# yz-cnsdqz/PSI-release

Measured on AMD Instinct MI355X. Metric: fitting iters/sec (SMPL-X+SDF+Chamfer), PROX-E batch=32, higher is better.
Workload: dtype f32

## Files before the change

include/psi_hip.h:

```cpp
#ifndef PSI_HIP_H
#define PSI_HIP_H

#include <stdint.h>

#ifdef __cplusplus
extern "C" {
#endif

#define PSI_EINVAL (-22)
#define PSI_ETIMEOUT (-110)
#define PSI_ENOMEM (-12)

const char *psi_last_error(void);
int psi_version(void);
int psi_device_info(int *cu_count, int *wave_size, int *clock_khz, int *is_gfx950);

int psi_chamfer_arith_mode(void);
size_t psi_chamfer_workspace_bytes(int B, int n, int m);
int psi_chamfer_forward(const float *xyz1, const float *xyz2, int B, int n, int m,
                        float *dist1, int32_t *idx1, float *dist2, int32_t *idx2,
                        void *workspace, void *stream);
int psi_scratch_release(void *stream, int all);
int psi_chamfer_backward(const float *xyz1, const float *xyz2, float *gradxyz1, float *gradxyz2,
                         const float *graddist1, const float *graddist2,
                         const int32_t *idx1, const int32_t *idx2, int B, int n, int m, void *stream);

typedef struct psi_nn_index psi_nn_index;
int psi_nn_index_create(psi_nn_index **out, const float *h_points, int m);
void psi_nn_index_destroy(psi_nn_index *index);
int psi_nn_index_query(const psi_nn_index *index, const float *xyz1, int B, int n, float *dist1, int32_t *idx1,
                       int32_t *hint, void *stream);

typedef struct psi_nn_index_set psi_nn_index_set;
int psi_nn_index_set_create(psi_nn_index_set **out, const psi_nn_index *const *indices, int S);
void psi_nn_index_set_destroy(psi_nn_index_set *set);
int psi_nn_index_set_query(const psi_nn_index_set *set, const int32_t *slot, const float *xyz1, int B, int n,
                           float *dist1, int32_t *idx1, void *stream);

int psi_sdf_sample_forward(const float *sdf, const int32_t *scene_id, const float *gmin, const float *gmax,
                           const float *verts, int B, int V, int D, int S, int align_corners,
                           float *out_sdf, float *out_grad, void *stream);
int psi_sdf_sample_backward(const float *grad_sdf, const float *out_grad, int B, int V,
                            float *grad_verts, void *stream);
int psi_sdf_penetration_stats(const float *sdf_vals, long n, float *stats, void *stream);

typedef struct psi_lbs_model psi_lbs_model;
int psi_lbs_create(psi_lbs_model **out, const float *h_v_template, const float *h_shapedirs,
                   const float *h_posedirs, const float *h_J_regressor, const float *h_weights,
                   const int32_t *h_parents, int V, int J, int NB);
void psi_lbs_destroy(psi_lbs_model *model);
size_t psi_lbs_workspace_floats(const psi_lbs_model *model, int B);
int psi_lbs_forward(const psi_lbs_model *model, const float *betas, const float *pose, const float *transl,
                    const float *cam_ext, int B, float *verts, float *joints, float *ws, void *stream);
int psi_lbs_backward(const psi_lbs_model *model, const float *grad_verts, const float *betas, const float *pose,
                     const float *cam_ext, int B, float *ws, float *grad_betas, float *grad_pose,
                     float *grad_transl, void *stream);

typedef struct psi_fit_engine psi_fit_engine;
typedef struct psi_fit_config {
    int B, n_contact, m_scene, D, align_corners, world_size, num_pca_comps, max_history;
    int nn_mode;
    float w_rec, w_vposer, w_contact, w_collision, contact_const;
    float lr, beta1, beta2, eps;
    int independent_bodies;
    int concurrent_engines;
    double lr_d, beta1_d, beta2_d;
} psi_fit_config;
int psi_fit_create(psi_fit_engine **out, const psi_lbs_model *lbs, const psi_fit_config *cfg,
                   const float *h_w1, const float *h_b1, const float *h_w2, const float *h_b2,
                   const float *h_w3, const float *h_b3, const float *h_lh_comp, const float *h_rh_comp,
                   const float *h_pose_mean, const int32_t *h_contact_ids,
                   const float *d_scene_verts, const float *d_sdf, const float *h_gmin, const float *h_gmax);
void psi_fit_destroy(psi_fit_engine *engine);
typedef struct psi_fit_scene {
    const float *d_verts;
    const float *d_sdf;
    int m, D;
    float gmin[3], gmax[3];
} psi_fit_scene;
int psi_fit_create_scenes(psi_fit_engine **out, const psi_lbs_model *lbs, const psi_fit_config *cfg,
                          const float *h_w1, const float *h_b1, const float *h_w2, const float *h_b2,
                          const float *h_w3, const float *h_b3, const float *h_lh_comp, const float *h_rh_comp,
                          const float *h_pose_mean, const int32_t *h_contact_ids,
                          const psi_fit_scene *h_scenes, int S);
int psi_fit_set_scene_slots(psi_fit_engine *engine, const int32_t *d_slot, void *stream);
int psi_fit_scene_count(const psi_fit_engine *engine);
int psi_fit_set_problem(psi_fit_engine *engine, const float *d_xhr, const float *d_x_init, const float *d_cam_ext,
                        int reset_optimizer, void *stream);
int psi_fit_forward(psi_fit_engine *engine, float *d_stats, int use_graph, void *stream);
int psi_fit_backward_step(psi_fit_engine *engine, const float *d_stats, int use_graph, void *stream);
int psi_fit_iterate(psi_fit_engine *engine, int n_iter, int use_graph, void *stream);
int psi_fit_read(psi_fit_engine *engine, float *d_x_out, float *d_history_out, int n_hist, int *h_step, void *stream);
int psi_fit_read_losses(psi_fit_engine *engine, int adam_step, float *d_out4, void *stream);
int psi_fit_decode_forward(psi_fit_engine *engine, const float *d_x75, const float *d_cam_ext, float *d_verts, void *stream);
int psi_fit_decode_backward(psi_fit_engine *engine, const float *d_grad_verts, float *d_grad_x75, void *stream);

#define PSI_DP_ID_BYTES 128
typedef struct psi_dp_comm psi_dp_comm;
int psi_dp_unique_id(char *h_id128);
int psi_dp_comm_create(psi_dp_comm **out, const char *h_id128, int rank, int world);
void psi_dp_comm_destroy(psi_dp_comm *comm);
int psi_dp_comm_info(const psi_dp_comm *comm, int *rank, int *world, int *rccl_version);
int psi_dp_allreduce_sum(psi_dp_comm *comm, float *d_buf, int n, void *stream);
int psi_fit_iterate_dp(psi_fit_engine *engine, psi_dp_comm *comm, int n_iter, int use_graph, float *d_stats, void *stream);
int psi_fit_dp_mode(const psi_fit_engine *engine);
int psi_fit_chain_mode(const psi_fit_engine *engine);
int psi_stream_wait(void *stream, int timeout_ms);

int psi_fit_profile(psi_fit_engine *engine, int n_rep, char *h_names, int name_stride, float *h_ms, int max_stages,
                    int *h_n_stages, void *stream);
int psi_fit_copy_buffer(psi_fit_engine *engine, const char *name, float *d_out, long n_floats, void *stream);

size_t psi_linear_workspace_floats(int M, int N, int K);
int psi_linear_forward(const void *x, int x_is_bf16, const float *W, const float *bias, const float *residual, int M, int N, int K,
                       int act, float slope, float *y, float *act_out, float *ws, void *stream);
int psi_linear_forward3(const void *x, int x_is_bf16, const float *W, const float *bias, const float *residual, int M, int N, int K,
                        int act, float slope, float *y, float *act_out, float *ws, void *stream);
size_t psi_linear_backward_workspace_floats(int M, int N, int K);
int psi_linear_backward3(const float *gy, const float *act_out, const float *x, const float *W, int M, int N, int K, float slope, float *gx,
                         float *gW, float *gbias, float *ws, void *stream);
int psi_linear_backward(const float *gy, const float *act_out, const void *x, int x_is_bf16, const float *W, int M, int N, int K,
                        float slope, void *gx, float *gW, float *gbias, float *ws, void *stream);

size_t psi_bn_workspace_floats(long M, int C);
int psi_bn_forward(const void *x, const void *residual, const float *gamma, const float *beta, float *running_mean,
                   float *running_var, long long *num_batches_tracked, long M, int C, int relu, float momentum, float eps,
                   void *y, float *save_mean, float *save_invstd, float *ws, void *stream);
int psi_bn_backward(const void *dy, const void *x, const void *y, const float *gamma, const float *save_mean,
                    const float *save_invstd, long M, int C, int relu, void *dx, void *dresidual, float *dgamma, float *dbeta,
                    float *ws, void *stream);

int psi_conv3x3_supported(int Cin, int Cout, int H, int W);
int psi_conv3x3_forward(const void *x, const void *w, const float *bias, int N, int H, int W, int Cin, int Cout, void *y, void *stream);
size_t psi_conv3x3_wrw_workspace_floats(int N, int H, int W, int Cin, int Cout);
int psi_conv3x3_weight_grad(const void *x, const void *dy, int N, int H, int W, int Cin, int Cout, float *gw, float *ws, void *stream);
int psi_conv3x3_rotate_weight(const void *w, int Cin, int Cout, void *wt, void *stream);
int psi_conv3x3_prepare_weight(const float *w32, int Cin, int Cout, void *wb, void *wt, void *stream);

int psi_maxpool3x3s2_forward(const void *x, int N, int H, int W, int C, void *y, void *idx, void *stream);
int psi_maxpool3x3s2_backward(const void *dy, const void *idx, int N, int H, int W, int C, void *dx, void *stream);

int psi_conv2d_supported(int Cin, int Cout, int KH, int KW, int stride, int pad);
int psi_conv2d_forward(const void *x, int x_bf16, const float *w, const float *bias, int N, int H, int W, int Cin, int Cout, int KH, int KW,
                       int stride, int pad, void *y, int y_bf16, int nterm, void *stream);
int psi_conv2d_input_grad(const void *dy, int dy_bf16, const float *wt, int N, int H, int W, int Cin, int Cout, int KH, int KW, int stride, int pad,
                          void *dx, int dx_bf16, int nterm, void *stream);
int psi_conv2d_prepared_ok(int Cin, int Cout, int KH, int KW, int stride, int pad);
int psi_conv2d_prepare_weight(const float *w, int Cout, int KH, int KW, int Cin, int nterm, void *wf, void *wt, void *stream);
int psi_conv2d_forward_p(const void *x, int x_bf16, const void *wf, const float *bias, int N, int H, int W, int Cin, int Cout, int KH, int KW,
                         int stride, int pad, void *y, int y_bf16, int nterm, void *stream);
int psi_conv2d_input_grad_p(const void *dy, int dy_bf16, const void *wt, int N, int H, int W, int Cin, int Cout, int KH, int KW, int stride, int pad,
                            void *dx, int dx_bf16, int nterm, void *stream);
size_t psi_conv2d_wgrad_workspace_floats(int N, int H, int W, int Cin, int Cout, int KH, int KW, int stride, int pad);
int psi_conv2d_weight_grad(const void *x, int x_bf16, const void *dy, int dy_bf16, int N, int H, int W, int Cin, int Cout, int KH, int KW, int stride,
                           int pad, float *gw, float *ws, int nterm, void *stream);
int psi_adam_step(void *const *p, const void *const *g, void *const *m, void *const *v, const long *n, int count, float *step, unsigned *ticket,
                  double lr, double beta1, double beta2, double eps, double weight_decay, void *stream);
int psi_bn_forward_t(const void *x, int map_f32, const void *residual, const float *gamma, const float *beta, float *running_mean,
                     float *running_var, long long *num_batches_tracked, long M, int C, int relu, float momentum, float eps, void *y,
                     float *save_mean, float *save_invstd, float *ws, int eval_mode, void *stream);
int psi_bn_backward_t(const void *dy, int map_f32, const void *x, const void *y, const float *gamma, const float *beta, const float *save_mean,
                      const float *save_invstd, long M, int C, int relu, void *dx, void *dresidual, float *dgamma, float *dbeta, float *ws,
                      void *stream);
int psi_maxpool3x3s2_forward_t(const void *x, int map_f32, int N, int H, int W, int C, void *y, void *idx, void *stream);
int psi_maxpool3x3s2_backward_t(const void *dy, int map_f32, const void *idx, int N, int H, int W, int C, void *dx, void *stream);

size_t psi_cvae_losses_workspace_floats(void);
int psi_cvae_target(const float *xh72, const float *cam_int, const float *max_d, int B, float *out75, void *stream);
int psi_cvae_losses_forward(const float *rec75, const float *target75, const float *xh72, const float *cam_int, const float *max_d,
                            const float *mu0, const float *logvar0, int nz0, const float *mu1, const float *logvar1, int nz1, int B,
                            float w_rec, float w_kl, float w_vposer, float fca, const float *fca_dev, float *ws, float *xh_rec75,
                            float *losses5, void *stream);
int psi_cvae_losses_backward(const float *rec75, const float *target75, const float *xh72, const float *cam_int, const float *max_d,
                             const float *mu0, const float *logvar0, int nz0, const float *mu1, const float *logvar1, int nz1, int B,
                             float w_rec, float w_kl, float w_vposer, float fca, const float *fca_dev, const float *xh_rec75,
                             const float *g_losses5, const float *g_xh_rec75, float *g_rec75, float *g_mu0, float *g_logvar0,
                             float *g_mu1, float *g_logvar1, void *stream);

size_t psi_scene_losses_workspace_floats(void);
int psi_scene_losses_forward(const float *dist, long n_contact, const float *sdf_vals, long n_sdf, float w_contact, float w_collision,
                             float gate, float *ws, float *losses2, float *stats2, void *stream);
int psi_scene_losses_backward(const float *g_losses2, const float *stats2, const float *dist, const float *xyz1, const int32_t *idx,
                              const int32_t *slot, const float *verts_table, long m, const int32_t *vid, const float *sdf_vals,
                              const float *sdf_grad, int B, int V, int n_c, float w_contact, float w_collision, float gate,
                              const int32_t *chain, float *g_verts, void *stream);
int psi_contact_slot_chain(const int32_t *vid, int n_c, int32_t *chain, void *stream);

int psi_lbs_sdf_counts(const psi_lbs_model *model, const float *betas, const float *pose, const float *transl,
                       const float *cam_ext, int B, const float *sdf, const int32_t *scene_id, const float *gmin,
                       const float *gmax, int D, int S, int align_corners, int32_t *counts, float *ws, void *stream);

typedef struct psi_kmeans psi_kmeans;
int psi_kmeans_create(psi_kmeans **out, const float *obs, int N, int d, const float *guess, int k, int R, float thresh);
void psi_kmeans_destroy(psi_kmeans *km);
int psi_kmeans_iterate(psi_kmeans *km, int n_iter, void *stream);
int psi_kmeans_read(psi_kmeans *km, float *book, int32_t *k_eff, double *avg_dist, int32_t *iters, int *h_converged, void *stream);
int psi_vq(const float *obs, int N, int d, const float *book, int k, int32_t *code, float *dist, void *stream);

typedef struct psi_raster_mesh psi_raster_mesh;
int psi_raster_mesh_create(psi_raster_mesh **out, const float *d_verts, const int32_t *d_faces, const float *d_vlabel, int nv, int nf);
void psi_raster_mesh_destroy(psi_raster_mesh *mesh);
size_t psi_raster_workspace_bytes(int nf, int n_views, int W, int H);
int psi_raster_render(psi_raster_mesh *mesh, const float *d_w2c, const float *d_intr, int n_views, int W, int H, float near_z,
                      float *d_depth, int32_t *d_tri, float *d_seg, int32_t *d_stats, void *d_workspace, void *stream);

typedef struct psi_raster_bodies psi_raster_bodies;
int psi_raster_bodies_create(psi_raster_bodies **out, const int32_t *d_faces, int V, int F);
void psi_raster_bodies_destroy(psi_raster_bodies *bodies);
int psi_raster_bodies_normals(psi_raster_bodies *bodies, const float *d_bverts, int B, float *d_normals, void *stream);
size_t psi_raster_bodies_workspace_bytes(int F, int draws_per_pass, int n_views, int W, int H);
int psi_raster_bodies_render(psi_raster_mesh *scene, const float *d_vrgb, psi_raster_bodies *bodies, const float *d_bverts, int B,
                             const int32_t *d_draw_body, const int32_t *d_draw_view, const float *d_draw_rgb, int M, const float *d_w2c,
                             const float *d_intr, int n_views, int W, int H, float near_z, const float *d_sdepth, const int32_t *d_stri,
                             float bg_r, float bg_g, float bg_b, int draws_per_pass, uint8_t *d_rgb, float *d_depth, int32_t *d_draw,
                             float *d_bdepth, int32_t *d_bid, int32_t *d_counts, int32_t *d_stats, void *d_workspace, void *stream);

typedef struct psi_mesh_sdf psi_mesh_sdf;
int psi_mesh_sdf_create(psi_mesh_sdf **out, const float *d_verts, const int32_t *d_faces, int nv, int nf);
void psi_mesh_sdf_destroy(psi_mesh_sdf *m);
int psi_mesh_sdf_info(const psi_mesh_sdf *m, int32_t info[4]);
int psi_mesh_sdf_compute(psi_mesh_sdf *m, const float gmin[3], const float gmax[3], int D, int mode, float *d_out, void *stream);
int psi_mesh_sdf_count_pairs(psi_mesh_sdf *m, const float gmin[3], const float gmax[3], int D, int mode, unsigned long long *d_pairs,
                             void *stream);

int psi_mesh_winding_compute(psi_mesh_sdf *m, const float gmin[3], const float gmax[3], int D, float beta, int cluster, float *d_f, void *stream);
int psi_mesh_winding_count(psi_mesh_sdf *m, const float gmin[3], const float gmax[3], int D, float beta, int cluster,
                           unsigned long long *d_counts , void *stream);
int psi_mesh_sdf_apply_sign(const float *d_f, float level, float *d_vol, long long n, void *stream);

size_t psi_snapshot_canvas_workspace_bytes(int n_views);
int psi_snapshot_canvas(const float *d_depth, const float *d_seg, int n_views, int H, int W, int th, int tw, float clip_depth, float clip_seg,
                        const int32_t *d_windows, const float *d_target_z, float *d_depth_canvas, float *d_seg_canvas, float *d_max_d,
                        float *d_seg_max, int32_t *d_usable, void *d_workspace, void *stream);

int psi_mesh_cloud_count(const float *d_verts, const int32_t *d_faces, int nv, int nf, float spacing, int32_t *d_tri_rows, float origin[3],
                         long long *n_rows, long long *n_cands, void *stream);
int psi_mesh_cloud_rows(const float *d_verts, const int32_t *d_faces, int nv, int nf, float spacing, const int64_t *d_tri_row_off,
                        long long n_rows, int32_t *d_row_tri, int32_t *d_row_cnt, void *stream);
int psi_mesh_cloud_emit(const float *d_verts, const int32_t *d_faces, int nv, int nf, float spacing, const float origin[3],
                        const int64_t *d_tri_row_off, const int32_t *d_row_tri, const int64_t *d_row_off, long long n_rows, long long n_cands,
                        float *d_pos, int32_t *d_tri, int64_t *d_cell, uint32_t *d_key, void *stream);
int psi_mesh_cloud_winners(const int64_t *d_cell_sorted, const int64_t *d_perm, const uint32_t *d_key, long long n, int32_t *d_keep,
                           void *stream);
int psi_mesh_cloud_compact(const float *d_pos, const int32_t *d_tri, const int32_t *d_keep, const int64_t *d_keep_scan, long long n,
                           long long n_out, float *d_points, int32_t *d_out_tri, void *stream);

int psi_flood_fill(const uint8_t *d_open, int Dx, int Dy, int Dz, const int32_t *d_seed_nodes, int n, uint8_t *d_free, int *h_rounds, void *stream);
int psi_mesh_orient_votes(const float *d_points, const int32_t *d_tri, long long n, const float *d_verts, int nv, const int32_t *d_faces, int nf,
                          const uint8_t *d_free, const float gmin[3], const float gmax[3], int D, float delta, int32_t *d_votes, void *stream);

typedef struct psi_body_overlap psi_body_overlap;
int psi_body_overlap_create(psi_body_overlap **out, const int32_t *h_faces, int V, int F);
void psi_body_overlap_destroy(psi_body_overlap *h);
int psi_body_overlap_info(const psi_body_overlap *h, int32_t info[2]);
size_t psi_body_overlap_workspace_bytes(long long n_cand, int F);
int psi_body_overlap_boxes(const psi_body_overlap *h, const float *d_verts, int B, float *d_boxes, int32_t *d_bad, void *stream);
int psi_body_overlap_count(const psi_body_overlap *h, const float *d_verts, const int32_t *d_group, int B, const float *d_boxes,
                           int32_t *d_pair_count, void *stream);
int psi_body_overlap_emit(const psi_body_overlap *h, const float *d_verts, const int32_t *d_group, int B, const float *d_boxes,
                          const int32_t *d_pair_count, const int64_t *d_cand_off, const int64_t *d_chunk_off, long long n_cand,
                          long long n_chunks, int32_t *d_cand, int32_t *d_chunks, void *stream);
int psi_body_overlap_wind(const psi_body_overlap *h, const float *d_verts, int B, const int32_t *d_cand, long long n_cand,
                          const int32_t *d_chunks, long long n_chunks, void *d_workspace, size_t workspace_bytes, void *stream);
int psi_body_overlap_decide(const psi_body_overlap *h, int B, const int32_t *d_cand, long long n_cand, const void *d_workspace,
                            size_t workspace_bytes, float *d_w, int32_t *d_counts, uint32_t *d_mask, void *stream);
// ... 72 lines not shown
```

psi-release_amd/csrc/fit.hip:

```cpp
#include "psi_internal.h"
#include "blob.h"
#ifdef PSI_HEAD_STOPS
__device__ int psi_dbg_sstop;
#define PSI_SSTOP(k) do { if (psi_dbg_sstop == (k)) return; } while (0)
__device__ int psi_dbg_pstop;
#define PSI_PSTOP(k) do { if (psi_dbg_pstop == (k)) asm volatile("s_endpgm"); } while (0)
__device__ int psi_dbg_cstop;
#define PSI_CSTOP() do { if (psi_dbg_cstop) asm volatile("s_endpgm"); } while (0)
#define PSI_TRACE(lo, hi) PsiBlockTrace trace_((lo), (hi))
__device__ unsigned long long psi_dbg_tl[4 * 8192];
struct PsiBlockTrace {
    unsigned long long t0;
    int kind;
    int sel_lo, sel_hi;
    __device__ PsiBlockTrace(int lo = 9, int hi = 10) : t0(wall_clock64()), kind(0), sel_lo(lo), sel_hi(hi) {}
    __device__ ~PsiBlockTrace()
    {
        const unsigned bid = blockIdx.y * gridDim.x + blockIdx.x;
        if (psi_dbg_sstop < sel_lo || psi_dbg_sstop > sel_hi || threadIdx.x != 0 || bid >= 8192) return;
        unsigned long long *o = psi_dbg_tl + 4 * (size_t)bid;
        o[0] = t0;
        o[1] = wall_clock64();
        o[2] = (unsigned long long)__builtin_amdgcn_s_getreg((31 << 11) | 4) | ((unsigned long long)__builtin_amdgcn_s_getreg((31 << 11) | 20) << 32);
        o[3] = (unsigned long long)kind;
    }
};
extern "C" int psi_dbg_timeline(unsigned long long *out, int nblocks)
{
    return (int)hipMemcpyFromSymbol(out, HIP_SYMBOL(psi_dbg_tl), sizeof(unsigned long long) * 4 * (size_t)(nblocks < 8192 ? nblocks : 8192));
}
#endif
#include "lbs_device.h"
#include "chain_plan.h"
#include "lbs_joint_device.h"
#include "sdf_device.h"
#include "nnindex_device.h"
#include <initializer_list>
#include <limits.h>
#include <memory>
#include <math.h>
#include <stdlib.h>
#include <string.h>
#include <type_traits>
#include <vector>

namespace {

constexpr int NH = 512;
constexpr int NZ = 32;
constexpr int NJ6 = 126;
constexpr int XD = 75;
#ifndef PSI_HEAD_THREADS
#define PSI_HEAD_THREADS 512
#endif
constexpr int HB = PSI_HEAD_THREADS;
static_assert(HB >= 384 && HB % 128 == 0, "the head / tail kernels place work on threads up to 256 + 75");
constexpr int KQ = HB / 128;
constexpr int KS3 = HB / 32;
constexpr int OS1 = HB / 8;
typedef float f4 __attribute__((ext_vector_type(4)));

struct FitDev {
    int B, V, Vpad, J, NB, n_c, m, D, align_corners, world, ncomp, nfp, nsdfblk;
    int indep;
    float w_rec, w_vp, w_contact, w_col, cconst;
    float lr, beta1, beta2, eps;
    float one_m_beta1, one_m_beta2;
    double lr_d, beta1_d, beta2_d;
    const float *W1T, *b1, *W2T, *b2, *W3T, *b3;
    const float *W1, *W2, *W3;
    const float *lhc, *rhc, *pose_mean;
    const int *vid;
    const int *cs_ptr, *cs_idx;
    const int *cs_first;
    const float *scene, *sdf, *gmin, *gmax;
    const float *sdf_cells;
    const float *Wct;
    float *x, *xhr, *cam, *adam_m, *adam_v;
    int *step;
    float *h1, *h2, *o6, *betas20, *pose, *transl, *verts, *og, *gq, *fpart, *penpart, *recpart, *vppart;
    float *cverts;
    float *g_betas, *g_pose, *g_transl, *g_rot;
    unsigned long long *hx_o6, *hx_gh1;
    unsigned *hx_epoch;
    int *hx_err;
    int hc;
#ifdef PSI_HEAD_STOPS
    int stop_h, stop_t;
#define HSTOP(k) do { if (f.stop_h == (k)) return; } while (0)
#define TSTOP(k) do { if (f.stop_t == (k)) return; } while (0)
#else
#define HSTOP(k)
#define TSTOP(k)
#endif
    int *nn_hint;
    float *history;
    int max_hist;
    int fused_bwd, ncp, ncp3;
    float *glc, *gvpc, *vpc;
    float *gtc_part;
#ifndef PSI_GV_SLOTS
#define PSI_GV_SLOTS 1024
#endif
    static_assert(PSI_GV_SLOTS >= 128, "one slot per body and class at least: fused_bwd runs batches up to 128 (merged_scene)");
    unsigned *gvbits;
    int gv_sps;
    const float *dirs_ch;
    const float *WTt_c;
    float *gA_part, *gfeat_part;
    float *spb;
    int nsv, nsv_c, nsn_m, nsn_c, spm, spc;
    unsigned long long *penmask;
    int pen_skip;
};

__device__ __forceinline__ float leaky(float v, float slope) { return v > 0.0f ? v : v * slope; }

__device__ __forceinline__ void gs_forward(const float *x6, float *R)
{
    float a1[3] = {x6[0], x6[2], x6[4]}, a2[3] = {x6[1], x6[3], x6[5]};
    float n1 = fmaxf(sqrtf(a1[0] * a1[0] + a1[1] * a1[1] + a1[2] * a1[2]), 1e-12f);
    float b1[3] = {a1[0] / n1, a1[1] / n1, a1[2] / n1};
    float d = b1[0] * a2[0] + b1[1] * a2[1] + b1[2] * a2[2];
    float u[3] = {a2[0] - d * b1[0], a2[1] - d * b1[1], a2[2] - d * b1[2]};
    float n2 = fmaxf(sqrtf(u[0] * u[0] + u[1] * u[1] + u[2] * u[2]), 1e-12f);
    float b2[3] = {u[0] / n2, u[1] / n2, u[2] / n2};
    float b3[3] = {b1[1] * b2[2] - b1[2] * b2[1], b1[2] * b2[0] - b1[0] * b2[2], b1[0] * b2[1] - b1[1] * b2[0]};
    for (int r = 0; r < 3; r++) {
        R[r * 3 + 0] = b1[r];
        R[r * 3 + 1] = b2[r];
        R[r * 3 + 2] = b3[r];
    }
}

__device__ __forceinline__ void gs_backward(const float *x6, const float *gR, float *g6)
{
    float a1[3] = {x6[0], x6[2], x6[4]}, a2[3] = {x6[1], x6[3], x6[5]};
    float n1 = fmaxf(sqrtf(a1[0] * a1[0] + a1[1] * a1[1] + a1[2] * a1[2]), 1e-12f);
    float b1[3] = {a1[0] / n1, a1[1] / n1, a1[2] / n1};
    float d = b1[0] * a2[0] + b1[1] * a2[1] + b1[2] * a2[2];
    float u[3] = {a2[0] - d * b1[0], a2[1] - d * b1[1], a2[2] - d * b1[2]};
    float n2 = fmaxf(sqrtf(u[0] * u[0] + u[1] * u[1] + u[2] * u[2]), 1e-12f);
    float b2[3] = {u[0] / n2, u[1] / n2, u[2] / n2};
    float gb1[3] = {gR[0], gR[3], gR[6]}, gb2[3] = {gR[1], gR[4], gR[7]}, gb3[3] = {gR[2], gR[5], gR[8]};
    gb1[0] += b2[1] * gb3[2] - b2[2] * gb3[1];
    gb1[1] += b2[2] * gb3[0] - b2[0] * gb3[2];
    gb1[2] += b2[0] * gb3[1] - b2[1] * gb3[0];
    gb2[0] += gb3[1] * b1[2] - gb3[2] * b1[1];
    gb2[1] += gb3[2] * b1[0] - gb3[0] * b1[2];
    gb2[2] += gb3[0] * b1[1] - gb3[1] * b1[0];
    float p = b2[0] * gb2[0] + b2[1] * gb2[1] + b2[2] * gb2[2];
    float gu[3] = {(gb2[0] - b2[0] * p) / n2, (gb2[1] - b2[1] * p) / n2, (gb2[2] - b2[2] * p) / n2};
    float q = gu[0] * b1[0] + gu[1] * b1[1] + gu[2] * b1[2];
    float ga2[3] = {gu[0] - b1[0] * q, gu[1] - b1[1] * q, gu[2] - b1[2] * q};
    for (int i = 0; i < 3; i++) gb1[i] += -d * gu[i] - q * a2[i];
    float r = b1[0] * gb1[0] + b1[1] * gb1[1] + b1[2] * gb1[2];
    float ga1[3] = {(gb1[0] - b1[0] * r) / n1, (gb1[1] - b1[1] * r) / n1, (gb1[2] - b1[2] * r) / n1};
    g6[0] = ga1[0]; g6[2] = ga1[1]; g6[4] = ga1[2];
    g6[1] = ga2[0]; g6[3] = ga2[1]; g6[5] = ga2[2];
}

__device__ __forceinline__ void rotmat_to_aa(const float *R, float *aa)
{
    const float m00 = R[0], m01 = R[3], m02 = R[6], m10 = R[1], m11 = R[4], m12 = R[7], m20 = R[2], m21 = R[5], m22 = R[8];
    float q[4], t;
    if (m22 < 1e-6f) {
        if (m00 > m11) {
            t = 1 + m00 - m11 - m22;
            q[0] = m12 - m21; q[1] = t; q[2] = m01 + m10; q[3] = m20 + m02;
        } else {
            t = 1 - m00 + m11 - m22;
            q[0] = m20 - m02; q[1] = m01 + m10; q[2] = t; q[3] = m12 + m21;
        }
    } else {
        if (m00 < -m11) {
            t = 1 - m00 - m11 + m22;
            q[0] = m01 - m10; q[1] = m20 + m02; q[2] = m12 + m21; q[3] = t;
        } else {
            t = 1 + m00 + m11 + m22;
            q[0] = t; q[1] = m12 - m21; q[2] = m20 - m02; q[3] = m01 - m10;
        }
    }
// ... 262 lines not shown
            return;
        }
        const int cw = psi_ld<int>(contact_of, (unsigned)v * 4u);
        if (!(cw >> 24)) return;
        float *row = cverts + (size_t)b * n_c * 3;
        psi_st(row, (unsigned)(cw & 0xffffff) * 12u, psi_p3{x, y, z});
        if ((cw >> 24) > 1)
            for (int ci = cs_ptr[v] + 1; ci < cs_ptr[v + 1]; ci++) psi_st(row, (unsigned)cs_idx[ci] * 12u, psi_p3{x, y, z});
    }
    __device__ __forceinline__ void vertex(int n, int b, int v, float x, float y, float z, bool live) { vertex_at(G, n, b, v, x, y, z, live); }
    __device__ __forceinline__ void vertex_at(const PsiSdfGrid &G, int n, int b, int v, float x, float y, float z, bool live)
    {
        s[n] = 0.0f;
        neg[n] = false;
#pragma unroll
        for (int a = 0; a < 3; a++) gm[n][a] = 0.0f;
        if (!live) return;
        float g[3];
        if (G.cells) {
            bool in[3];
            const float val = psi_sdf_sample_cells(G, x, y, z, g, in);
            neg[n] = val < 0.0f;
#pragma unroll
            for (int a = 0; a < 3; a++) g[a] = (neg[n] && in[a]) ? g[a] : 0.0f;
            s[n] = neg[n] ? -val : 0.0f;
        } else {
            const float val = psi_trilinear(sdf, gmin, gmax, x, y, z, D, align_corners, g);
            neg[n] = val < 0.0f;
#pragma unroll
            for (int a = 0; a < 3; a++) g[a] = neg[n] ? g[a] : 0.0f;
            s[n] = neg[n] ? -val : 0.0f;
        }
        if (gl) {
#pragma unroll
            for (int a = 0; a < 3; a++) gm[n][a] = g[a];
            return;
        }
        psi_st(og + (size_t)b * Vpad * 4, (unsigned)v * 16u, f4{g[0], g[1], g[2], 0.0f});
    }
    __device__ __forceinline__ void backward(int n, int b, unsigned v12, const psi_f2 (&T2)[6], const float *C)
    {
        if (!gl) return;
        const float gx = gm[n][0], gy = gm[n][1], gz = gm[n][2];
        float lx = gx, ly = gy, lz = gz;
        if (C) {
            lx = psi_dot3(C[0], C[4], C[8], gx, gy, gz);
            ly = psi_dot3(C[1], C[5], C[9], gx, gy, gz);
            lz = psi_dot3(C[2], C[6], C[10], gx, gy, gz);
        }
        psi_st(gl + (size_t)b * Npad, v12, psi_p3{lx, ly, lz});
        const float vx = psi_dot3(T2[0].x, T2[2].x, T2[4].x, lx, ly, lz), vy = psi_dot3(T2[0].y, T2[2].y, T2[4].y, lx, ly, lz),
                    vz = psi_dot3(T2[1].x, T2[3].x, T2[5].x, lx, ly, lz);
        psi_st(gvp + (size_t)b * Npad, v12, psi_p3{vx, vy, vz});
        gvmax[n] = fmaxf(gvmax[n], fmaxf(fabsf(vx), fmaxf(fabsf(vy), fabsf(vz))));
        gs[n][0] = lx; gs[n][1] = ly; gs[n][2] = lz;
    }
    __device__ __forceinline__ void finish(int n, int b, int vblock, int nvb)
    {
        __shared__ psi_f2 red[PSI_SKIN_BLK / 64];
        __shared__ float red3[PSI_SKIN_BLK / 64][3];
        __shared__ float redm[PSI_SKIN_BLK / 64];
        const float ws = psi_wave_sum(s[n]);
        const unsigned long long negm = __builtin_amdgcn_ballot_w64(neg[n]);
        const float wc = (float)(int)__builtin_popcountll(negm);
        if ((threadIdx.x & 63) == 0) red[threadIdx.x >> 6] = (psi_f2){ws, wc};
        if (gl) {
            if ((threadIdx.x & 63) == 0) penmask[((size_t)b * nvb + vblock) * (PSI_SKIN_BLK / 64) + (threadIdx.x >> 6)] = negm;
            const float sx = psi_wave_sum(gs[n][0]), sy = psi_wave_sum(gs[n][1]), sz = psi_wave_sum(gs[n][2]);
            float mx = gvmax[n];
#pragma unroll
            for (int o2 = 32; o2 > 0; o2 >>= 1) mx = fmaxf(mx, __shfl_xor(mx, o2, 64));
            if ((threadIdx.x & 63) == 0) {
                red3[threadIdx.x >> 6][0] = sx;
                red3[threadIdx.x >> 6][1] = sy;
                red3[threadIdx.x >> 6][2] = sz;
                redm[threadIdx.x >> 6] = mx;
            }
        }
        __syncthreads();
        if (gl && threadIdx.x == 64) {
            float mx = redm[0];
#pragma unroll
            for (int w = 1; w < PSI_SKIN_BLK / 64; w++) mx = fmaxf(mx, redm[w]);
            if (mx > 0.0f) atomicMax(gmaxp + (size_t)b * gv_sps + (vblock & (gv_sps - 1)), __float_as_uint(mx));
        }
        if (threadIdx.x == 0) {
            psi_f2 a = red[0];
#pragma unroll
            for (int w = 1; w < PSI_SKIN_BLK / 64; w++) a += red[w];
            *(psi_f2 *)(penpart + ((size_t)b * nvb + vblock) * 2) = a;
        }
        if (gl && threadIdx.x < 3) {
            float a = 0.0f;
#pragma unroll
            for (int w = 0; w < PSI_SKIN_BLK / 64; w++) a += red3[w][threadIdx.x];
            gtp[((size_t)vblock * B + b) * 4 + threadIdx.x] = a;
        }
    }
};

struct SdfPenEpilogueScenes : SdfPenEpilogue {
    const PsiSdfGrid *gtab;
    const int *slot;
    PsiSdfGrid Gb[2];
    template <int NB>
    __device__ __forceinline__ void load_grids(int b0, int B)
    {
#pragma unroll
        for (int n = 0; n < NB; n++) Gb[n] = gtab[slot[min(b0 + n, B - 1)]];
    }
    __device__ __forceinline__ void vertex(int n, int b, int v, float x, float y, float z, bool live) { vertex_at(Gb[n], n, b, v, x, y, z, live); }
};

template <bool SCENES>
using SdfEpilogue = std::conditional_t<SCENES, SdfPenEpilogueScenes, SdfPenEpilogue>;

template <bool SCENES>
static inline SdfEpilogue<SCENES> make_sdf_epilogue(const FitDev &f, const PsiSdfGrid &G, bool contact_vertices_only, const PsiLbsView *bwd,
                                                    const PsiSdfGrid *gtab = nullptr, const int *slot = nullptr)
{
    SdfEpilogue<SCENES> e;
    static_cast<SdfPenEpilogue &>(e) = {SCENES ? PsiSdfGrid{} : G, f.sdf, f.gmin, f.gmax, f.og, f.penpart, f.D, f.align_corners, f.Vpad,
                                        contact_vertices_only ? f.cs_first : nullptr, {0.0f, 0.0f}, {false, false}, f.cverts, f.cs_ptr, f.cs_idx, f.n_c,
                                        nullptr, nullptr, nullptr, 0, f.B, {}, {}, {0.0f, 0.0f}, f.gvbits, f.gv_sps, nullptr};
    if (bwd) {
        e.penmask = f.penmask;
        e.gl = bwd->gl;
        e.gvp = bwd->g_vp;
        e.gtp = bwd->gt_part_w;
        e.Npad = bwd->m.Npad;
    }
    if constexpr (SCENES) {
        e.gtab = gtab;
        e.slot = slot;
        e.Gb[0] = e.Gb[1] = PsiSdfGrid{};
    }
    return e;
}

template <int LPQ>
__device__ __forceinline__ void psi_contact_part_sums(float x, float (&out)[psi_sum_parts_per_wave(LPQ)])
{
    x += psi_dpp<0xB1, 0xf>(x);
    x += psi_dpp<0x4E, 0xf>(x);
    x += psi_dpp<0x124, 0xf>(x);
    x += psi_dpp<0x128, 0xf>(x);
    x += psi_dpp<0x142, 0xa>(x);
    if (psi_sum_part_lanes(LPQ) == 64) x += psi_dpp<0x143, 0xc>(x);
#pragma unroll
    for (int p = 0; p < psi_sum_parts_per_wave(LPQ); p++)
        out[p] = __builtin_bit_cast(float, __builtin_amdgcn_readlane(__builtin_bit_cast(int, x), psi_sum_last_lane(LPQ, p)));
}

template <int LPQ>
struct ContactSkinSrc {
    static_assert(LPQ == 2 || LPQ == 4, "the query's lane group skins its own vertex with 2 or 4 lanes");
    static constexpr int NT = psikd::kd_threads(LPQ);
    static constexpr int NST = (PSI_JP * 6 + NT - 1) / NT;
    static constexpr int CT0 = LPQ == 2 ? 80 : 128;
    FitDev f;
    LbsDev m;
    const float *As, *v_posed;
    psi_f2 (*sA)[6];
    psi_f2 st[NST];
    float ct;
    int v;
    float px, py, pz;
    float *sCT;
    static constexpr int NWQ = PSI_JP / 4 - 2, NWE = 10;
    f4 wq[NWE];
    int jslot;
    float (*sTR)[9] = nullptr;
    float gvm = 0.0f;
    float gs[3] = {0.0f, 0.0f, 0.0f};
    int bq = 0;
    bool live = false;
    __device__ __forceinline__ void issue(int b, int j, bool active)
    {
        jslot = j;
        bq = b;
        live = active;
#pragma unroll
        for (int q = 0; q < NST; q++) {
            const int idx = threadIdx.x + q * NT;
            st[q] = idx < m.J * 6 ? psi_ld<psi_f2>(As + (size_t)b * m.J * 12, (unsigned)idx * 8u) : (psi_f2){0.0f, 0.0f};
        }
        const int k = (int)threadIdx.x - CT0;
        ct = 0.0f;
        if (k >= 0 && k < 12) ct = f.cam[(size_t)b * 16 + k];
        else if (k >= 12 && k < 15) ct = f.transl[(size_t)b * 3 + (k - 12)];
        v = f.vid[j];
    }
    __device__ __forceinline__ void fetch(int b)
    {
        const psi_p3 p = psi_ld<psi_p3>(v_posed + (size_t)b * m.Npad, (unsigned)v * 12u);
        px = p.x; py = p.y; pz = p.z;
        const f4 *wrow = (const f4 *)(f.Wct + (size_t)jslot * PSI_JP);
#pragma unroll
        for (int q = 0; q < NWE; q++) wq[q] = wrow[q];
    }
    __device__ __forceinline__ void prepare(int)
    {
        psi_f2 (*sA_)[6] = psi_transform_stage<1>()[0];
        __shared__ float sCT_[16];
        __shared__ float sTR_[psikd::kd_qpb(LPQ)][9];
#pragma unroll
        for (int q = 0; q < NST; q++) {
            const int idx = threadIdx.x + q * NT;
            if (idx < PSI_JP * 6) (&sA_[0][0])[idx] = st[q];
        }
        const int k = (int)threadIdx.x - CT0;
        if (k >= 0 && k < 16) sCT_[k] = ct;
        __syncthreads();
        sA = sA_;
        sCT = sCT_;
        sTR = sTR_;
    }
    __device__ __forceinline__ void point(int b, int j, int c, float &qx, float &qy, float &qz) const
    {
        if constexpr (LPQ == 2) {
            const f4 *wrow = (const f4 *)(f.Wct + (size_t)j * PSI_JP);
            psi_f2 T0 = {0.0f, 0.0f}, T1 = {0.0f, 0.0f}, U0 = {0.0f, 0.0f}, U1 = {0.0f, 0.0f};
#pragma unroll
            for (int q = 0; q < NWQ; q++) {
                const f4 w4 = q < NWE ? wq[q] : wrow[q];
#pragma unroll
                for (int t = 0; t < 4; t++) {
                    const psi_f2 w2 = {w4[t], w4[t]};
                    T0 = __builtin_elementwise_fma(w2, sA[q * 4 + t][2 * c], T0);
                    T1 = __builtin_elementwise_fma(w2, sA[q * 4 + t][2 * c + 1], T1);
                    U0 = __builtin_elementwise_fma(w2, sA[q * 4 + t][4], U0);
                    U1 = __builtin_elementwise_fma(w2, sA[q * 4 + t][5], U1);
                }
            }
            if (f.fused_bwd) {
                float *tr = sTR[threadIdx.x / LPQ];
                tr[3 * c] = T0.x; tr[3 * c + 1] = T0.y; tr[3 * c + 2] = T1.x;
                if (c == 0) { tr[6] = U0.x; tr[7] = U0.y; tr[8] = U1.x; }
                if (c == 0 && live) psi_st(f.vpc + (size_t)b * f.ncp3, (unsigned)j * 12u, psi_p3{px, py, pz});
            }
            const float xr = psi_dot3p(T0.x, T0.y, T1.x, T1.y, px, py, pz) + sCT[12 + c];
            const float xr2 = psi_dot3p(U0.x, U0.y, U1.x, U1.y, px, py, pz) + sCT[14];
            const int base = (threadIdx.x & 63) & ~1;
            const float x = __shfl(xr, base, 64), y = __shfl(xr, base + 1, 64), z = __shfl(xr2, base, 64);
            const float *C = sCT;
            qx = psi_dot3p(C[0], C[1], C[2], C[3], x, y, z);
            qy = psi_dot3p(C[4], C[5], C[6], C[7], x, y, z);
            qz = psi_dot3p(C[8], C[9], C[10], C[11], x, y, z);
            return;
        }
        const int r = c < 2 ? c : 2;
        const f4 *wrow = (const f4 *)(f.Wct + (size_t)j * PSI_JP);
        psi_f2 T0 = {0.0f, 0.0f}, T1 = {0.0f, 0.0f};
#pragma unroll
        for (int q = 0; q < NWQ; q++) {
            const f4 w4 = q < NWE ? wq[q] : wrow[q];
#pragma unroll
            for (int t = 0; t < 4; t++) {
                const psi_f2 w2 = {w4[t], w4[t]};
                T0 = __builtin_elementwise_fma(w2, sA[q * 4 + t][2 * r], T0);
                T1 = __builtin_elementwise_fma(w2, sA[q * 4 + t][2 * r + 1], T1);
            }
        }
        if (f.fused_bwd && c < 3) {
            float *tr = &sTR[threadIdx.x / LPQ][3 * c];
            tr[0] = T0.x; tr[1] = T0.y; tr[2] = T1.x;
        }
        float xr = psi_dot3p(T0.x, T0.y, T1.x, T1.y, px, py, pz) + sCT[12 + r];
        const int base = (threadIdx.x & 63) & ~3;
        const float x = __shfl(xr, base, 64), y = __shfl(xr, base + 1, 64), z = __shfl(xr, base + 2, 64);
        const float *C = sCT;
        qx = psi_dot3p(C[0], C[1], C[2], C[3], x, y, z);
        qy = psi_dot3p(C[4], C[5], C[6], C[7], x, y, z);
        qz = psi_dot3p(C[8], C[9], C[10], C[11], x, y, z);
    }
    __device__ __forceinline__ void contact_post(size_t, float gx, float gy, float gz)
    {
        if (!f.fused_bwd) return;
        const float *C = sCT;
        const float lx = psi_dot3(C[0], C[4], C[8], gx, gy, gz), ly = psi_dot3(C[1], C[5], C[9], gx, gy, gz), lz = psi_dot3(C[2], C[6], C[10], gx, gy, gz);
        const float *R = sTR[threadIdx.x / LPQ];
        const size_t row = (size_t)bq * f.ncp3;
        const unsigned off = (unsigned)jslot * 12u;
        psi_st(f.glc + row, off, psi_p3{lx, ly, lz});
        const float vx = psi_dot3(R[0], R[3], R[6], lx, ly, lz), vy = psi_dot3(R[1], R[4], R[7], lx, ly, lz), vz = psi_dot3(R[2], R[5], R[8], lx, ly, lz);
        psi_st(f.gvpc + row, off, psi_p3{vx, vy, vz});
        gvm = fmaxf(fabsf(vx), fmaxf(fabsf(vy), fabsf(vz)));
        if constexpr (LPQ != 2) psi_st(f.vpc + row, off, psi_p3{px, py, pz});
        gs[0] = lx; gs[1] = ly; gs[2] = lz;
    }
    __device__ __forceinline__ void contact_finish(int b, int bx, int nbx)
    {
        if (!f.fused_bwd) return;
        constexpr int PPW = psi_sum_parts_per_wave(LPQ);
        __shared__ float wsum3[psi_sum_parts(LPQ)][3];
        __shared__ float wmax[psi_sum_waves(LPQ)];
        float sx[PPW], sy[PPW], sz[PPW];
        psi_contact_part_sums<LPQ>(gs[0], sx);
        psi_contact_part_sums<LPQ>(gs[1], sy);
        psi_contact_part_sums<LPQ>(gs[2], sz);
        float mx = gvm;
#pragma unroll
        for (int o2 = 32; o2 > 0; o2 >>= 1) mx = fmaxf(mx, __shfl_xor(mx, o2, 64));
        if ((threadIdx.x & 63) == 0) {
#pragma unroll
            for (int p = 0; p < PPW; p++) {
                wsum3[psi_sum_slot(LPQ, threadIdx.x >> 6, p)][0] = sx[p];
                wsum3[psi_sum_slot(LPQ, threadIdx.x >> 6, p)][1] = sy[p];
                wsum3[psi_sum_slot(LPQ, threadIdx.x >> 6, p)][2] = sz[p];
            }
            wmax[threadIdx.x >> 6] = mx;
        }
        __syncthreads();
        if (threadIdx.x == 64) {
            float m2 = wmax[0];
#pragma unroll
            for (int w = 1; w < psi_sum_waves(LPQ); w++) m2 = fmaxf(m2, wmax[w]);
            if (m2 > 0.0f) atomicMax(f.gvbits + PSI_GV_SLOTS + (size_t)b * f.gv_sps + (bx & (f.gv_sps - 1)), __float_as_uint(m2));
        }
        if (threadIdx.x < 3) {
            float a = 0.0f;
#pragma unroll
            for (int w = 0; w < psi_sum_parts(LPQ); w++) a += wsum3[w][threadIdx.x];
            f.gtc_part[((size_t)b * nbx + bx) * 4 + threadIdx.x] = a;
        }
    }
};

#ifdef PSI_HEAD_STOPS
extern "C" int psi_dbg_kd_mark(unsigned long long *out, int nblocks)
{
    return (int)hipMemcpyFromSymbol(out, HIP_SYMBOL(psi_kd_mark), sizeof(unsigned long long) * 4 * (size_t)(nblocks < 8192 ? nblocks : 8192));
}
extern "C" int psi_dbg_kd_reason(int *out) { return (int)hipMemcpyFromSymbol(out, HIP_SYMBOL(psi_kd_reason), sizeof(int) * 8); }
extern "C" int psi_dbg_kd_stat(int *out, int nblocks)
{
    return (int)hipMemcpyFromSymbol(out, HIP_SYMBOL(psi_kd_stat), sizeof(int) * 4 * (size_t)(nblocks < 8192 ? nblocks : 8192));
}
#endif
template <bool SCENES>
using SceneTrees = std::conditional_t<SCENES, const psikd::KdDev *__restrict__, psikd::KdDev>;

template <int NB, bool SCENES, int LPQ>
__global__ __launch_bounds__(256, 6) void fwd_scene_kernel(FitDev f, LbsDev m, const float *__restrict__ As, const float *__restrict__ v_posed,
                                                           SceneTrees<SCENES> T, int n_kd, int nqb, int rows, float gscale, int skin_first, SdfEpilogue<SCENES> epi)
{
    extern __shared__ int smem_i[];
#ifdef PSI_HEAD_STOPS
    if (psi_dbg_sstop == 1 && (int)blockIdx.x >= n_kd) return;
    if (psi_dbg_sstop == 2 && (int)blockIdx.x < n_kd) return;
    if (psi_dbg_sstop == 3) return;
    PsiBlockTrace trace;
    if (threadIdx.x < 4 && blockIdx.x < 8192) psi_kd_stat[4 * blockIdx.x + threadIdx.x] = 0;
    trace.kind = skin_first ? ((int)blockIdx.x >= (int)gridDim.x - n_kd) : ((int)blockIdx.x < n_kd);
#endif
    int bid = blockIdx.x;
    bool is_kd;
    if (skin_first) {
        const int n_sk = (int)gridDim.x - n_kd;
        is_kd = bid >= n_sk;
        if (is_kd) bid -= n_sk;
    } else {
        is_kd = bid < n_kd;
        if (!is_kd) bid -= n_kd;
    }
    if (is_kd) {
        const int b = bid / nqb, bx = bid % nqb;
        psikd::KdDev tree = psikd::KdDev();
        const psikd::KdDev *__restrict__ tab = nullptr;
        const int *slot = nullptr;
        if constexpr (SCENES) {
            tab = T;
            slot = epi.slot;
        } else tree = T;
        psikd::kd_query_body<LPQ, true, SCENES>(tree, ContactSkinSrc<LPQ>{f, m, As, v_posed, nullptr, {}, 0.0f, 0, 0.0f, 0.0f, 0.0f, nullptr, {}, 0}, f.n_c, (float *)nullptr, (int *)nullptr,
                                           f.cconst, gscale, f.fused_bwd ? (float *)nullptr : f.gq, f.fpart, f.nn_hint, rows, tab, slot, bx, b, nqb, smem_i);
    } else {
        const int i = bid;
        if constexpr (SCENES) epi.template load_grids<NB>((i / f.nsdfblk) * NB, f.B);
        psi_skin_fwd_body<NB, PsiBlendCompact>(m, As, v_posed, f.transl, f.cam, f.B, f.verts, epi, i % f.nsdfblk, (i / f.nsdfblk) * NB, f.nsdfblk);
    }
}

template <int NB, bool SCENES>
__global__ __launch_bounds__(PSI_SKIN_BLK, 6) void skin_fwd_sdf_kernel(LbsDev m, const float *__restrict__ As, const float *__restrict__ v_posed,
                                                                     const float *__restrict__ transl, const float *__restrict__ cam_ext,
                                                                     int B, float *__restrict__ verts, SdfEpilogue<SCENES> epi)
{
    if constexpr (SCENES) epi.template load_grids<NB>((int)blockIdx.y * NB, B);
    psi_skin_fwd_body<NB, PsiBlendPipelined>(m, As, v_posed, transl, cam_ext, B, verts, epi, (int)blockIdx.x, (int)blockIdx.y * NB, (int)gridDim.x);
}

__global__ void contact_weight_table_kernel(const float *__restrict__ WT, int Vpad, const int *__restrict__ vid, int n_c, int J, float *__restrict__ Wct)
{
    const int i = blockIdx.x * 256 + threadIdx.x;
    if (i >= n_c * PSI_JP) return;
    const int slot = i / PSI_JP, j = i % PSI_JP;
    Wct[i] = j < J ? WT[(size_t)j * Vpad + vid[slot]] : 0.0f;
}

__global__ __launch_bounds__(1024) void loss_finalize_kernel(FitDev f, float *stats)
{
    __shared__ float red[16];
    const int t = threadIdx.x, nt = 1024;
    auto total = [&](const float *p, int n, int stride) {
        float a0 = 0, a1 = 0, a2 = 0, a3 = 0;
        int i = t;
        for (; i + 3 * nt < n; i += 4 * nt) {
            a0 += p[(size_t)i * stride];
            a1 += p[(size_t)(i + nt) * stride];
            a2 += p[(size_t)(i + 2 * nt) * stride];
            a3 += p[(size_t)(i + 3 * nt) * stride];
        }
        for (; i < n; i += nt) a0 += p[(size_t)i * stride];
        return block_sum((a0 + a1) + (a2 + a3), red);
    };
    float s_rec = total(f.recpart, f.B, 1);
    float s_vp = total(f.vppart, f.B, 1);
    float s_f = total(f.fpart, f.B * f.nfp, 1);
    float s_pen = total(f.penpart, f.B * f.nsdfblk, 2);
    float n_pen = total(f.penpart + 1, f.B * f.nsdfblk, 2);
    if (t == 0) {
        stats[0] = s_rec; stats[1] = s_vp; stats[2] = s_f; stats[3] = s_pen; stats[4] = n_pen; stats[5] = 0.0f;
        *f.step += 1;
    }
}

__device__ __forceinline__ void fit_stats_body(const FitDev &f, float *__restrict__ stats)
{
    __shared__ float red[16];
    const int t = threadIdx.x, nt = blockDim.x;
    if (f.indep) {
        float a0 = 0, a1 = 0, a2 = 0, a3 = 0;
        for (int b = t; b < f.B; b += nt) {
            a0 += f.recpart[b];
            a1 += f.vppart[b];
            float sf = 0, sp = 0, cn = 0;
            for (int k = 0; k < f.nfp; k++) sf += f.fpart[(size_t)b * f.nfp + k];
            for (int k = 0; k < f.nsdfblk; k++) {
                sp += f.penpart[2 * ((size_t)b * f.nsdfblk + k)];
                cn += f.penpart[2 * ((size_t)b * f.nsdfblk + k) + 1];
            }
            a2 += sf;
            a3 += cn > 0.0f ? sp / cn : 0.0f;
            f.spb[b] = cn > 0.0f ? -f.w_col / cn : 0.0f;
        }
        const float s0 = block_sum(a0, red), s1 = block_sum(a1, red), s2 = block_sum(a2, red), s3 = block_sum(a3, red);
        if (t == 0) {
            stats[0] = s0; stats[1] = s1; stats[2] = s2; stats[3] = s3; stats[4] = 0.0f; stats[5] = 0.0f;
            *f.step += 1;
        }
        return;
    }
    auto total = [&](const float *p, int n, int stride) {
        float a0 = 0, a1 = 0, a2 = 0, a3 = 0;
        int i = t;
        for (; i + 3 * nt < n; i += 4 * nt) {
            a0 += p[(size_t)i * stride];
            a1 += p[(size_t)(i + nt) * stride];
            a2 += p[(size_t)(i + 2 * nt) * stride];
            a3 += p[(size_t)(i + 3 * nt) * stride];
        }
        for (; i < n; i += nt) a0 += p[(size_t)i * stride];
        return block_sum((a0 + a1) + (a2 + a3), red);
    };
    const float s_rec = total(f.recpart, f.B, 1);
    const float s_vp = total(f.vppart, f.B, 1);
    const float s_f = total(f.fpart, f.B * f.nfp, 1);
    const float s_pen = total(f.penpart, f.B * f.nsdfblk, 2);
    const float n_pen = total(f.penpart + 1, f.B * f.nsdfblk, 2);
    if (t == 0) {
        stats[0] = s_rec; stats[1] = s_vp; stats[2] = s_f; stats[3] = s_pen; stats[4] = n_pen; stats[5] = 0.0f;
        *f.step += 1;
    }
}

#ifndef PSI_FIT_PF_MODEL
#define PSI_FIT_PF_MODEL 1
#endif
#ifndef PSI_FIT_PF_CONTACT
#define PSI_FIT_PF_CONTACT 2
#endif
template <int MT, int PF_MODEL, int PF_CONTACT>
__global__ __launch_bounds__(256) __attribute__((amdgpu_waves_per_eu(2, 2))) void fit_bwd_joint_kernel(
    FitDev f, LbsDev m, const float *__restrict__ g_vp, const float *__restrict__ gl, const float *__restrict__ v_posed, PsiSkaPlan ska, int n_blend,
    int kgroups, float *__restrict__ stats)
{
    const int n_ska = ska.n_ska;
    constexpr int SMEM_B = psi_blend_bwd_h_smem_f4<(MT + 1) / 2>();
    __shared__ f4 smem[SMEM_B > SKA_SMEM_F4 ? SMEM_B : SKA_SMEM_F4];
    const int bid = blockIdx.x;
#ifdef PSI_HEAD_STOPS
    PsiBlockTrace trace(11, 11);
    trace.kind = bid < n_ska ? (bid < ska.n_c ? 1 : 0) : (bid < n_ska + n_blend ? 2 : 4);
#endif
    if (bid < n_ska) {
        int sl, b0, nbody;
        psi_ska_map(ska, bid, sl, b0, nbody);
        float *part = f.gA_part + (size_t)sl * f.B * PSI_JP * 16;
        if (sl < f.nsv) {
            const PsiSkaSlice o = {m.WTt + (size_t)sl * 4 * PSI_JP * 64, gl + (size_t)sl * 768, v_posed + (size_t)sl * 768, (size_t)m.Npad, part};
            const unsigned all = (1u << min(nbody, f.B - b0)) - 1u;
            const unsigned live = f.pen_skip ? psi_pen_slice_live(f.penmask, f.Vpad / 64, sl, f.B, b0, nbody) : all;
            skin_bwd_A_zero(o, b0, all & ~live);
            if (live) skin_bwd_A_dispatch_live(o, b0, live, smem);
        } else {
            const int c = sl - f.nsv;
            const PsiSkaSlice o = {f.WTt_c + (size_t)c * 4 * PSI_JP * 64, f.glc + (size_t)c * 768, f.vpc + (size_t)c * 768, (size_t)f.ncp3, part};
            skin_bwd_A_dispatch(o, f.B, b0, nbody, smem);
        }
    } else if (bid < n_ska + n_blend) {
        int kg, slice, bg;
        psi_blend_bwd_place(bid - n_ska, kgroups, f.nsn_m + f.nsn_c, kg, slice, bg);
#ifdef PSI_HEAD_STOPS
        trace.kind = slice < f.nsn_m ? 2 : 3;
#endif
        float *part = f.gfeat_part + (size_t)slice * f.B * m.Kpad;
        const float dsc_inv = m.dirs_unscale * PSI_FEAT_SCALE;
        if (slice < f.nsn_m) {
            const PsiBlendBwdColsH o = {m.dirs_bh, g_vp, (size_t)m.Npad, m.Kpad, m.Npad / 16, f.gvbits, f.gv_sps, dsc_inv, f.pen_skip ? f.penmask : nullptr, f.Vpad / 64};
            blend_bwd_h_body<(MT + 1) / 2, PF_MODEL>(o, f.B, slice * f.spm, (slice + 1) * f.spm, part, kg, bg, smem);
        } else {
            const int c = slice - f.nsn_m;
            const PsiBlendBwdColsH o = {f.dirs_ch, f.gvpc, (size_t)f.ncp3, m.Kpad, f.ncp3 / 16, f.gvbits + PSI_GV_SLOTS, f.gv_sps, dsc_inv, nullptr, 0};
            blend_bwd_h_body<(MT + 1) / 2, PF_CONTACT>(o, f.B, c * f.spc, (c + 1) * f.spc, part, kg, bg, smem);
        }
    } else {
        fit_stats_body(f, stats);
    }
// ... 322 lines not shown
        gs_backward(o6v, sgrot + t * 9, g6);
        for (int i = 0; i < 6; i++) sg6[(t - 1) * 6 + i] = g6[i];
    } else if (t >= 64 && t < 64 + 2 * f.ncomp) {
        int i = t - 64;
        const float *comp = i < f.ncomp ? f.lhc : f.rhc;
        int ii = i < f.ncomp ? i : i - f.ncomp;
        const float *gp = sgpose + (i < f.ncomp ? 75 : 120);
        float a = 0;
        for (int e = 0; e < 45; e++) a += comp[ii * 45 + e] * gp[e];
        sgx[(i < f.ncomp ? 51 : 63) + ii] = a;
    } else if (t >= 128 && t < 128 + 3) {
        sgx[t - 128] = gtv;
    } else if (t >= 160 && t < 160 + 10) {
        sgx[9 + (t - 160)] = sgbetas[t - 160];
    }
    __syncthreads();
    TSTOP(3);
    {
        f4 a = {0, 0, 0, 0};
#pragma unroll
        for (int i = 0; i < PRE3; i++) a += w3p[i] * sg6[o0 + i];
#pragma unroll 8
        for (int o = o0 + PRE3; o < o1; o++) a += *(const f4 *)(w3 + (size_t)o * NH) * sg6[o];
        part4[os3 * NQ + og3] = a;
    }
    __syncthreads();
    if (t < NS) {
        float a = 0.0f;
        const float *p = (const float *)part4;
#pragma unroll
        for (int q = 0; q < OSPL; q++) a += p[q * NS + t];
        sga2[t] = a * (h2v > 0.0f ? 1.0f : 0.2f);
    }
    __syncthreads();
    TSTOP(4);
    {
        f4 a0 = {0, 0, 0, 0}, a1 = {0, 0, 0, 0};
        const float *g = sga2 + kq2 * RPER;
#pragma unroll
        for (int o = 0; o < PRE2; o += 2) {
            a0 += w2p[o] * g[o];
            a1 += w2p[o + 1] * g[o + 1];
        }
#pragma unroll 8
        for (int o = PRE2; o < RPER; o += 2) {
            a0 += *(const f4 *)(w2 + (size_t)o * NH) * g[o];
            a1 += *(const f4 *)(w2 + (size_t)(o + 1) * NH) * g[o + 1];
        }
        part4[kq2 * 128 + og2] = a0 + a1;
    }
    __syncthreads();
    TSTOP(5);
    {
        const float *p = (const float *)part4;
        float a = p[t];
#pragma unroll
        for (int q = 1; q < KQ; q++) a += p[q * NH + t];
        if (C == 1) {
            sga1[t] = a * (h1[t] > 0.0f ? 1.0f : 0.2f);
        } else if (!last) {
            hx_put(f.hx_gh1 + ((size_t)b * C + c) * NH + t, a, tag);
            return;
        } else {
            unsigned long long *p8 = f.hx_gh1 + (size_t)b * C * NH + t;
            unsigned long long w[C - 1 ? C - 1 : 1];
#pragma unroll
            for (int cc = 0; cc < C - 1; cc++) w[cc] = hx_peek(p8 + (size_t)cc * NH);
            float o = 0.0f;
#pragma unroll
            for (int cc = 0; cc < C - 1; cc++) o += hx_value(p8 + (size_t)cc * NH, w[cc], tag, f.hx_err);
            sga1[t] = (o + a) * (h1v > 0.0f ? 1.0f : 0.2f);
        }
    }
    __syncthreads();
    TSTOP(6);
    {
        f4 a = {0, 0, 0, 0};
        if (C == 1) {
#pragma unroll
            for (int i = 0; i < O1; i++) a += *(const f4 *)(w1 + (size_t)i * NZ) * sga1[os1 * O1 + i];
        } else {
#pragma unroll
            for (int i = 0; i < O1; i++) a += w1p[i] * sga1[os1 * O1 + i];
        }
        part1[os1][kg1] = a;
    }
    __syncthreads();
    if (t < 8) {
        f4 a = {0, 0, 0, 0};
        for (int os = 0; os < OS1; os++) a += part1[os][t];
        for (int e = 0; e < 4; e++) sgx[19 + t * 4 + e] = a[e];
    }
    __syncthreads();
    TSTOP(7);
    if (C > 1 && t == 0) f.hx_epoch[f.B + b] = tag;
    if (!ADAM) {
        if (t < XD) g_out[(size_t)b * XD + t] = sgx[t];
        return;
    }
    if (ta >= 0 && ta < XD) {
        const float Bg = f.indep ? 1.0f : (float)f.B * (float)f.world;
        float g = sgx[ta];
        float df = xhrv - sx[ta];
        g += f.w_rec / (Bg * XD) * (df > 0.0f ? -1.0f : (df < 0.0f ? 1.0f : 0.0f));
        if (ta >= 19 && ta < 19 + NZ) g += f.w_vp / (Bg * NZ) * 2.0f * sx[ta];
        size_t o = (size_t)b * XD + ta;
        float m = am * f.beta1 + f.one_m_beta1 * g;
        float v = av * f.beta2 + f.one_m_beta2 * g * g;
        f.adam_m[o] = m;
        f.adam_v[o] = v;
        float denom = sqrtf(v) / bc2_sqrt + f.eps;
        f.x[o] = sx[ta] - step_size * (m / denom);
    }
}

__global__ void sdf_to_cells_kernel(const float *__restrict__ src, float *__restrict__ dst, int D)
{
    const int nbr = D >> 2;
    const size_t i = (size_t)blockIdx.x * 256 + threadIdx.x, n = (size_t)D * D * D * 8;
    if (i >= n) return;
    const int c = (int)(i & 7), l = (int)((i >> 3) & 63);
    const size_t br = i >> 9;
    const int bz = (int)(br % nbr), by = (int)((br / nbr) % nbr), bx = (int)(br / ((size_t)nbr * nbr));
    const int ix = min(4 * bx + (l >> 4) + (c >> 2), D - 1), iy = min(4 * by + ((l >> 2) & 3) + ((c >> 1) & 1), D - 1),
              iz = min(4 * bz + (l & 3) + (c & 1), D - 1);
    dst[i] = src[((size_t)ix * D + iy) * D + iz];
}

__global__ void scene_slots_kernel(const int *__restrict__ src, int *__restrict__ dst, int B, int S)
{
    const int b = blockIdx.x * 256 + threadIdx.x;
    if (b < B) dst[b] = min(max(src[b], 0), S - 1);
}

__global__ void adam_reset_kernel(float *m, float *v, int *step, int n)
{
    int i = blockIdx.x * 256 + threadIdx.x;
    if (i < n) { m[i] = 0.0f; v[i] = 0.0f; }
    if (i == 0) *step = 0;
}

}

#ifndef PSI_FIT_SEARCH_LANES_DEFAULT
#define PSI_FIT_SEARCH_LANES_DEFAULT 2
#endif
#ifndef PSI_GRAPH_UNROLL
#define PSI_GRAPH_UNROLL 10
#endif
constexpr int GRAPH_UNROLL = PSI_GRAPH_UNROLL;

struct FitKnobs {
    bool split_scene, keep_verts, no_fused_bwd, sdf_linear, scene_skin_first, bwdv_mb, no_pen_skip, bwd_pf1, chain_in_head;
    int head_cluster, skin_nb, ska_nbody, search_lanes;
#ifdef PSI_HEAD_STOPS
    int head_stop, tail_stop, skin_stop;
#endif
};

static FitKnobs fit_read_knobs()
{
    auto is = [](const char *name, char c) { const char *v = getenv(name); return v && v[0] == c; };
    auto num = [](const char *name) { const char *v = getenv(name); return v ? atoi(v) : 0; };
    FitKnobs k = {};
    k.split_scene = is("PSI_SPLIT_SCENE", '1');
    k.keep_verts = is("PSI_KEEP_VERTS", '1');
    k.no_fused_bwd = is("PSI_FIT_FUSED_BWD", '0');
    k.no_pen_skip = is("PSI_FIT_PEN_SKIP", '0');
    k.bwd_pf1 = is("PSI_FIT_BWD_PF", '1');
    k.chain_in_head = is("PSI_FIT_CHAIN_IN_HEAD", '1');
    k.sdf_linear = is("PSI_SDF_LINEAR", '1');
    k.scene_skin_first = is("PSI_SCENE_ORDER", '1');
    k.bwdv_mb = is("PSI_BWDV_MB", '1');
    const int hc = num("PSI_HEAD_CLUSTER");
    if (hc == 1 || hc == 2 || hc == 4 || hc == 8) k.head_cluster = hc;
    if (getenv("PSI_SKIN_NB")) k.skin_nb = num("PSI_SKIN_NB") == 2 ? 2 : 1;
    k.ska_nbody = psi_ska_nbody_override(SKA_NBODY);
    const int sl = num("PSI_FIT_SEARCH_LANES");
    if (sl == 2 || sl == 4) k.search_lanes = sl;
#ifdef PSI_HEAD_STOPS
    k.head_stop = num("PSI_HEAD_STOP");
    k.tail_stop = num("PSI_TAIL_STOP");
    k.skin_stop = num("PSI_SKIN_STOP");
#endif
    return k;
}

struct FitModes {
    bool self_skin;
    bool merged_scene;
    bool keep_verts;
    bool fused_bwd;
    int skin_nb;
    int search_lanes;
    int hc;
    int gv_sps;
    PsiStreamSplit split;
    PsiChainPlan chain;
};

static FitModes fit_decide(const psi_fit_config *cfg, const FitKnobs &knobs, int J, int ncp3, const PsiLbsCounts &mc, int cus)
{
    FitModes d = {};
    d.self_skin = cfg->nn_mode == 1 && J <= PSI_JP - 8 && psikd::kd_qpb(psikd::LPQ_OPS) == psikd::kd_qpb(2);
    d.search_lanes = knobs.search_lanes ? knobs.search_lanes : mc.compressed_weights ? 4 : PSI_FIT_SEARCH_LANES_DEFAULT;
    d.merged_scene = d.self_skin && cfg->B <= 128 && !knobs.split_scene;
    d.keep_verts = !d.merged_scene || knobs.keep_verts;
    const long bodies = (long)cfg->B * (cfg->concurrent_engines > 1 ? cfg->concurrent_engines : 1);
    d.hc = bodies <= 32 ? 8 : bodies <= 64 ? 4 : bodies <= 128 ? 2 : 1;
    if (knobs.head_cluster) d.hc = knobs.head_cluster;
    d.gv_sps = 16;
    while (d.gv_sps > 1 && (long)d.gv_sps * cfg->B > PSI_GV_SLOTS) d.gv_sps >>= 1;
    d.split = psi_stream_split(mc.Npad / 16, ncp3 / 16, mc.nsn);
    d.fused_bwd = d.merged_scene && !knobs.no_fused_bwd && d.split.nsn_c > 0;
    d.skin_nb = cfg->B > 128 && !mc.compressed_weights ? 2 : 1;
    if (knobs.skin_nb) d.skin_nb = knobs.skin_nb;
    d.chain = knobs.chain_in_head ? PsiChainPlan{0, 0} : psi_chain_plan(cfg->B, d.hc, mc.blend_wg, mc.blend_gy, cus);
    return d;
}

struct FitPlan {
    int mt;
    int kgroups, n_blend;
    PsiSkaPlan ska;
    bool pf1;
};
static FitPlan fit_plan_make(const FitDev &f, const LbsDev &m, int ska_nbody_override, bool pf1)
{
    FitPlan p;
    p.kgroups = m.Kpad / 64;
    p.mt = f.B > 32 ? 4 : (f.B > 16 ? 2 : 1);
    p.n_blend = p.kgroups * (f.nsn_m + f.nsn_c) * psi_cdiv(f.B, 16 * p.mt);
    p.ska = psi_ska_plan(f.B, f.nsv, f.nsv_c, SKA_NBODY, ska_nbody_override);
    p.pf1 = pf1;
    return p;
}

struct FitGraph { hipGraph_t g; hipGraphExec_t exec; bool ready; };

struct FitCaptured {
    enum Kind { Ok, Refused, Error } kind;
    int rc;
};

template <class Seq>
static FitCaptured fit_graph_capture(FitGraph *G, hipStream_t st, Seq &&seq)
{
    auto failed = [](const char *what, hipError_t he) {
        psi_set_error("%s failed: %s", what, hipGetErrorString(he));
        return FitCaptured{FitCaptured::Error, (int)he};
    };
    if (!st) {
        psi_set_error("invalid argument: graph capture needs a non-default stream");
        return {FitCaptured::Error, PSI_EINVAL};
    }
    hipError_t he = hipStreamBeginCapture(st, hipStreamCaptureModeRelaxed);
    if (he != hipSuccess) return failed("begin of the stream capture", he);
    const int rc = seq();
    hipGraph_t g = nullptr;
    he = hipStreamEndCapture(st, &g);
    if (!rc && he == hipSuccess) {
        he = hipGraphInstantiate(&G->exec, g, nullptr, nullptr, 0);
        if (he != hipSuccess) {
            (void)hipGraphDestroy(g);
            return failed("hipGraphInstantiate", he);
        }
        G->g = g;
        G->ready = true;
        return {FitCaptured::Ok, 0};
    }
    if (g) (void)hipGraphDestroy(g);
    if (!rc) (void)failed("hipStreamEndCapture", he);
    const bool refused = (he >= hipErrorStreamCaptureUnsupported && he <= hipErrorStreamCaptureWrongThread) || rc == 1000 + 4 || rc == 1000 + 5;
    return {refused ? FitCaptured::Refused : FitCaptured::Error, rc ? rc : (int)he};
}

static int fit_graph_launch(const FitGraph &G, hipStream_t st)
{
    PSI_CHECK_HIP(hipGraphLaunch(G.exec, st));
    return 0;
}

static void fit_graph_drop(FitGraph *G)
{
    if (G->ready) {
        (void)hipGraphExecDestroy(G->exec);
        (void)hipGraphDestroy(G->g);
    }
    *G = FitGraph{};
}

struct FitGraphTier { int iters; FitGraph *graph; };

template <class Seq>
static FitCaptured fit_run_graphs(hipStream_t st, int n_iter, int *done, std::initializer_list<FitGraphTier> tiers, Seq &&one)
{
    for (const FitGraphTier &t : tiers) {
        if (n_iter - *done < t.iters) continue;
        if (!t.graph->ready) {
            const FitCaptured c = fit_graph_capture(t.graph, st, [&]() {
                int rc = 0;
                for (int i = 0; i < t.iters && !rc; i++) rc = one();
                return rc;
            });
            if (c.kind != FitCaptured::Ok) return c;
        }
        for (; *done + t.iters <= n_iter; *done += t.iters)
            if (int rc = fit_graph_launch(*t.graph, st)) return {FitCaptured::Error, rc};
    }
    return {FitCaptured::Ok, 0};
}

enum {
    FIT_G_ITER_1, FIT_G_ITER_N, FIT_G_ITER_2N,
    FIT_G_HALF_FWD, FIT_G_HALF_BWD,
    FIT_G_DP_1, FIT_G_DP_N,
    FIT_N_GRAPHS
};

struct psi_fit_engine {
    FitDev d;
    PsiSdfGrid grid;
    const psi_lbs_model *lbs;
    psi_nn_index *nn_index;
    float *lbs_ws;
    PsiLbsView lv;
    void *nn_ws;
    char *blob;
    PsiBlob table;
    float *stats_local;
    FitKnobs knobs;
    FitModes mode;
    FitPlan plan;
    int n_scenes;
    psi_nn_index **scene_index;
    float **scene_vol;
    char *scene_blob;
    psikd::KdDev *d_kd_tab;
    PsiSdfGrid *d_grid_tab;
    int *d_slot;
    int kd_rows;
    FitGraph graphs[FIT_N_GRAPHS];
    const float *half_stats[2];
    const void *dp_comm;
    const float *dp_stats;
    bool dp_warm;
    bool dp_no_graph;
};

template <bool LINKS_IN_HEAD>
static void launch_head_fwd(const FitDev &f, const PsiLbsView &lv, hipStream_t st)
{
    const dim3 g(f.B * f.hc), blk(HB);
    switch (f.hc) {
    case 8: hipLaunchKernelGGL((head_fwd_kernel<8, LINKS_IN_HEAD>), g, blk, 0, st, f, lv); break;
    case 4: hipLaunchKernelGGL((head_fwd_kernel<4, LINKS_IN_HEAD>), g, blk, 0, st, f, lv); break;
    case 2: hipLaunchKernelGGL((head_fwd_kernel<2, LINKS_IN_HEAD>), g, blk, 0, st, f, lv); break;
    default: hipLaunchKernelGGL((head_fwd_kernel<1, true>), g, blk, 0, st, f, lv); break;
    }
}

static int fit_head_blend(psi_fit_engine *e, hipStream_t st)
{
    const FitDev &f = e->d;
    const PsiChainPlan &cp = e->mode.chain;
    const bool role = cp.n_links_wg > 0 && f.hc > 1;
    if (role) launch_head_fwd<false>(f, e->lv, st);
    else launch_head_fwd<true>(f, e->lv, st);
    PSI_CHECK_LAUNCH("head_fwd_kernel");
    psi_mark("head_fwd_kernel", st);
    return role ? psi_lbs_blend_forward_links(e->lbs, f.B, e->lbs_ws, cp.n_links_wg, cp.bodies_per_wave, st)
                : psi_lbs_blend_forward(e->lbs, f.B, e->lbs_ws, st);
}

template <bool ADAM>
static void launch_head_bwd(const FitDev &f, const PsiLbsView &lv, float *g_out, hipStream_t st)
{
    const dim3 g(f.B * f.hc), blk(HB);
    switch (f.hc) {
    case 8: hipLaunchKernelGGL((head_bwd_adam_kernel<8, ADAM>), g, blk, 0, st, f, lv, g_out); break;
    case 4: hipLaunchKernelGGL((head_bwd_adam_kernel<4, ADAM>), g, blk, 0, st, f, lv, g_out); break;
    case 2: hipLaunchKernelGGL((head_bwd_adam_kernel<2, ADAM>), g, blk, 0, st, f, lv, g_out); break;
    default: hipLaunchKernelGGL((head_bwd_adam_kernel<1, ADAM>), g, blk, 0, st, f, lv, g_out); break;
    }
}

enum class FitStats {
    Finalize,
    Backward,
    Caller
};

static inline FitStats fit_stats_source(const psi_fit_engine *e, FitStats wish)
{
    return wish == FitStats::Backward && !e->mode.fused_bwd && e->d.B >= PSI_SKIN_MB_MIN_B ? FitStats::Finalize : wish;
}

static int fit_launch_stats(psi_fit_engine *e, float *stats, hipStream_t st)
{
    hipLaunchKernelGGL(loss_finalize_kernel, dim3(1), dim3(1024), 0, st, e->d, stats);
    PSI_CHECK_LAUNCH("loss_finalize_kernel");
    psi_mark("loss_finalize_kernel", st);
    return 0;
}

template <int NB, bool SCENES, int LPQ>
static void launch_fwd_scene(const psi_fit_engine *e, float gscale, hipStream_t st)
{
    const FitDev &f = e->d;
    const int nqb = f.nfp, n_kd = nqb * f.B, skin_first = e->knobs.scene_skin_first ? 1 : 0;
    const dim3 grid(n_kd + f.nsdfblk * psi_cdiv(f.B, NB));
    FitDev fk = f;
    if (!e->mode.keep_verts) fk.verts = nullptr;
    const auto epi = make_sdf_epilogue<SCENES>(f, e->grid, false, e->mode.fused_bwd ? &e->lv : nullptr, e->d_grid_tab, e->d_slot);
    SceneTrees<SCENES> T;
    int rows;
    if constexpr (SCENES) {
        T = e->d_kd_tab;
        rows = e->kd_rows;
    } else {
        T = psi_nn_index_dev(e->nn_index);
        rows = T.rows;
    }
    hipLaunchKernelGGL((fwd_scene_kernel<NB, SCENES, LPQ>), grid, dim3(256), psikd::kd_lds_bytes(LPQ, rows), st, fk, e->lv.m, e->lv.A, e->lv.v_posed, T, n_kd, nqb, rows,
                       gscale, skin_first, epi);
}

template <int NB, bool SCENES>
static void launch_skin_fwd_sdf(const psi_fit_engine *e, bool all_verts, hipStream_t st)
{
    const FitDev &f = e->d;
    hipLaunchKernelGGL((skin_fwd_sdf_kernel<NB, SCENES>), dim3(f.nsdfblk, psi_cdiv(f.B, NB)), dim3(PSI_SKIN_BLK), 0, st, e->lv.m, e->lv.A, e->lv.v_posed,
                       f.transl, f.cam, f.B, f.verts, make_sdf_epilogue<SCENES>(f, e->grid, !all_verts, nullptr, e->d_grid_tab, e->d_slot));
}

template <class L>
static void fit_scene_dispatch(const psi_fit_engine *e, L &&launch)
{
    using One = std::integral_constant<int, 1>;
    using Two = std::integral_constant<int, 2>;
    switch ((e->n_scenes ? 2 : 0) | (e->mode.skin_nb == 2 ? 1 : 0)) {
    case 0: launch(One{}, std::false_type{}); break;
    case 1: launch(Two{}, std::false_type{}); break;
    case 2: launch(One{}, std::true_type{}); break;
    default: launch(Two{}, std::true_type{}); break;
    }
}

static int fit_forward(psi_fit_engine *e, float *stats, hipStream_t st, FitStats who)
{
    FitDev &f = e->d;
    int rc = fit_head_blend(e, st);
    if (rc) return rc;
    float gscale = f.w_contact / ((f.indep ? 1.0f : (float)f.B * (float)f.world) * (float)f.n_c);
    if (e->nn_index && e->mode.merged_scene) {
        fit_scene_dispatch(e, [&](auto nb, auto scenes) {
            if (e->mode.search_lanes == 2) launch_fwd_scene<decltype(nb)::value, decltype(scenes)::value, 2>(e, gscale, st);
            else launch_fwd_scene<decltype(nb)::value, decltype(scenes)::value, 4>(e, gscale, st);
        });
        PSI_CHECK_LAUNCH("fwd_scene_kernel");
        psi_mark("fwd_scene_kernel", st);
    } else {
        const bool all_verts = !e->nn_index || e->knobs.keep_verts;
        fit_scene_dispatch(e, [&](auto nb, auto scenes) { launch_skin_fwd_sdf<decltype(nb)::value, decltype(scenes)::value>(e, all_verts, st); });
        PSI_CHECK_LAUNCH("skin_fwd_sdf_kernel");
        psi_mark("skin_fwd_sdf_kernel", st);
        if (e->n_scenes)
            rc = psi_nn_index_contact_set(e->d_kd_tab, e->d_slot, e->kd_rows, all_verts ? f.verts : f.cverts, all_verts ? (long)f.V * 3 : (long)f.n_c * 3,
                                          all_verts ? f.vid : nullptr, f.B, f.n_c, f.cconst, gscale, f.gq, f.fpart, f.nn_hint, st);
        else if (e->nn_index && !all_verts)
            rc = psi_nn_index_contact(e->nn_index, f.cverts, (long)f.n_c * 3, nullptr, f.B, f.n_c, f.cconst, gscale, f.gq, f.fpart, f.nn_hint, st);
        else if (e->nn_index)
            rc = psi_nn_index_contact(e->nn_index, f.verts, (long)f.V * 3, f.vid, f.B, f.n_c, f.cconst, gscale, f.gq, f.fpart, f.nn_hint, st);
        else
            rc = psi_nn_contact(f.verts, (long)f.V * 3, f.vid, f.scene, f.B, f.n_c, f.m, e->nn_ws, f.cconst, gscale, f.gq, f.fpart, nullptr, st);
        if (rc) return rc;
    }
    return fit_stats_source(e, who) == FitStats::Finalize ? fit_launch_stats(e, stats, st) : 0;
}

static int fit_backward_joint(psi_fit_engine *e, float *stats, hipStream_t st, FitStats who)
{
    FitDev &f = e->d;
    const FitPlan &p = e->plan;
    const dim3 grid(p.ska.n_ska + p.n_blend + (fit_stats_source(e, who) == FitStats::Backward ? 1 : 0));
#define PSI_LAUNCH_FIT_JOINT(MT_, PFM_, PFC_)                                                                                      \
    hipLaunchKernelGGL((fit_bwd_joint_kernel<MT_, PFM_, PFC_>), grid, dim3(256), 0, st, f, e->lv.m, e->lv.g_vp, e->lv.gl, e->lv.v_posed, p.ska, p.n_blend, p.kgroups, stats)
#define PSI_LAUNCH_FIT_JOINT_MT(MT_)                                                                                               \
    do {                                                                                                                           \
        if (p.pf1) PSI_LAUNCH_FIT_JOINT(MT_, 1, 1);                                                                                \
        else PSI_LAUNCH_FIT_JOINT(MT_, PSI_FIT_PF_MODEL, PSI_FIT_PF_CONTACT);                                                      \
    } while (0)
    if (p.mt == 4) PSI_LAUNCH_FIT_JOINT_MT(4);
    else if (p.mt == 2) PSI_LAUNCH_FIT_JOINT_MT(2);
    else PSI_LAUNCH_FIT_JOINT_MT(1);
#undef PSI_LAUNCH_FIT_JOINT_MT
#undef PSI_LAUNCH_FIT_JOINT
    PSI_CHECK_LAUNCH("fit_bwd_joint_kernel");
    psi_mark("bwd_joint_kernel", st);
    return 0;
}

static int fit_backward_tail(psi_fit_engine *e, float *stats, hipStream_t st)
{
    FitDev &f = e->d;
    const long nred = (long)f.B * PSI_JP * 16 + (long)f.B * e->lv.m.Kpad + (long)f.B * 4;
    hipLaunchKernelGGL(fit_reduce_kernel, dim3(psi_cdiv(nred * PSI_RSPL, 256)), dim3(256), 0, st, f, e->lv, stats);
    PSI_CHECK_LAUNCH("fit_reduce_kernel");
    psi_mark("reduce_partials_kernel", st);
    launch_head_bwd<true>(f, e->lv, nullptr, st);
    PSI_CHECK_LAUNCH("head_bwd_adam_kernel");
    psi_mark("head_bwd_adam_kernel", st);
    return 0;
}

static int fit_backward(psi_fit_engine *e, float *stats, hipStream_t st, FitStats who)
{
    FitDev &f = e->d;
    if (e->mode.fused_bwd) {
        int rc = fit_backward_joint(e, stats, st, who);
        return rc ? rc : fit_backward_tail(e, stats, st);
    }
    const bool big = f.B >= PSI_SKIN_MB_MIN_B;
    const bool mb = big && (e->lv.m.Wc || e->knobs.bwdv_mb);
    const dim3 bgrid(f.nsdfblk, mb ? psi_cdiv(f.B, PSI_SKIN_MB) : f.B);
#define PSI_LAUNCH_BWD_V(...)                                                                                                      \
    hipLaunchKernelGGL((psi_skin_bwd_v_kernel<__VA_ARGS__>), bgrid, dim3(PSI_SKIN_BLK), 0, st, e->lv.m, e->lv.A, src, f.cam, f.B, e->lv.gl, e->lv.g_vp, e->lv.gt_part_w)
    if (fit_stats_source(e, who) == FitStats::Backward) {
        const FitGradSource<true> src{f, stats, 0.0f, nullptr, 0, {}, false};
        if (mb) psi_launch_skin_bwd_v_mb(e->lv.m, e->lv.A, src, f.cam, f.B, e->lv.gl, e->lv.g_vp, e->lv.gt_part_w, st);
        else PSI_LAUNCH_BWD_V(FitGradSource<true>);
    } else {
        const FitGradSource<false> src{f, stats, 0.0f, nullptr, 0, {}, false};
        if (mb) psi_launch_skin_bwd_v_mb(e->lv.m, e->lv.A, src, f.cam, f.B, e->lv.gl, e->lv.g_vp, e->lv.gt_part_w, st);
        else if (big) PSI_LAUNCH_BWD_V(FitGradSource<false>, PsiBlendPipelined);
        else PSI_LAUNCH_BWD_V(FitGradSource<false>);
    }
#undef PSI_LAUNCH_BWD_V
    PSI_CHECK_LAUNCH("skin_bwd_v_grad_kernel");
    psi_mark("skin_bwd_v_grad_kernel", st);
    int rc = psi_lbs_backward_joint_parts(e->lbs, f.B, e->lbs_ws, f.g_transl, st);
    if (rc) return rc;
    launch_head_bwd<true>(f, e->lv, nullptr, st);
    PSI_CHECK_LAUNCH("head_bwd_adam_kernel");
    psi_mark("head_bwd_adam_kernel", st);
    return 0;
}

static int fit_build_scenes(psi_fit_engine *e, const psi_fit_scene *h_scenes, int S);

static inline size_t fit_x_bytes(const FitDev &f) { return (size_t)f.B * XD * 4; }
static inline size_t fit_cam_bytes(const FitDev &f) { return (size_t)f.B * 16 * 4; }
static inline size_t fit_hint_bytes(const FitDev &f) { return (size_t)f.B * f.n_c * 4; }
static inline hipError_t fit_hints_reset(const FitDev &f, hipStream_t st) { return hipMemsetAsync(f.nn_hint, 0xff, fit_hint_bytes(f), st); }

static inline size_t sdf_cells_bytes(int D) { return (size_t)D * D * D * 32; }
static void sdf_cells_fill(const float *d_sdf, float *d_cells, int D)
{
    hipLaunchKernelGGL(sdf_to_cells_kernel, dim3((unsigned)psi_cdiv((long)(sdf_cells_bytes(D) / 4), 256)), dim3(256), 0, 0, d_sdf, d_cells, D);
}

static int fit_scene_index(psi_nn_index **out, const float *d_verts, int m, hipError_t *err)
{
    std::vector<float> hs((size_t)m * 3);
    *err = hipMemcpy(hs.data(), d_verts, hs.size() * 4, hipMemcpyDeviceToHost);
    return *err == hipSuccess ? psi_nn_index_create(out, hs.data(), m) : (int)*err;
}

static int fit_create(psi_fit_engine **out, const psi_lbs_model *lbs, const psi_fit_config *cfg,
                      const float *h_w1, const float *h_b1, const float *h_w2, const float *h_b2,
                      const float *h_w3, const float *h_b3, const float *h_lh_comp, const float *h_rh_comp,
                      const float *h_pose_mean, const int32_t *h_contact_ids,
                      const float *d_scene_verts, const float *d_sdf, const float *h_gmin, const float *h_gmax,
                      const psi_fit_scene *h_scenes, int S)
{
    PSI_REQUIRE(out && lbs && cfg && h_w1 && h_b1 && h_w2 && h_b2 && h_w3 && h_b3 && h_lh_comp && h_rh_comp && h_pose_mean &&
                h_contact_ids && d_scene_verts && d_sdf && h_gmin && h_gmax, "null pointer");
    int V, J, NB;
    psi_lbs_dims(lbs, &V, &J, &NB);
    PSI_REQUIRE(J == 55 && NB >= 10 && NB <= 32, "the fused engine is SMPL-X shaped (J=55, 10..32 betas)");
    PSI_REQUIRE(cfg->B > 0 && cfg->n_contact > 0 && cfg->n_contact < (1 << 24) && cfg->m_scene > 0 && cfg->D >= 2 && cfg->world_size >= 1, "bad sizes");
    PSI_REQUIRE(cfg->num_pca_comps > 0 && cfg->num_pca_comps <= 12, "1..12 hand PCA components");
    PSI_REQUIRE(!(cfg->independent_bodies && cfg->world_size > 1), "independent bodies have no cross-rank coupling: use world_size 1");
    for (int i = 0; i < 66; i++) PSI_REQUIRE(h_pose_mean[i] == 0.0f, "pose_mean must be zero for global_orient/body joints");
    for (int i = 0; i < cfg->n_contact; i++) PSI_REQUIRE(h_contact_ids[i] >= 0 && h_contact_ids[i] < V, "contact id out of range");
    PsiLbsCounts mc;
    if (int rcv = psi_lbs_counts(lbs, cfg->B, &mc)) return rcv;
    psi_fit_engine *e = new psi_fit_engine();
    std::unique_ptr<psi_fit_engine, void (*)(psi_fit_engine *)> owner(e, psi_fit_destroy);
    const FitKnobs &knobs = e->knobs = fit_read_knobs();
    e->lbs = lbs;
    FitDev &f = e->d;
    f.B = cfg->B; f.V = V; f.J = J; f.NB = NB; f.n_c = cfg->n_contact; f.m = cfg->m_scene; f.D = cfg->D;
    f.align_corners = cfg->align_corners; f.world = cfg->world_size; f.ncomp = cfg->num_pca_comps;
    f.indep = cfg->independent_bodies ? 1 : 0;
    f.w_rec = cfg->w_rec; f.w_vp = cfg->w_vposer; f.w_contact = cfg->w_contact; f.w_col = cfg->w_collision; f.cconst = cfg->contact_const;
    f.lr = cfg->lr; f.beta1 = cfg->beta1; f.beta2 = cfg->beta2; f.eps = cfg->eps;
    f.lr_d = cfg->lr_d != 0.0 ? cfg->lr_d : (double)cfg->lr;
    f.beta1_d = cfg->beta1_d != 0.0 ? cfg->beta1_d : (double)cfg->beta1;
    f.beta2_d = cfg->beta2_d != 0.0 ? cfg->beta2_d : (double)cfg->beta2;
    f.one_m_beta1 = (float)(1.0 - f.beta1_d);
    f.one_m_beta2 = (float)(1.0 - f.beta2_d);
    f.nsdfblk = psi_cdiv(V, 256);
    f.Vpad = f.nsdfblk * 256;
    f.nfp = cfg->nn_mode == 1 ? psi_nn_index_fparts(f.n_c) : psi_nn_contact_fparts(f.n_c);
    f.max_hist = cfg->max_history > 0 ? cfg->max_history : 1024;
    f.ncp = psi_cdiv(f.n_c, 256) * 256;
    f.ncp3 = 3 * f.ncp;
    f.nsv = mc.nsv;
    f.nsv_c = f.ncp / 256;
    f.scene = d_scene_verts;
    f.sdf = d_sdf;
    int dev = 0, cus = 0;
    PSI_CHECK_HIP(hipGetDevice(&dev));
    PSI_CHECK_HIP(hipDeviceGetAttribute(&cus, hipDeviceAttributeMultiprocessorCount, dev));
    const FitModes &mode = e->mode = fit_decide(cfg, knobs, J, f.ncp3, mc, cus);
    f.hc = mode.hc;
    f.gv_sps = mode.gv_sps;
    f.fused_bwd = mode.fused_bwd ? 1 : 0;
    f.pen_skip = mode.fused_bwd && !knobs.no_pen_skip ? 1 : 0;
    f.nsn_m = mode.split.nsn_m; f.nsn_c = mode.split.nsn_c; f.spm = mode.split.spm; f.spc = mode.split.spc;
#ifdef PSI_HEAD_STOPS
    f.stop_h = knobs.head_stop;
    f.stop_t = knobs.tail_stop;
    (void)hipMemcpyToSymbol(HIP_SYMBOL(psi_dbg_sstop), &knobs.skin_stop, sizeof(int));
    (void)hipMemcpyToSymbol(HIP_SYMBOL(psi_dbg_pstop), &f.stop_t, sizeof(int));
    const int cstop = knobs.head_stop == 9;
    (void)hipMemcpyToSymbol(HIP_SYMBOL(psi_dbg_cstop), &cstop, sizeof(int));
#endif
    const size_t B = (size_t)f.B;
    std::vector<float> W1T((size_t)NZ * NH), W2T((size_t)NH * NH), W3T((size_t)NH * 128, 0.0f), b3p(128, 0.0f);
    memcpy(b3p.data(), h_b3, NJ6 * 4);
    for (int o = 0; o < NH; o++) for (int k = 0; k < NZ; k++) W1T[(size_t)k * NH + o] = h_w1[(size_t)o * NZ + k];
    for (int o = 0; o < NH; o++) for (int k = 0; k < NH; k++) W2T[(size_t)k * NH + o] = h_w2[(size_t)o * NH + k];
    for (int o = 0; o < NJ6; o++) for (int k = 0; k < NH; k++) W3T[(size_t)k * 128 + o] = h_w3[(size_t)o * NH + k];
    std::vector<int> cs_ptr(V + 1, 0), cs_idx(f.n_c), cs_first(V, 0);
    for (int i = 0; i < f.n_c; i++) cs_ptr[h_contact_ids[i] + 1]++;
    for (int v = 0; v < V; v++) cs_ptr[v + 1] += cs_ptr[v];
    {
        std::vector<int> fill(cs_ptr.begin(), cs_ptr.end() - 1);
        for (int i = 0; i < f.n_c; i++) cs_idx[fill[h_contact_ids[i]]++] = i;
        for (int v = 0; v < V; v++)
            if (cs_ptr[v + 1] > cs_ptr[v]) cs_first[v] = cs_idx[cs_ptr[v]] | (std::min(cs_ptr[v + 1] - cs_ptr[v], 127) << 24);
    }
    const size_t hand_pca = (size_t)f.ncomp * 45 * 4, hidden = B * NH * 4, betas = B * NB * 4, pose = B * J * 3 * 4, transl = B * 3 * 4,
                 crows = B * f.n_c * 3 * 4, per_body = B * 4, slot_rows = B * f.ncp3 * 4;
    PsiBlob &T = e->table;
    T.upload(f.W1T, W1T.data(), W1T.size() * 4);
    T.upload(f.b1, h_b1, NH * 4);
    T.upload(f.W2T, W2T.data(), W2T.size() * 4);
    T.upload(f.b2, h_b2, NH * 4);
    T.upload(f.W3T, W3T.data(), W3T.size() * 4);
    T.upload(f.b3, b3p.data(), 128 * 4);
    T.upload(f.W1, h_w1, (size_t)NH * NZ * 4);
    T.upload(f.W2, h_w2, (size_t)NH * NH * 4);
    T.upload(f.W3, h_w3, (size_t)NJ6 * NH * 4);
    T.upload(f.lhc, h_lh_comp, hand_pca);
    T.upload(f.rhc, h_rh_comp, hand_pca);
    T.upload(f.pose_mean, h_pose_mean, (size_t)J * 3 * 4);
    T.upload(f.vid, h_contact_ids, (size_t)f.n_c * sizeof(int32_t));
    T.upload(f.cs_ptr, cs_ptr.data(), cs_ptr.size() * sizeof(int));
    T.upload(f.cs_idx, cs_idx.data(), cs_idx.size() * sizeof(int));
    T.upload(f.cs_first, cs_first.data(), cs_first.size() * sizeof(int));
    T.upload(f.gmin, h_gmin, 12);
    T.upload(f.gmax, h_gmax, 12);
    T.zero_begin = T.size;
    T.zero(f.x, fit_x_bytes(f));
    T.zero(f.xhr, fit_x_bytes(f));
    T.zero(f.cam, fit_cam_bytes(f));
    T.zero(f.adam_m, fit_x_bytes(f), "adam_m");
    T.zero(f.adam_v, fit_x_bytes(f), "adam_v");
    T.zero(f.step, 256);
    T.zero(f.h1, hidden);
    T.zero(f.h2, hidden);
    T.zero(f.o6, B * 128 * 4);
    T.zero(f.betas20, betas);
    T.zero(f.pose, pose, "pose");
    T.zero(f.transl, transl);
    T.zero(f.verts, B * V * 3 * 4, "verts");
    T.zero(f.cverts, crows);
    T.zero(f.og, B * f.Vpad * 4 * 4);
    T.zero(f.gq, crows);
    T.zero(f.fpart, B * f.nfp * 4, "fpart");
    T.zero(f.penpart, B * f.nsdfblk * 2 * 4);
    T.zero(f.recpart, per_body);
    T.zero(f.vppart, per_body);
    T.zero(f.g_betas, betas);
    T.zero(f.g_pose, pose, "g_pose");
    T.zero(f.g_transl, transl, "g_transl");
    T.zero(f.g_rot, B * J * 9 * 4, "g_rot");
    T.zero(f.history, (size_t)f.max_hist * 4 * 4);
    T.zero(e->stats_local, 256);
    T.ones(f.nn_hint, fit_hint_bytes(f), "nn_hint");
    T.zero(f.hx_o6, B * f.hc * 128 * 8);
    T.zero(f.hx_gh1, B * f.hc * NH * 8);
    T.zero(f.hx_epoch, 2 * B * 4);
    T.zero(f.Wct, (size_t)f.n_c * PSI_JP * 4);
    if (mode.fused_bwd) {
        T.zero(f.glc, slot_rows, "glc");
        T.zero(f.gvpc, slot_rows, "gvpc");
        T.zero(f.vpc, slot_rows, "vpc");
        T.zero(f.gtc_part, B * f.nfp * 4 * 4, "gtc_part");
        T.zero(f.gvbits, 2 * PSI_GV_SLOTS * 4);
        T.zero(f.WTt_c, (size_t)f.ncp * PSI_JP * 4);
        T.zero(f.dirs_ch, (size_t)f.ncp3 * mc.Kpad * 4);
        T.zero(f.gA_part, (size_t)(f.nsv + f.nsv_c) * B * PSI_JP * 16 * 4);
        T.zero(f.gfeat_part, (size_t)(f.nsn_m + f.nsn_c) * B * mc.Kpad * 4);
        T.zero(f.spb, per_body, "spb");
        T.zero(f.penmask, B * (f.Vpad / 64) * 8, "penmask");
    }
    const bool cells = !h_scenes && psi_sdf_cells_fit(f.D) && !knobs.sdf_linear;
    if (cells) T.zero(f.sdf_cells, sdf_cells_bytes(f.D));
    T.zero(e->lbs_ws, psi_lbs_workspace_floats(lbs, f.B) * 4);
    T.zero(e->nn_ws, psi_nn_ws_bytes(f.B, f.n_c, f.m));
    if (int rc = psi_blob_realise(T, &e->blob, "psi_fit_create")) return rc;
    f.hx_err = f.step + 1;
    if (int rcv = psi_lbs_view(lbs, f.B, e->lbs_ws, &e->lv)) return rcv;
    e->plan = fit_plan_make(f, e->lv.m, knobs.ska_nbody, knobs.bwd_pf1);
    hipLaunchKernelGGL(contact_weight_table_kernel, dim3(psi_cdiv((long)f.n_c * PSI_JP, 256)), dim3(256), 0, 0, e->lv.m.WT, e->lv.m.Vpad, f.vid,
                       f.n_c, J, (float *)f.Wct);
    if (mode.fused_bwd) {
        hipLaunchKernelGGL(contact_weight_tiles_kernel, dim3(psi_cdiv((long)f.ncp * PSI_JP, 256)), dim3(256), 0, 0, f.Wct, f.n_c, f.ncp, (float *)f.WTt_c);
        hipLaunchKernelGGL(contact_dirs_h_kernel, dim3(psi_cdiv((long)f.ncp3 * e->lv.m.Kpad, 256)), dim3(256), 0, 0, e->lv.m.dirs_bh, e->lv.m.Kpad, f.vid,
                           f.n_c, f.ncp3, (float *)f.dirs_ch);
    }
    if (cells) sdf_cells_fill(d_sdf, (float *)f.sdf_cells, f.D);
    e->grid = psi_sdf_grid_make(f.sdf_cells, h_gmin, h_gmax, f.D, f.align_corners);
    hipError_t err = hipDeviceSynchronize();
    if (err == hipSuccess) err = hipGetLastError();
    if (err != hipSuccess) {
        psi_set_error("psi_fit_create: layout kernels failed: %s", hipGetErrorString(err));
        return (int)err;
    }
    if (h_scenes) {
        if (int rc = fit_build_scenes(e, h_scenes, S)) return rc;
    } else if (cfg->nn_mode == 1) {
        if (int rc = fit_scene_index(&e->nn_index, d_scene_verts, f.m, &err)) return rc;
    }
    owner.release();
    *out = e;
    return 0;
}

extern "C" int psi_fit_create(psi_fit_engine **out, const psi_lbs_model *lbs, const psi_fit_config *cfg,
                              const float *h_w1, const float *h_b1, const float *h_w2, const float *h_b2,
                              const float *h_w3, const float *h_b3, const float *h_lh_comp, const float *h_rh_comp,
                              const float *h_pose_mean, const int32_t *h_contact_ids,
                              const float *d_scene_verts, const float *d_sdf, const float *h_gmin, const float *h_gmax)
{
    return fit_create(out, lbs, cfg, h_w1, h_b1, h_w2, h_b2, h_w3, h_b3, h_lh_comp, h_rh_comp, h_pose_mean, h_contact_ids, d_scene_verts, d_sdf,
                      h_gmin, h_gmax, nullptr, 0);
}

static int fit_build_scenes(psi_fit_engine *e, const psi_fit_scene *h_scenes, int S)
{
    FitDev &f = e->d;
    e->n_scenes = S;
    e->scene_index = new psi_nn_index *[S]();
    e->scene_vol = new float *[S]();
    std::vector<psikd::KdDev> kd(S);
    std::vector<PsiSdfGrid> grids(S);
    for (int s = 0; s < S; s++) {
        const psi_fit_scene &sc = h_scenes[s];
        const int D = sc.D;
        const size_t bytes = sdf_cells_bytes(D);
        hipError_t err = hipMalloc((void **)&e->scene_vol[s], bytes);
        if (err != hipSuccess) {
            (void)hipGetLastError();
            e->scene_vol[s] = nullptr;
            psi_set_error("psi_fit_create_scenes: no memory for the copy of scene %d's volume (%zu bytes, 8 x the volume): %s", s, bytes, hipGetErrorString(err));
            return PSI_ENOMEM;
        }
        sdf_cells_fill(sc.d_sdf, e->scene_vol[s], D);
        grids[s] = psi_sdf_grid_make(e->scene_vol[s], sc.gmin, sc.gmax, D, f.align_corners);
        if (int rc = fit_scene_index(&e->scene_index[s], sc.d_verts, sc.m, &err)) {
            if (err != hipSuccess) psi_set_error("psi_fit_create_scenes: reading scene %d's vertices failed: %s", s, hipGetErrorString(err));
            return rc;
        }
        kd[s] = psi_nn_index_dev(e->scene_index[s]);
        e->kd_rows = std::max(e->kd_rows, kd[s].rows);
    }
    e->nn_index = e->scene_index[0];
    PsiBlob T;
    T.upload(e->d_kd_tab, kd.data(), sizeof(psikd::KdDev) * S);
    T.upload(e->d_grid_tab, grids.data(), sizeof(PsiSdfGrid) * S);
    T.zero(e->d_slot, sizeof(int) * (size_t)f.B);
    if (int rc = psi_blob_realise(T, &e->scene_blob, "psi_fit_create_scenes")) return rc;
    hipError_t err = hipDeviceSynchronize();
    if (err == hipSuccess) err = hipGetLastError();
    if (err != hipSuccess) {
        psi_set_error("psi_fit_create_scenes: layout kernels failed: %s", hipGetErrorString(err));
        return (int)err;
    }
    return 0;
}

extern "C" int psi_fit_create_scenes(psi_fit_engine **out, const psi_lbs_model *lbs, const psi_fit_config *cfg,
                                     const float *h_w1, const float *h_b1, const float *h_w2, const float *h_b2,
                                     const float *h_w3, const float *h_b3, const float *h_lh_comp, const float *h_rh_comp,
                                     const float *h_pose_mean, const int32_t *h_contact_ids,
                                     const psi_fit_scene *h_scenes, int S)
{
    PSI_REQUIRE(out, "null pointer");
    *out = nullptr;
    PSI_REQUIRE(cfg, "null pointer");
    PSI_REQUIRE(S >= 1, "psi_fit_create_scenes: S must be at least 1");
    PSI_REQUIRE(h_scenes, "psi_fit_create_scenes: null scene table");
    PSI_REQUIRE(cfg->nn_mode == 1, "psi_fit_create_scenes: nn_mode must be 1 (there is no brute-force search over several scenes)");
    PSI_REQUIRE(cfg->world_size <= 1, "psi_fit_create_scenes: world_size > 1 (data-parallel runs over several scenes) is not supported");
    for (int s = 0; s < S; s++) {
        const psi_fit_scene &sc = h_scenes[s];
        PSI_REQUIRE(sc.d_verts && sc.d_sdf, "psi_fit_create_scenes: null scene pointer");
        PSI_REQUIRE(sc.m > 0, "psi_fit_create_scenes: a scene without vertices");
        if (!psi_sdf_cells_fit(sc.D)) {
            psi_set_error("invalid argument: psi_fit_create_scenes: D = %d of scene %d: D must be a multiple of 4, at least 4 and at most %d (the engine samples "
                          "a cell-major copy of the volume and has no plain-volume fallback)", sc.D, s, PSI_SDF_CELLS_MAX_D);
            return PSI_EINVAL;
        }
    }
    psi_fit_config c = *cfg;
    c.m_scene = h_scenes[0].m;
    c.D = h_scenes[0].D;
    c.world_size = 1;
    return fit_create(out, lbs, &c, h_w1, h_b1, h_w2, h_b2, h_w3, h_b3, h_lh_comp, h_rh_comp, h_pose_mean, h_contact_ids, h_scenes[0].d_verts,
                      h_scenes[0].d_sdf, h_scenes[0].gmin, h_scenes[0].gmax, h_scenes, S);
}

extern "C" int psi_fit_scene_count(const psi_fit_engine *e) { return e ? (e->n_scenes ? e->n_scenes : 1) : 0; }

extern "C" int psi_fit_set_scene_slots(psi_fit_engine *e, const int32_t *d_slot, void *stream)
{
    PSI_REQUIRE(e && d_slot, "null pointer");
    hipStream_t st = (hipStream_t)stream;
    hipStreamCaptureStatus cap = hipStreamCaptureStatusNone;
    PSI_CHECK_HIP(hipStreamIsCapturing(st, &cap));
    PSI_REQUIRE(cap == hipStreamCaptureStatusNone, "psi_fit_set_scene_slots: not inside a stream capture (the captured iterations read the engine's own slot buffer)");
    FitDev &f = e->d;
    if (e->n_scenes) {
        hipLaunchKernelGGL(scene_slots_kernel, dim3(psi_cdiv(f.B, 256)), dim3(256), 0, st, (const int *)d_slot, e->d_slot, f.B, e->n_scenes);
        PSI_CHECK_LAUNCH("scene_slots_kernel");
    }
    PSI_CHECK_HIP(fit_hints_reset(f, st));
    return 0;
}

extern "C" void psi_fit_destroy(psi_fit_engine *e)
{
    if (!e) return;
    if (e->scene_index) {
        for (int s = 0; s < e->n_scenes; s++)
            if (e->scene_index[s]) psi_nn_index_destroy(e->scene_index[s]);
        delete[] e->scene_index;
    } else if (e->nn_index) psi_nn_index_destroy(e->nn_index);
    if (e->scene_vol) {
        for (int s = 0; s < e->n_scenes; s++) (void)hipFree(e->scene_vol[s]);
        delete[] e->scene_vol;
    }
    (void)hipFree(e->scene_blob);
    for (FitGraph &G : e->graphs) fit_graph_drop(&G);
    (void)hipFree(e->blob);
    delete e;
}

extern "C" int psi_fit_set_problem(psi_fit_engine *e, const float *d_xhr, const float *d_x_init, const float *d_cam_ext,
                                   int reset_optimizer, void *stream)
{
    PSI_REQUIRE(e && d_xhr && d_cam_ext, "null pointer");
    FitDev &f = e->d;
    hipStream_t st = (hipStream_t)stream;
    PSI_CHECK_HIP(hipMemcpyAsync(f.xhr, d_xhr, fit_x_bytes(f), hipMemcpyDeviceToDevice, st));
    PSI_CHECK_HIP(hipMemcpyAsync(f.x, d_x_init ? d_x_init : d_xhr, fit_x_bytes(f), hipMemcpyDeviceToDevice, st));
    PSI_CHECK_HIP(hipMemcpyAsync(f.cam, d_cam_ext, fit_cam_bytes(f), hipMemcpyDeviceToDevice, st));
    PSI_CHECK_HIP(fit_hints_reset(f, st));
    if (reset_optimizer) {
        hipLaunchKernelGGL(adam_reset_kernel, dim3(psi_cdiv((long)f.B * XD, 256)), dim3(256), 0, st, f.adam_m, f.adam_v, f.step, f.B * XD);
        PSI_CHECK_LAUNCH("adam_reset_kernel");
    psi_mark("adam_reset_kernel", st);
    }
    return 0;
}

static int fit_iteration(psi_fit_engine *e, hipStream_t st)
{
    int rc = fit_forward(e, e->stats_local, st, FitStats::Backward);
    return rc ? rc : fit_backward(e, e->stats_local, st, FitStats::Backward);
}

static int fit_half(psi_fit_engine *e, int which, float *stats, int use_graph, hipStream_t st)
{
    auto half = [&]() { return which == 0 ? fit_forward(e, stats, st, FitStats::Finalize) : fit_backward(e, stats, st, FitStats::Caller); };
    if (!use_graph) return half();
    FitGraph *G = &e->graphs[FIT_G_HALF_FWD + which];
    if (G->ready && e->half_stats[which] != stats) fit_graph_drop(G);
    if (!G->ready) {
        const FitCaptured c = fit_graph_capture(G, st, half);
        if (c.kind != FitCaptured::Ok) return c.rc;
        e->half_stats[which] = stats;
    }
    return fit_graph_launch(*G, st);
}

extern "C" int psi_fit_forward(psi_fit_engine *e, float *d_stats, int use_graph, void *stream)
{
    PSI_REQUIRE(e, "null engine");
    return fit_half(e, 0, d_stats ? d_stats : e->stats_local, use_graph, (hipStream_t)stream);
}

extern "C" int psi_fit_backward_step(psi_fit_engine *e, const float *d_stats, int use_graph, void *stream)
{
    PSI_REQUIRE(e, "null engine");
    return fit_half(e, 1, (float *)(d_stats ? d_stats : e->stats_local), use_graph, (hipStream_t)stream);
}

extern "C" int psi_fit_iterate(psi_fit_engine *e, int n_iter, int use_graph, void *stream)
{
    PSI_REQUIRE(e && n_iter >= 0, "bad arguments");
    PSI_REQUIRE(e->d.world == 1, "psi_fit_iterate is the single-process path; data-parallel runs call forward / all-reduce / backward_step");
    hipStream_t st = (hipStream_t)stream;
    auto one = [&]() { return fit_iteration(e, st); };
    int done = 0, rc = 0;
    if (!use_graph) {
        for (; done < n_iter && !rc; done++) rc = one();
        return rc;
    }
    return fit_run_graphs(st, n_iter, &done,
                          {{2 * GRAPH_UNROLL, &e->graphs[FIT_G_ITER_2N]}, {GRAPH_UNROLL, &e->graphs[FIT_G_ITER_N]}, {1, &e->graphs[FIT_G_ITER_1]}}, one).rc;
}

extern "C" int psi_fit_iterate_dp(psi_fit_engine *e, psi_dp_comm *comm, int n_iter, int use_graph, float *d_stats, void *stream)
{
    PSI_REQUIRE(e && comm && n_iter >= 0, "bad arguments");
    PSI_REQUIRE(psi_dp_world(comm) == e->d.world, "the communicator's size differs from psi_fit_config.world_size");
    hipStream_t st = (hipStream_t)stream;
    float *stats = d_stats ? d_stats : e->stats_local;
    auto one = [&]() -> int {
        if (e->mode.fused_bwd) {
            int rc = fit_forward(e, stats, st, FitStats::Backward);
            if (!rc) rc = fit_backward_joint(e, stats, st, FitStats::Backward);
            if (!rc) rc = psi_dp_allreduce_sum(comm, stats, 6, st);
            return rc ? rc : fit_backward_tail(e, stats, st);
        }
        int rc = fit_forward(e, stats, st, FitStats::Finalize);
        if (!rc) rc = psi_dp_allreduce_sum(comm, stats, 6, st);
        if (!rc) rc = fit_backward(e, stats, st, FitStats::Finalize);
        return rc;
    };
    if (e->dp_comm != comm || e->dp_stats != stats) {
        fit_graph_drop(&e->graphs[FIT_G_DP_1]);
        fit_graph_drop(&e->graphs[FIT_G_DP_N]);
        e->dp_warm = e->dp_warm && e->dp_comm == comm;
        e->dp_comm = comm;
        e->dp_stats = stats;
    }
    int done = 0;
    auto eager = [&](int upto) {
        int rc = 0;
        for (; done < upto && !rc; done++) rc = one();
        return rc;
    };
    if (!use_graph || (!e->dp_warm && n_iter > 0)) {
        if (int rc = eager(use_graph ? 1 : n_iter)) return rc;
        e->dp_warm = true;
        if (!use_graph) return 0;
    }
    if (!e->dp_no_graph) {
        const FitCaptured c = fit_run_graphs(st, n_iter, &done, {{GRAPH_UNROLL, &e->graphs[FIT_G_DP_N]}, {1, &e->graphs[FIT_G_DP_1]}}, one);
        if (c.kind != FitCaptured::Refused) return c.rc;
        (void)hipGetLastError();
        e->dp_no_graph = true;
    }
    return eager(n_iter);
}

extern "C" int psi_fit_chain_mode(const psi_fit_engine *e)
{
    return e && e->mode.chain.n_links_wg > 0 && e->d.hc > 1 ? 1 : 0;
}

extern "C" int psi_fit_dp_mode(const psi_fit_engine *e)
{
    if (!e || !e->dp_warm) return 0;
    return e->dp_no_graph ? 2 : 1;
}

extern "C" int psi_fit_decode_forward(psi_fit_engine *e, const float *d_x75, const float *d_cam_ext, float *d_verts, void *stream)
{
    PSI_REQUIRE(e && d_x75 && d_cam_ext && d_verts, "null pointer");
    FitDev &f = e->d;
    hipStream_t st = (hipStream_t)stream;
    PSI_CHECK_HIP(hipMemcpyAsync(f.x, d_x75, fit_x_bytes(f), hipMemcpyDeviceToDevice, st));
    PSI_CHECK_HIP(hipMemcpyAsync(f.cam, d_cam_ext, fit_cam_bytes(f), hipMemcpyDeviceToDevice, st));
    int rc = fit_head_blend(e, st);
    if (rc) return rc;
    hipLaunchKernelGGL(psi_skin_fwd_kernel<PsiSkinNoEpilogue>, dim3(f.nsdfblk, f.B), dim3(PSI_SKIN_BLK), 0, st, e->lv.m, e->lv.A,
                       e->lv.v_posed, f.transl, f.cam, f.B, d_verts, PsiSkinNoEpilogue());
    PSI_CHECK_LAUNCH("skin_fwd_kernel");
    return 0;
}

extern "C" int psi_fit_decode_backward(psi_fit_engine *e, const float *d_grad_verts, float *d_grad_x75, void *stream)
{
    PSI_REQUIRE(e && d_grad_verts && d_grad_x75, "null pointer");
    FitDev &f = e->d;
    hipStream_t st = (hipStream_t)stream;
    if (f.B >= PSI_SKIN_MB_MIN_B)
        psi_launch_skin_bwd_v_mb(e->lv.m, e->lv.A, PsiGradFromMemory{d_grad_verts, f.V}, f.cam, f.B, e->lv.gl, e->lv.g_vp, e->lv.gt_part_w, st);
    else
        hipLaunchKernelGGL(psi_skin_bwd_v_kernel<PsiGradFromMemory>, dim3(f.nsdfblk, f.B), dim3(PSI_SKIN_BLK), 0, st, e->lv.m, e->lv.A,
                           PsiGradFromMemory{d_grad_verts, f.V}, f.cam, f.B, e->lv.gl, e->lv.g_vp, e->lv.gt_part_w);
    PSI_CHECK_LAUNCH("skin_bwd_v_kernel");
    int rc = psi_lbs_backward_joint_parts(e->lbs, f.B, e->lbs_ws, f.g_transl, st);
    if (rc) return rc;
    launch_head_bwd<false>(f, e->lv, d_grad_x75, st);
    PSI_CHECK_LAUNCH("head_bwd_kernel");
    return 0;
}

extern "C" int psi_fit_profile(psi_fit_engine *e, int n_rep, char *h_names, int name_stride, float *h_ms, int max_stages,
                               int *h_n_stages, void *stream)
{
    PSI_REQUIRE(e && h_names && h_ms && h_n_stages && n_rep > 0 && max_stages > 0 && name_stride >= 16, "bad arguments");
    PSI_REQUIRE(e->d.world == 1, "profile the single-process path");
    hipStream_t st = (hipStream_t)stream;
    PsiStageTimer tm;
    memset(&tm, 0, sizeof(tm));
    for (int i = 0; i < 48; i++) PSI_CHECK_HIP(hipEventCreate(&tm.ev[i]));
    std::vector<double> acc(48, 0.0);
    int n_st = 0, rc = 0;
    for (int r = 0; r < n_rep && !rc; r++) {
        tm.n = 0;
        (void)hipEventRecord(tm.ev[0], st);
        tm.name[0] = "start";
        tm.n = 1;
        g_psi_timer = &tm;
        rc = fit_iteration(e, st);
        g_psi_timer = nullptr;
        if (rc) break;
        PSI_CHECK_HIP(hipStreamSynchronize(st));
        n_st = tm.n - 1;
        for (int i = 1; i < tm.n; i++) {
            float ms = 0;
            (void)hipEventElapsedTime(&ms, tm.ev[i - 1], tm.ev[i]);
            acc[i - 1] += ms;
        }
    }
    for (int i = 0; i < 48; i++) (void)hipEventDestroy(tm.ev[i]);
    if (rc) return rc;
    if (n_st > max_stages) n_st = max_stages;
    for (int i = 0; i < n_st; i++) {
        h_ms[i] = (float)(acc[i] / n_rep);
        strncpy(h_names + (size_t)i * name_stride, tm.name[i + 1], name_stride - 1);
        h_names[(size_t)i * name_stride + name_stride - 1] = 0;
    }
    *h_n_stages = n_st;
    return 0;
}

extern "C" int psi_fit_read(psi_fit_engine *e, float *d_x_out, float *d_history_out, int n_hist, int *h_step, void *stream)
{
    PSI_REQUIRE(e, "null engine");
    FitDev &f = e->d;
    hipStream_t st = (hipStream_t)stream;
    if (d_x_out) PSI_CHECK_HIP(hipMemcpyAsync(d_x_out, f.x, fit_x_bytes(f), hipMemcpyDeviceToDevice, st));
    if (d_history_out && n_hist > 0) {
        if (n_hist > f.max_hist) n_hist = f.max_hist;
        PSI_CHECK_HIP(hipMemcpyAsync(d_history_out, f.history, (size_t)n_hist * 16, hipMemcpyDeviceToDevice, st));
    }
    if (h_step) {
        int hs[2] = {0, 0};
        PSI_CHECK_HIP(hipMemcpyAsync(hs, f.step, 8, hipMemcpyDeviceToHost, st));
        PSI_CHECK_HIP(hipStreamSynchronize(st));
        *h_step = hs[0];
        if (hs[1]) {
            (void)hipMemsetAsync(f.hx_err, 0, 4, st);
            psi_set_error("psi_fit_read: a head / tail cluster exchange timed out (a producer workgroup never published its partials); "
                          "the results of this fit are invalid.  PSI_HEAD_CLUSTER=1 runs the kernels without clusters");
            return 902;
        }
    }
    return 0;
}

extern "C" int psi_fit_read_losses(psi_fit_engine *e, int adam_step, float *d_out4, void *stream)
{
    PSI_REQUIRE(e && d_out4 && adam_step >= 1, "bad arguments");
    FitDev &f = e->d;
    PSI_CHECK_HIP(hipMemcpyAsync(d_out4, f.history + (size_t)((adam_step - 1) % f.max_hist) * 4, 16, hipMemcpyDeviceToDevice, (hipStream_t)stream));
    return 0;
}

extern "C" int psi_fit_copy_buffer(psi_fit_engine *e, const char *name, float *d_out, long n_floats, void *stream)
{
    PSI_REQUIRE(e && name && d_out && n_floats >= 0, "bad arguments");
    FitDev &f = e->d;
    const PsiLbsView &lv = e->lv;
    const float *src = nullptr;
    long cap = 0;
    if (const PsiBuf *b = e->table.find(name)) { src = (const float *)(e->blob + b->off); cap = (long)(b->bytes / 4); }
    const struct { const char *name; const float *src; long cap; } more[] = {
        {"stats", e->stats_local, 8},
        {"gA", lv.gA, (long)f.B * PSI_JP * 16},
        {"gfeat", lv.gfeat, (long)f.B * lv.m.Kpad},
        {"gl", lv.gl, (long)f.B * lv.m.Npad},
        {"g_vp", lv.g_vp, (long)f.B * lv.m.Npad},
        {"v_posed", lv.v_posed, (long)f.B * lv.m.Npad},
        {"R", lv.R, (long)f.B * lv.m.J * 12},
        {"G", lv.G, (long)f.B * lv.m.J * 12},
        {"A", lv.A, (long)f.B * lv.m.J * 12 + PSI_A_TAIL * 12},
        {"feat", lv.feat, (long)((f.B + 31) & ~31) * lv.m.Kpad},
    };
    for (const auto &b : more)
        if (!strcmp(name, b.name)) { src = b.src; cap = b.cap; }
    if (!strcmp(name, "verts") && e->nn_index) {
        hipLaunchKernelGGL(psi_skin_fwd_kernel<PsiSkinNoEpilogue>, dim3(f.nsdfblk, f.B), dim3(PSI_SKIN_BLK), 0, (hipStream_t)stream, lv.m, lv.A,
                           lv.v_posed, f.transl, f.cam, f.B, f.verts, PsiSkinNoEpilogue());
        PSI_CHECK_LAUNCH("skin_fwd_kernel");
    }
    PSI_REQUIRE(src != nullptr, "unknown buffer name");
    PSI_REQUIRE(n_floats <= cap, "buffer is smaller than requested");
    PSI_CHECK_HIP(hipMemcpyAsync(d_out, src, (size_t)n_floats * 4, hipMemcpyDeviceToDevice, (hipStream_t)stream));
    return 0;
}
```

psi-release_amd/csrc/nnindex.hip:

```cpp
#include "psi_internal.h"
#include "blob.h"
#include "nnindex_device.h"
#include <algorithm>
#include <math.h>
#include <stdlib.h>
#include <string.h>
#include <cmath>
#include <limits>
#include <vector>

#pragma clang fp contract(off)

namespace {

using namespace psikd;

template <int LPQ, bool CONTACT, bool MULTI = false>
__global__ __launch_bounds__(QBLK) void kd_query_kernel(KdDev T0, const float *__restrict__ xyz1, const int *__restrict__ qidx,
                                                        long qstride, int n, float *__restrict__ dist, int *__restrict__ idx,
                                                        float cconst, float gscale, float *__restrict__ gq, float *__restrict__ fpart,
                                                        int *__restrict__ hint, int rows, const KdDev *__restrict__ tab = nullptr,
                                                        const int *__restrict__ slot = nullptr)
{
    extern __shared__ int smem_i[];
    kd_query_body<LPQ, CONTACT, MULTI>(T0, KdQueryFromMemory{xyz1, qidx, qstride}, n, dist, idx, cconst, gscale, gq, fpart, hint, rows, tab, slot,
                                  (int)blockIdx.x, (int)blockIdx.y, (int)gridDim.x, smem_i);
}

static int kd_lanes_from_env()
{
    const char *v = getenv("PSI_NN_SEARCH_LANES");
    return v && v[0] == '2' && v[1] == 0 && kd_qpb(LPQ_OPS) == kd_qpb(2) ? 2 : LPQ_OPS;
}
#define PSI_KD_LAUNCH(lanes, CONTACT, MULTI, ...)                                                          \
    do {                                                                                                   \
        if ((lanes) == 2) hipLaunchKernelGGL((kd_query_kernel<2, CONTACT, MULTI>), __VA_ARGS__);           \
        else hipLaunchKernelGGL((kd_query_kernel<LPQ_OPS, CONTACT, MULTI>), __VA_ARGS__);                  \
    } while (0)

struct Builder {
    const float *p;
    std::vector<int> order;
    std::vector<KdNode> nodes;
    std::vector<std::pair<int, int>> leaves;
    int depth_max = 0;

    void bounds(int lo, int hi, float *mn, float *mx)
    {
        for (int c = 0; c < 3; c++) { mn[c] = INFINITY; mx[c] = -INFINITY; }
        for (int i = lo; i < hi; i++)
            for (int c = 0; c < 3; c++) {
                float v = p[(size_t)order[i] * 3 + c];
                mn[c] = std::min(mn[c], v);
                mx[c] = std::max(mx[c], v);
            }
    }

    int median_split(int lo, int hi)
    {
        float mn[3], mx[3];
        bounds(lo, hi, mn, mx);
        int ax = 0;
        if (mx[1] - mn[1] > mx[ax] - mn[ax]) ax = 1;
        if (mx[2] - mn[2] > mx[ax] - mn[ax]) ax = 2;
        int mid = (lo + hi) / 2;
        const float *pp = p;
        std::nth_element(order.begin() + lo, order.begin() + mid, order.begin() + hi, [pp, ax](int u, int v) {
            float a = pp[(size_t)u * 3 + ax], b = pp[(size_t)v * 3 + ax];
            return a < b || (a == b && u < v);
        });
        return mid;
    }

    int build(int lo, int hi, int depth)
    {
        if (depth > depth_max) depth_max = depth;
        if (hi - lo <= LEAF) {
            leaves.push_back({lo, hi - lo});
            return -((int)leaves.size() - 1) - 1;
        }
        std::vector<std::pair<int, int>> rg = {{lo, hi}};
        for (int round = 0; round < 3; round++) {
            std::vector<std::pair<int, int>> nx;
            for (auto &r : rg) {
                if (r.second - r.first > LEAF) {
                    int mid = median_split(r.first, r.second);
                    nx.push_back({r.first, mid});
                    nx.push_back({mid, r.second});
                } else {
                    nx.push_back(r);
                }
            }
            rg.swap(nx);
        }
        int me = (int)nodes.size();
        nodes.push_back(KdNode());
        KdNode nd;
        memset(&nd, 0, sizeof(nd));
        for (int c = 0; c < WIDE; c++) {
            nd.c[c].ref = EMPTY;
            for (int a = 0; a < 3; a++) { nd.c[c].mn[a] = INFINITY; nd.c[c].mx[a] = -INFINITY; }
        }
        for (size_t c = 0; c < rg.size(); c++) {
            float mn[3], mx[3];
            bounds(rg[c].first, rg[c].second, mn, mx);
            for (int a = 0; a < 3; a++) { nd.c[c].mn[a] = mn[a]; nd.c[c].mx[a] = mx[a]; }
            nd.c[c].ref = build(rg[c].first, rg[c].second, depth + 1);
        }
        nodes[me] = nd;
        return me;
    }
};

}

struct psi_nn_index {
    KdDev d;
    char *blob;
    int lanes;
};

extern "C" int psi_nn_index_create(psi_nn_index **out, const float *h_points, int m)
{
    PSI_REQUIRE(out && h_points && m > 0 && m < (1 << 24), "bad arguments (0 < m < 2^24)");
    Builder bd;
    bd.p = h_points;
    bd.order.resize(m);
    for (int i = 0; i < m; i++) bd.order[i] = i;
    bd.nodes.reserve((size_t)2 * (m / LEAF + 2));
    int root = bd.build(0, m, 0);
    const int rows = 7 * (bd.depth_max + 1) + 2;
    PSI_REQUIRE(rows <= MAXSTACK, "tree too deep for the traversal stack");
    auto rec = [&](int oi) {
        float4 r;
        r.x = h_points[(size_t)oi * 3 + 0];
        r.y = h_points[(size_t)oi * 3 + 1];
        r.z = h_points[(size_t)oi * 3 + 2];
        memcpy(&r.w, &oi, 4);
        return r;
    };
    std::vector<float4> pts(bd.leaves.size() * LEAF), opts(m);
    for (size_t L = 0; L < bd.leaves.size(); L++)
        for (int k = 0; k < LEAF; k++) {
            int kk = k < bd.leaves[L].second ? k : bd.leaves[L].second - 1;
            pts[L * LEAF + k] = rec(bd.order[bd.leaves[L].first + kk]);
        }
    for (int i = 0; i < m; i++) opts[i] = rec(i);
    if (bd.nodes.empty()) bd.nodes.push_back(KdNode());
    float gmn[3], gmx[3];
    bd.bounds(0, m, gmn, gmx);
    float ext[3], emax = 0.0f;
    for (int a = 0; a < 3; a++) { ext[a] = gmx[a] - gmn[a]; emax = std::max(emax, ext[a]); }
    int gn[3] = {1, 1, 1};
    float ginv = 1.0f;
    const bool use_grid = emax > 0.0f && std::isfinite(emax) && !(getenv("PSI_NN_GRID") && getenv("PSI_NN_GRID")[0] == '0');
    std::vector<int> cell_start(2, 0);
    std::vector<float4> gpts;
    if (use_grid) {
        double vol = 1.0;
        for (int a = 0; a < 3; a++) vol *= std::max((double)ext[a], 1e-3 * emax);
        double h = std::cbrt(vol * 2.5 / m);
        h = std::max(h, (double)emax / 128.0);
        ginv = (float)(1.0 / h);
        for (int a = 0; a < 3; a++) gn[a] = std::min(128, std::max(1, (int)std::floor(ext[a] * ginv) + 1));
        const size_t ncell = (size_t)gn[0] * gn[1] * gn[2];
        auto cell_of = [&](int i) {
            int cc[3];
            for (int a = 0; a < 3; a++) {
                const float u = (h_points[(size_t)i * 3 + a] - gmn[a]) * ginv;
                cc[a] = std::min(std::max((int)std::floor(u), 0), gn[a] - 1);
            }
            return ((size_t)cc[0] * gn[1] + cc[1]) * gn[2] + cc[2];
        };
        std::vector<size_t> cid(m);
        for (int i = 0; i < m; i++) cid[i] = cell_of(i);
        std::vector<int> ord(m);
        for (int i = 0; i < m; i++) ord[i] = i;
        auto okey = [](float f) { f += 0.0f; unsigned u; memcpy(&u, &f, 4); return (u & 0x80000000u) ? ~u : (u | 0x80000000u); };
// ... 160 lines not shown
```

psi-release_amd/csrc/nnindex_device.h:

```cpp
#pragma once
#include <hip/hip_runtime.h>
#include <math.h>
#include "psi_common.h"
#include "search_sum_order.h"

#ifndef PSI_SSTOP
#define PSI_SSTOP(k)
#endif
#ifdef PSI_HEAD_STOPS
__device__ int psi_kd_stat[4 * 8192];
__device__ int psi_kd_reason[8];
__device__ unsigned long long psi_kd_mark[4 * 8192];
#define PSI_KD_STAT(what) what
#define PSI_KD_MARK(k) do { __builtin_amdgcn_sched_barrier(0); if (threadIdx.x == 0 && blockIdx.x < 8192 && psi_dbg_sstop >= 9) psi_kd_mark[4 * blockIdx.x + (k)] = wall_clock64(); __builtin_amdgcn_sched_barrier(0); } while (0)
#else
#define PSI_KD_STAT(what)
#define PSI_KD_MARK(k)
#endif

namespace psikd {

constexpr int LEAF = 8;
constexpr int WIDE = 8;
constexpr int MAXSTACK = 72;
constexpr int QBLK = 256;
#ifndef PSI_KD_LPQ
#define PSI_KD_LPQ 4
#endif
constexpr int LPQ_OPS = PSI_KD_LPQ;
static_assert(LPQ_OPS == 4 || LPQ_OPS == 8, "PSI_KD_LPQ: 4 or 8 (2 lanes are chosen at run time)");
constexpr int kd_cpl(int lpq) { return WIDE / lpq; }
constexpr int kd_qpb(int lpq) { return psi_sum_slice_queries(lpq); }
constexpr int kd_threads(int lpq) { return kd_qpb(lpq) * lpq; }
static_assert(kd_qpb(4) == QBLK / 4 && kd_qpb(8) == QBLK / 8 && kd_qpb(2) == 64 && kd_threads(2) == 128, "workgroup shapes");
constexpr int EMPTY = (int)0x80000000;

struct KdChild {
    float mn[3], mx[3];
    int ref;
    int pad;
};
struct KdNode {
    KdChild c[WIDE];
};
static_assert(sizeof(KdNode) == 256, "node record is 256 bytes");

struct KdDev {
    const KdNode *nodes;
    const float4 *pts;
    const float4 *opts;
    int root;
    int m;
    int rows;
    const int *cell_start;
    const float4 *gpts;
    float gorg[3], ginv;
    int gn[3];
};

constexpr int GRID_COLS_PER_LANE = 3;
#ifndef PSI_KD_GRID_COLS_2LANE
#define PSI_KD_GRID_COLS_2LANE 3
#endif
constexpr int kd_rpl(int lpq) { return lpq == 2 ? PSI_KD_GRID_COLS_2LANE : GRID_COLS_PER_LANE; }
#ifndef PSI_KD_GRID_LIST_MAX
#define PSI_KD_GRID_LIST_MAX 48
#endif
constexpr int GRID_LIST_MAX = PSI_KD_GRID_LIST_MAX;
#ifndef PSI_KD_GRID_PAIRS
#define PSI_KD_GRID_PAIRS 4
#endif
constexpr int GRID_PAIRS = PSI_KD_GRID_PAIRS;
#ifndef PSI_KD_GRID_MAX_CAND
#define PSI_KD_GRID_MAX_CAND 64
#endif
constexpr int GRID_MAX_CAND = PSI_KD_GRID_MAX_CAND;

template <int CTRL>
__device__ __forceinline__ float dpp_f(float v) { return __int_as_float(__builtin_amdgcn_update_dpp(0, __float_as_int(v), CTRL, 0xf, 0xf, false)); }
template <int CTRL>
__device__ __forceinline__ int dpp_i(int v) { return __builtin_amdgcn_update_dpp(0, v, CTRL, 0xf, 0xf, false); }
constexpr int DPP_XOR1 = 0xB1;
constexpr int DPP_XOR2 = 0x4E;
constexpr int DPP_HALF_MIRROR = 0x141;

typedef unsigned long long kd_key;
__device__ __forceinline__ kd_key kd_pack(float d, int i) { return ((kd_key)(unsigned)__float_as_int(d) << 32) | (unsigned)i; }
__device__ __forceinline__ float kd_key_d(kd_key k) { return __int_as_float((int)(k >> 32)); }
__device__ __forceinline__ int kd_key_i(kd_key k) { return (int)(unsigned)k; }

template <int LPQ>
__device__ __forceinline__ kd_key group_min(kd_key k)
{
#define PSI_STEP(CTRL)                                                                              \
    {                                                                                               \
        kd_key k2 = ((kd_key)(unsigned)dpp_i<CTRL>((int)(k >> 32)) << 32) | (unsigned)dpp_i<CTRL>((int)(unsigned)k); \
        k = k2 < k ? k2 : k;                                                                        \
    }
    static_assert(LPQ == 2 || LPQ == 4 || LPQ == 8, "lanes per query");
    PSI_STEP(DPP_XOR1)
    if (LPQ >= 4) PSI_STEP(DPP_XOR2)
    if (LPQ == 8) PSI_STEP(DPP_HALF_MIRROR)
#undef PSI_STEP
    return k;
}

struct KdQueryFromMemory {
    const float *xyz1;
    const int *qidx;
    long qstride;
    __device__ __forceinline__ void issue(int, int, bool) {}
    __device__ __forceinline__ void fetch(int) {}
    __device__ __forceinline__ void prepare(int) {}
    __device__ __forceinline__ void point(int b, int j, int, float &qx, float &qy, float &qz) const
    {
        const size_t qrow = qidx ? (size_t)qidx[j] : (size_t)j;
        const float *qp = xyz1 + (size_t)b * qstride + qrow * 3;
        qx = qp[0]; qy = qp[1]; qz = qp[2];
    }
    __device__ __forceinline__ void contact_post(size_t, float, float, float) {}
    __device__ __forceinline__ void contact_finish(int, int, int) {}
};

template <int LPQ>
__device__ __forceinline__ void kd_block_fsum(float fval, float *__restrict__ out)
{
    __shared__ float wsum[psi_sum_parts(LPQ)];
    const int tid = threadIdx.x;
    float v = fval;
#pragma unroll
    for (int o2 = psi_sum_part_lanes(LPQ) / 2; o2 > 0; o2 >>= 1) v += __shfl_down(v, o2, 64);
#pragma unroll
    for (int p = 0; p < psi_sum_parts_per_wave(LPQ); p++)
        if ((tid & 63) == psi_sum_first_lane(LPQ, p)) wsum[(int)psi_sum_slot(LPQ, tid >> 6, p)] = v;
    __syncthreads();
    if (tid == 0) {
        float t = 0.0f;
#pragma unroll
        for (int w = 0; w < psi_sum_parts(LPQ); w++) t += wsum[w];
        *out = t;
    }
}

__device__ __forceinline__ int kd_warm_hint(const int *__restrict__ hint, bool active, size_t o) { return (active && hint) ? hint[o] : -1; }
__device__ __forceinline__ int kd_warm_candidate(const KdDev &T, int h, float4 &hp)
{
    hp = make_float4(0.0f, 0.0f, 0.0f, 0.0f);
    if (h < 0 || h >= T.m) return -1;
    hp = T.opts[h];
    return h;
}

template <class T>
__device__ __forceinline__ T &kd_slot(T *tab, size_t obase, int jq, int K, int k)
{
    return *(T *)((char *)(tab + obase * K + k) + (unsigned)jq * (unsigned)(4 * K));
}

template <int LPQ, int RPL, bool CONTACT, class QSrc>
__device__ __forceinline__ float kd_query_round(const KdDev &T, QSrc &qsrc, float qx, float qy, float qz, bool active, size_t o, float *__restrict__ dist,
                                                int *__restrict__ idx, float cconst, float gscale, float *__restrict__ gq, int *__restrict__ hint,
                                                int rows, int *smem_i, int h, const float4 &hp, size_t obase, int jq)
{
#pragma clang fp contract(off)
    constexpr int CPL = kd_cpl(LPQ);
    const int tid = threadIdx.x;
    const int c = tid & (LPQ - 1);
    const int g = tid / LPQ;
    int *stk_n = smem_i + (size_t)g * rows * 2;
    float *stk_d = (float *)(stk_n + rows);
    kd_key bestk = kd_pack(INFINITY, 0x7fffffff);
    float best = INFINITY;
    if (h >= 0) {
        float x2 = hp.x - qx, y2 = hp.y - qy, z2 = hp.z - qz;
        best = PSI_SQ3(x2, y2, z2);
        bestk = kd_pack(best, h);
    }
    int sp = 0;
    int cur = T.root;
    float curd = 0.0f;
    bool have = active;
    PSI_KD_STAT(int nvis = 0; int ngp = 0;)
#ifndef PSI_KD_SEED_CELLS
#define PSI_KD_SEED_CELLS 1.5f
#endif
    if (have && T.cell_start && !(best * T.ginv * T.ginv <= PSI_KD_SEED_CELLS * PSI_KD_SEED_CELLS)) {
        const float fx = fminf(fmaxf(floorf((qx - T.gorg[0]) * T.ginv), 0.0f), (float)(T.gn[0] - 1));
        const float fy = fminf(fmaxf(floorf((qy - T.gorg[1]) * T.ginv), 0.0f), (float)(T.gn[1] - 1));
        const float fz = fminf(fmaxf(floorf((qz - T.gorg[2]) * T.ginv), 0.0f), (float)(T.gn[2] - 1));
        const int cz0 = max((int)fz - 1, 0), cz1 = min((int)fz + 1, T.gn[2] - 1);
        const unsigned cbase = (unsigned)((int)fx * T.gn[1] + (int)fy) * (unsigned)T.gn[2];
        const int p0 = T.cell_start[cbase + cz0], p1 = T.cell_start[cbase + cz1 + 1];
        if (p1 > p0) {
            const float4 *rp = (const float4 *)((const char *)T.gpts + ((unsigned)((p0 + p1) >> 2) << 5));
            const float4 a = rp[0], b = rp[1];
            const float xa = a.x - qx, ya = a.z - qy, za = b.x - qz, xb = a.y - qx, yb = a.w - qy, zb = b.y - qz;
            const float da = PSI_SQ3(xa, ya, za), db = PSI_SQ3(xb, yb, zb);
            const kd_key ka = kd_pack(da, __float_as_int(b.z)), kb = kd_pack(db, __float_as_int(b.w));
            if (da == da && ka < bestk) bestk = ka;
            if (db == db && kb < bestk) bestk = kb;
            best = kd_key_d(bestk);
        }
    }
    const int gshift = (tid & 63) & ~(LPQ - 1);
    if (have && T.cell_start && best < INFINITY) {
        const float ru = __builtin_amdgcn_sqrtf(best) * T.ginv * 1.0001f + 0.01f;
        const float uq[3] = {(qx - T.gorg[0]) * T.ginv, (qy - T.gorg[1]) * T.ginv, (qz - T.gorg[2]) * T.ginv};
        const float topx = (float)(T.gn[0] - 1), topy = (float)(T.gn[1] - 1), topz = (float)(T.gn[2] - 1);
        const float ru2 = ru * ru;
        const float ox = fmaxf(fmaxf(-uq[0], uq[0] - topx - 1.0f), 0.0f), oy = fmaxf(fmaxf(-uq[1], uq[1] - topy - 1.0f), 0.0f),
                    oz = fmaxf(fmaxf(-uq[2], uq[2] - topz - 1.0f), 0.0f);
        const float oz2 = oz * oz;
        const float rx = __builtin_amdgcn_sqrtf(fmaxf(ru2 - oy * oy - oz2, 0.0f)), ry = __builtin_amdgcn_sqrtf(fmaxf(ru2 - ox * ox - oz2, 0.0f));
        const float flx = fminf(fmaxf(floorf(uq[0] - rx), 0.0f), topx), fhx = fminf(fmaxf(floorf(uq[0] + rx), 0.0f), topx);
        const float fly = fminf(fmaxf(floorf(uq[1] - ry), 0.0f), topy), fhy = fminf(fmaxf(floorf(uq[1] + ry), 0.0f), topy);
        const float fny = fhy - fly + 1.0f, fncand = (fhx - flx + 1.0f) * fny;
        if (fncand <= (float)GRID_MAX_CAND) {
            const int ncand = (int)fncand;
            const float rny = __builtin_amdgcn_rcpf(fny);
            const int list_max = min(GRID_LIST_MAX, 2 * rows);
            int nsurv = 0;
            for (int c0 = 0; c0 < ncand; c0 += LPQ) {
                const float fcol = (float)(c0 + c);
                const float fcx = floorf((fcol + 0.5f) * rny);
                const float cxf = flx + fcx, cyf = fly + (fcol - fcx * fny);
                const float dx = fmaxf(fmaxf(cxf - uq[0], uq[0] - cxf - 1.0f), 0.0f), dy = fmaxf(fmaxf(cyf - uq[1], uq[1] - cyf - 1.0f), 0.0f);
                const float h2 = ru2 - dx * dx - dy * dy;
                const bool ok = c0 + c < ncand && h2 >= oz2;
                const float hz = __builtin_amdgcn_sqrtf(fmaxf(h2, 0.0f));
                const int zlo = (int)fminf(fmaxf(floorf(uq[2] - hz), 0.0f), topz), zhi = (int)fminf(fmaxf(floorf(uq[2] + hz), 0.0f), topz);
                const unsigned gm = (unsigned)(__ballot(ok) >> gshift) & ((1u << LPQ) - 1u);
                const int pos = nsurv + __popc(gm & ((1u << c) - 1u));
                if (ok && pos < list_max) stk_n[pos] = (((int)cxf * T.gn[1] + (int)cyf) << 14) | (zlo << 7) | zhi;
                nsurv += __popc(gm);
            }
            if (nsurv <= list_max && nsurv > 0) {
              typedef float v2f __attribute__((ext_vector_type(2)));
              const v2f qxx = {qx, qx}, qyy = {qy, qy}, qzz = {qz, qz};
              float bd = INFINITY;
              int bi = 0x7fffffff;
              bool tie = false;
              for (int s0 = 0; s0 < nsurv; s0 += RPL * LPQ) {
                int ps[RPL], nr[RPL];
                int cs[RPL], ce[RPL];
                const char *csb = (const char *)T.cell_start;
#pragma unroll
                for (int u = 0; u < RPL; u++) {
                    const int e = stk_n[s0 + c + u * LPQ < nsurv ? s0 + c + u * LPQ : 0];
                    const unsigned base = (unsigned)(e >> 14) * (unsigned)T.gn[2];
                    cs[u] = *(const int *)(csb + ((base + ((unsigned)e >> 7 & 127u)) << 2));
                    ce[u] = *(const int *)(csb + ((base + ((unsigned)e & 127u) + 1u) << 2));
                }
                int rounds = 0;
                PSI_KD_MARK(1);
#pragma unroll
                for (int u = 0; u < RPL; u++) {
                    ps[u] = cs[u] >> 1;
                    nr[u] = (ce[u] > cs[u] && s0 + c + u * LPQ < nsurv) ? (((ce[u] + 1) >> 1) - ps[u] + GRID_PAIRS - 1) / GRID_PAIRS : 0;
                    rounds += nr[u];
                }
                static_assert(RPL >= 2, "the round -> pair mapping below takes at least two runs");
                int upto[RPL - 1], off[RPL];
                upto[0] = nr[0];
                off[0] = ps[0];
#pragma unroll
                for (int u = 1; u < RPL; u++) {
                    off[u] = ps[u] - GRID_PAIRS * upto[u - 1];
                    if (u < RPL - 1) upto[u] = upto[u - 1] + nr[u];
                }
                for (int t = 0; t < rounds; t++) {
                    PSI_KD_STAT(ngp += 1;)
                    int offt = off[RPL - 1];
#pragma unroll
                    for (int u = RPL - 2; u >= 0; u--) offt = t < upto[u] ? off[u] : offt;
                    const int pr = GRID_PAIRS * t + offt;
                    const float4 *rp = (const float4 *)((const char *)T.gpts + ((unsigned)pr << 5));
                    float4 a[GRID_PAIRS], b[GRID_PAIRS];
#pragma unroll
                    for (int k = 0; k < GRID_PAIRS; k++) { a[k] = rp[2 * k]; b[k] = rp[2 * k + 1]; }
#pragma unroll
                    for (int k = 0; k < GRID_PAIRS; k++) {
                        const v2f x2 = (v2f){a[k].x, a[k].y} - qxx, y2 = (v2f){a[k].z, a[k].w} - qyy, z2 = (v2f){b[k].x, b[k].y} - qzz;
#ifdef PSI_CHAMFER_FMA
                        const v2f d = __builtin_elementwise_fma(z2, z2, __builtin_elementwise_fma(y2, y2, x2 * x2));
#else
                        const v2f d = x2 * x2 + y2 * y2 + z2 * z2;
#endif
                        const int i2[2] = {__float_as_int(b[k].z), __float_as_int(b[k].w)};
#pragma unroll
                        for (int e = 0; e < 2; e++) {
                            const bool lt = d[e] < bd;
                            tie = tie || d[e] == bd;
                            bi = lt ? i2[e] : bi;
                            bd = lt ? d[e] : bd;
                        }
                    }
                }
              }
                kd_key k = group_min<LPQ>(kd_pack(bd, bi));
                PSI_KD_MARK(2);
                bestk = k < bestk ? k : bestk;
                best = kd_key_d(bestk);
                have = ((__ballot(tie) >> gshift) & ((1ull << LPQ) - 1ull)) != 0;
                PSI_KD_STAT(if (have && c == 0 && psi_dbg_sstop == 10) atomicAdd(psi_kd_reason + 2, 1);)
            } else { PSI_KD_STAT(if (c == 0 && psi_dbg_sstop == 10) { atomicAdd(psi_kd_reason + 1, 1); atomicMax(psi_kd_reason + 5, nsurv); }) }
        } else { PSI_KD_STAT(if (c == 0 && psi_dbg_sstop == 10) { atomicAdd(psi_kd_reason + 0, 1); atomicMax(psi_kd_reason + 4, (int)fminf(fncand, 1e6f)); }) }
    } else { PSI_KD_STAT(if (have && c == 0 && psi_dbg_sstop == 10) atomicAdd(psi_kd_reason + 3, 1);) }
    while (true) {
        while (!have && sp > 0) {
            --sp;
            cur = stk_n[sp];
            curd = stk_d[sp];
            have = !(curd * 0.999999f > best);
        }
        if (!have) break;
        PSI_KD_STAT(nvis += 1;)
        if (cur >= 0) {
            float dc[CPL];
            int ref[CPL];
            kd_key km = ~0ull;
#pragma unroll
            for (int u = 0; u < CPL; u++) {
                const float4 *cp = (const float4 *)(T.nodes + cur) + 2 * (c + u * LPQ);
                const float4 lo = cp[0], hi = cp[1];
                float dx = fmaxf(fmaxf(lo.x - qx, qx - lo.w), 0.0f);
                float dy = fmaxf(fmaxf(lo.y - qy, qy - hi.x), 0.0f);
                float dz = fmaxf(fmaxf(lo.z - qz, qz - hi.y), 0.0f);
                dc[u] = dx * dx + dy * dy + dz * dz;
                ref[u] = __float_as_int(hi.z);
                const kd_key k = kd_pack(dc[u], c + u * LPQ);
                km = k < km ? k : km;
                if (CPL > 2 && u == CPL / 2 - 1) __builtin_amdgcn_sched_barrier(0);
            }
            km = group_min<LPQ>(km);
            const float dmin = kd_key_d(km);
            const int cmin = kd_key_i(km);
#pragma unroll
            for (int u = 0; u < CPL; u++) {
                const bool push = (c + u * LPQ) != cmin && dc[u] * 0.999999f <= best;
                const unsigned gm = (unsigned)(__ballot(push) >> gshift) & ((1u << LPQ) - 1u);
                if (push) {
                    const int pos = sp + __popc(gm & ((1u << c) - 1u));
                    stk_n[pos] = ref[u];
                    stk_d[pos] = dc[u];
                }
                sp += __popc(gm);
            }
            int rsel = ref[0];
#pragma unroll
            for (int u = 1; u < CPL; u++) rsel = (cmin / LPQ == u) ? ref[u] : rsel;
            cur = __shfl(rsel, (tid & 63 & ~(LPQ - 1)) | (cmin & (LPQ - 1)), 64);
            curd = dmin;
            have = dmin < INFINITY && !(dmin * 0.999999f > best);
        }
        if (have && cur < 0) {
            kd_key k = ~0ull;
#pragma unroll
            for (int u = 0; u < CPL; u++) {
                const float4 p = T.pts[(size_t)(-cur - 1) * LEAF + c + u * LPQ];
                float x2 = p.x - qx, y2 = p.y - qy, z2 = p.z - qz;
                const float d = PSI_SQ3(x2, y2, z2);
                const kd_key ku = kd_pack(d, __float_as_int(p.w));
                k = ku < k ? ku : k;
            }
            k = group_min<LPQ>(k);
            bestk = k < bestk ? k : bestk;
            best = kd_key_d(bestk);
            have = false;
        }
    }
    PSI_KD_STAT(if (blockIdx.x < 8192 && psi_dbg_sstop == 10) {
        int *st_ = psi_kd_stat + 4 * blockIdx.x;
        if (c == 0 && nvis > 0) { atomicAdd(st_ + 0, 1); atomicAdd(st_ + 2, nvis); }
        atomicMax(st_ + 1, nvis);
        atomicMax(st_ + 3, ngp);
    })
    float fval = 0.0f;
    PSI_KD_MARK(3);
    if (active && c == 0) {
        const int besti = kd_key_i(bestk);
        if constexpr (LPQ == 2) {
            if (dist) kd_slot(dist, obase, jq, 1, 0) = best;
            if (idx) kd_slot(idx, obase, jq, 1, 0) = besti;
            if (hint) kd_slot(hint, obase, jq, 1, 0) = besti;
        } else {
            if (dist) dist[o] = best;
            if (idx) idx[o] = besti;
            if (hint) hint[o] = besti;
        }
        if (CONTACT) {
            float4 w = hp;
            if (besti != h) w = T.opts[besti];
            float sq = sqrtf(best + 1e-4f);
            float den = sq + cconst;
            fval = sq / den;
            float gg = gscale * (cconst / (2.0f * sq * den * den)) * 2.0f;
            const float gx = gg * (qx - w.x), gy = gg * (qy - w.y), gz = gg * (qz - w.z);
            if (LPQ == 2 && gq) {
                kd_slot(gq, obase, jq, 3, 0) = gx;
                kd_slot(gq, obase, jq, 3, 1) = gy;
                kd_slot(gq, obase, jq, 3, 2) = gz;
            } else if (gq) {
                gq[o * 3 + 0] = gx;
                gq[o * 3 + 1] = gy;
                gq[o * 3 + 2] = gz;
            }
            qsrc.contact_post(o, gx, gy, gz);
        }
    }
    return fval;
}

template <int LPQ, bool CONTACT, bool MULTI, class QSrc>
__device__ __forceinline__ void kd_query_body(KdDev T0, QSrc qsrc, int n, float *__restrict__ dist, int *__restrict__ idx, float cconst,
                                              float gscale, float *__restrict__ gq, float *__restrict__ fpart, int *__restrict__ hint,
                                              int rows, const KdDev *__restrict__ tab, const int *__restrict__ slot, int bx, int b, int nbx,
                                              int *smem_i)
{
    constexpr int QPB = kd_qpb(LPQ);
    const int tid = threadIdx.x;
    if (kd_threads(LPQ) < QBLK && tid >= kd_threads(LPQ)) return;
    const int c = tid & (LPQ - 1), g = tid / LPQ;
    const KdDev T = MULTI ? tab[slot[b]] : T0;
    const int j = bx * QPB + g;
    const bool active = j < n;
    const size_t o = (size_t)b * n + (active ? j : 0);
    float qx = 0, qy = 0, qz = 0;
    float4 hp;
    qsrc.issue(b, active ? j : 0, active);
    const size_t obase = (size_t)b * n;
    const int jq = active ? j : 0;
    const int h0 = LPQ == 2 ? ((active && hint) ? kd_slot(hint, obase, jq, 1, 0) : -1) : kd_warm_hint(hint, active, o);
    qsrc.fetch(b);
    const int h = kd_warm_candidate(T, h0, hp);
    qsrc.prepare(b);
    qsrc.point(b, active ? j : 0, c, qx, qy, qz);
    PSI_SSTOP(4);
    PSI_KD_MARK(0);
    const float fval = kd_query_round<LPQ, kd_rpl(LPQ), CONTACT>(T, qsrc, qx, qy, qz, active, o, dist, idx, cconst, gscale, gq, hint, rows, smem_i, h, hp, obase, jq);
    if (CONTACT) {
        kd_block_fsum<LPQ>(fval, fpart + (size_t)b * nbx + bx);
        qsrc.contact_finish(b, bx, nbx);
    }
}

static inline size_t kd_lds_bytes(int lpq, int rows) { return (size_t)kd_qpb(lpq) * rows * 8; }

}

struct psi_nn_index;
psikd::KdDev psi_nn_index_dev(const psi_nn_index *ix);
int psi_nn_index_contact_set(const psikd::KdDev *tab, const int *slot, int rows, const float *verts, long vstride, const int *vid, int B, int n,
                             float cconst, float gscale, float *gq, float *fpart, int *hint, hipStream_t st);
```

psi-release_amd/csrc/search_sum_order.h:

```cpp
#pragma once

#if defined(__HIPCC__) || defined(__CUDACC__)
#define PSI_SUM_HD __host__ __device__
#else
#define PSI_SUM_HD
#endif

PSI_SUM_HD constexpr int psi_sum_part_queries(int lpq) { return lpq == 8 ? 8 : 16; }
PSI_SUM_HD constexpr int psi_sum_part_lanes(int lpq) { return psi_sum_part_queries(lpq) * lpq; }
PSI_SUM_HD constexpr int psi_sum_parts_per_wave(int lpq) { return 64 / psi_sum_part_lanes(lpq); }
PSI_SUM_HD constexpr int psi_sum_parts(int lpq) { return 4; }
PSI_SUM_HD constexpr int psi_sum_slice_queries(int lpq) { return psi_sum_parts(lpq) * psi_sum_part_queries(lpq); }
PSI_SUM_HD constexpr int psi_sum_waves(int lpq) { return psi_sum_parts(lpq) / psi_sum_parts_per_wave(lpq); }
PSI_SUM_HD constexpr unsigned psi_sum_slot(int lpq, unsigned w, int p) { return w * (unsigned)psi_sum_parts_per_wave(lpq) + (unsigned)p; }
PSI_SUM_HD constexpr int psi_sum_first_lane(int lpq, int p) { return p * psi_sum_part_lanes(lpq); }
PSI_SUM_HD constexpr int psi_sum_last_lane(int lpq, int p) { return (p + 1) * psi_sum_part_lanes(lpq) - 1; }
PSI_SUM_HD inline float psi_sum_slots(const float *slot, int stride, int lpq)
{
    float t = 0.0f;
    for (int s = 0; s < psi_sum_parts(lpq); s++) t += slot[s * stride];
    return t;
}
```

psi-release_amd/hip.py:

```python
from __future__ import annotations

import ctypes
import os

import torch

_PKG = os.path.dirname(os.path.abspath(__file__))
LIB_PATH = os.environ.get('PSI_HIP_LIB') or os.path.join(
    _PKG, 'lib', 'libpsi_hip_fma.so' if os.environ.get('PSI_CHAMFER_FMA') == '1' else 'libpsi_hip.so')
_lib = None

c_void_p, c_int, c_long, c_size_t, c_float, c_double = ctypes.c_void_p, ctypes.c_int, ctypes.c_long, ctypes.c_size_t, ctypes.c_float, ctypes.c_double

SIGNATURES = {
    'psi_last_error': (ctypes.c_char_p, []),
    'psi_version': (c_int, []),
    'psi_device_info': (c_int, [c_void_p] * 4),
    'psi_chamfer_arith_mode': (c_int, []),
    'psi_chamfer_workspace_bytes': (c_size_t, [c_int] * 3),
    'psi_chamfer_forward': (c_int, [c_void_p, c_void_p, c_int, c_int, c_int, c_void_p, c_void_p, c_void_p, c_void_p,
                                    c_void_p, c_void_p]),
    'psi_chamfer_backward': (c_int, [c_void_p] * 8 + [c_int] * 3 + [c_void_p]),
    'psi_scratch_release': (c_int, [c_void_p, c_int]),
    'psi_nn_index_create': (c_int, [c_void_p, c_void_p, c_int]),
    'psi_nn_index_destroy': (None, [c_void_p]),
    'psi_nn_index_query': (c_int, [c_void_p, c_void_p, c_int, c_int, c_void_p, c_void_p, c_void_p, c_void_p]),
    'psi_nn_index_set_create': (c_int, [c_void_p, c_void_p, c_int]),
    'psi_nn_index_set_destroy': (None, [c_void_p]),
    'psi_nn_index_set_query': (c_int, [c_void_p, c_void_p, c_void_p, c_int, c_int, c_void_p, c_void_p, c_void_p]),
    'psi_sdf_sample_forward': (c_int, [c_void_p] * 5 + [c_int] * 5 + [c_void_p] * 3),
    'psi_sdf_sample_backward': (c_int, [c_void_p, c_void_p, c_int, c_int, c_void_p, c_void_p]),
    'psi_sdf_penetration_stats': (c_int, [c_void_p, c_long, c_void_p, c_void_p]),
    'psi_lbs_create': (c_int, [c_void_p] * 7 + [c_int] * 3),
    'psi_lbs_destroy': (None, [c_void_p]),
    'psi_lbs_workspace_floats': (c_size_t, [c_void_p, c_int]),
    'psi_lbs_forward': (c_int, [c_void_p] * 5 + [c_int] + [c_void_p] * 4),
    'psi_lbs_backward': (c_int, [c_void_p] * 5 + [c_int] + [c_void_p] * 5),
    'psi_linear_workspace_floats': (c_size_t, [c_int] * 3),
    'psi_linear_forward': (c_int, [c_void_p, c_int, c_void_p, c_void_p, c_void_p, c_int, c_int, c_int, c_int, c_float, c_void_p, c_void_p, c_void_p,
                                   c_void_p]),
    'psi_linear_forward3': (c_int, [c_void_p, c_int, c_void_p, c_void_p, c_void_p, c_int, c_int, c_int, c_int, c_float, c_void_p, c_void_p, c_void_p,
                                    c_void_p]),
    'psi_linear_backward_workspace_floats': (c_size_t, [c_int, c_int, c_int]),
    'psi_linear_backward': (c_int, [c_void_p, c_void_p, c_void_p, c_int, c_void_p, c_int, c_int, c_int, c_float, c_void_p, c_void_p, c_void_p,
                                    c_void_p, c_void_p]),
    'psi_linear_backward3': (c_int, [c_void_p, c_void_p, c_void_p, c_void_p, c_int, c_int, c_int, c_float, c_void_p, c_void_p, c_void_p, c_void_p, c_void_p]),
    'psi_adam_step': (c_int, [c_void_p] * 5 + [c_int, c_void_p, c_void_p] + [c_double] * 5 + [c_void_p]),
    'psi_fit_create': (c_int, [c_void_p] * 17),
    'psi_fit_destroy': (None, [c_void_p]),
    'psi_fit_create_scenes': (c_int, [c_void_p] * 14 + [c_int]),
    'psi_fit_set_scene_slots': (c_int, [c_void_p, c_void_p, c_void_p]),
    'psi_fit_scene_count': (c_int, [c_void_p]),
    'psi_fit_set_problem': (c_int, [c_void_p] * 4 + [c_int, c_void_p]),
    'psi_fit_forward': (c_int, [c_void_p, c_void_p, c_int, c_void_p]),
    'psi_fit_backward_step': (c_int, [c_void_p, c_void_p, c_int, c_void_p]),
    'psi_fit_iterate': (c_int, [c_void_p, c_int, c_int, c_void_p]),
    'psi_bn_workspace_floats': (c_size_t, [c_long, c_int]),
    'psi_bn_forward': (c_int, [c_void_p] * 7 + [c_long, c_int, c_int, c_float, c_float] + [c_void_p] * 5),
    'psi_bn_backward': (c_int, [c_void_p] * 6 + [c_long, c_int, c_int] + [c_void_p] * 6),
    'psi_bn_forward_t': (c_int, [c_void_p, c_int] + [c_void_p] * 6 + [c_long, c_int, c_int, c_float, c_float] + [c_void_p] * 4 + [c_int, c_void_p]),
    'psi_bn_backward_t': (c_int, [c_void_p, c_int] + [c_void_p] * 6 + [c_long, c_int, c_int] + [c_void_p] * 6),
    'psi_maxpool3x3s2_forward_t': (c_int, [c_void_p, c_int, c_int, c_int, c_int, c_int, c_void_p, c_void_p, c_void_p]),
    'psi_maxpool3x3s2_backward_t': (c_int, [c_void_p, c_int, c_void_p, c_int, c_int, c_int, c_int, c_void_p, c_void_p]),
    'psi_conv2d_supported': (c_int, [c_int] * 6),
    'psi_conv2d_forward': (c_int, [c_void_p, c_int, c_void_p, c_void_p] + [c_int] * 9 + [c_void_p, c_int, c_int, c_void_p]),
    'psi_conv2d_input_grad': (c_int, [c_void_p, c_int, c_void_p] + [c_int] * 9 + [c_void_p, c_int, c_int, c_void_p]),
    'psi_conv2d_prepared_ok': (c_int, [c_int] * 6),
    'psi_conv2d_prepare_weight': (c_int, [c_void_p] + [c_int] * 5 + [c_void_p, c_void_p, c_void_p]),
    'psi_conv2d_forward_p': (c_int, [c_void_p, c_int, c_void_p, c_void_p] + [c_int] * 9 + [c_void_p, c_int, c_int, c_void_p]),
    'psi_conv2d_input_grad_p': (c_int, [c_void_p, c_int, c_void_p] + [c_int] * 9 + [c_void_p, c_int, c_int, c_void_p]),
    'psi_conv2d_wgrad_workspace_floats': (c_size_t, [c_int] * 9),
    'psi_conv2d_weight_grad': (c_int, [c_void_p, c_int, c_void_p, c_int] + [c_int] * 9 + [c_void_p, c_void_p, c_int, c_void_p]),
    'psi_conv3x3_supported': (c_int, [c_int] * 4),
    'psi_conv3x3_forward': (c_int, [c_void_p, c_void_p, c_void_p, c_int, c_int, c_int, c_int, c_int, c_void_p, c_void_p]),
    'psi_conv3x3_wrw_workspace_floats': (c_size_t, [c_int] * 5),
    'psi_conv3x3_weight_grad': (c_int, [c_void_p, c_void_p, c_int, c_int, c_int, c_int, c_int, c_void_p, c_void_p, c_void_p]),
    'psi_conv3x3_rotate_weight': (c_int, [c_void_p, c_int, c_int, c_void_p, c_void_p]),
    'psi_conv3x3_prepare_weight': (c_int, [c_void_p, c_int, c_int, c_void_p, c_void_p, c_void_p]),
    'psi_maxpool3x3s2_forward': (c_int, [c_void_p, c_int, c_int, c_int, c_int, c_void_p, c_void_p, c_void_p]),
    'psi_maxpool3x3s2_backward': (c_int, [c_void_p, c_void_p, c_int, c_int, c_int, c_int, c_void_p, c_void_p]),
    'psi_cvae_target': (c_int, [c_void_p, c_void_p, c_void_p, c_int, c_void_p, c_void_p]),
    'psi_cvae_losses_workspace_floats': (c_size_t, []),
    'psi_cvae_losses_forward': (c_int, [c_void_p] * 7 + [c_int, c_void_p, c_void_p, c_int, c_int, c_float, c_float, c_float, c_float,
                                        c_void_p, c_void_p, c_void_p, c_void_p, c_void_p]),
    'psi_cvae_losses_backward': (c_int, [c_void_p] * 7 + [c_int, c_void_p, c_void_p, c_int, c_int, c_float, c_float, c_float, c_float,
                                         c_void_p, c_void_p, c_void_p, c_void_p, c_void_p, c_void_p, c_void_p, c_void_p, c_void_p, c_void_p]),
    'psi_scene_losses_workspace_floats': (c_size_t, []),
    'psi_scene_losses_forward': (c_int, [c_void_p, c_long, c_void_p, c_long, c_float, c_float, c_float, c_void_p, c_void_p, c_void_p, c_void_p]),
    'psi_scene_losses_backward': (c_int, [c_void_p] * 7 + [c_long, c_void_p, c_void_p, c_void_p, c_int, c_int, c_int, c_float, c_float, c_float,
                                          c_void_p, c_void_p, c_void_p]),
    'psi_contact_slot_chain': (c_int, [c_void_p, c_int, c_void_p, c_void_p]),
    'psi_fit_dp_mode': (c_int, [c_void_p]),
    'psi_fit_chain_mode': (c_int, [c_void_p]),
    'psi_stream_wait': (c_int, [c_void_p, c_int]),
    'psi_dp_unique_id': (c_int, [c_void_p]),
    'psi_dp_comm_create': (c_int, [c_void_p, c_void_p, c_int, c_int]),
    'psi_dp_comm_destroy': (None, [c_void_p]),
    'psi_dp_comm_info': (c_int, [c_void_p, c_void_p, c_void_p, c_void_p]),
    'psi_dp_allreduce_sum': (c_int, [c_void_p, c_void_p, c_int, c_void_p]),
    'psi_fit_iterate_dp': (c_int, [c_void_p, c_void_p, c_int, c_int, c_void_p, c_void_p]),
    'psi_fit_read': (c_int, [c_void_p, c_void_p, c_void_p, c_int, c_void_p, c_void_p]),
    'psi_fit_read_losses': (c_int, [c_void_p, c_int, c_void_p, c_void_p]),
    'psi_fit_decode_forward': (c_int, [c_void_p, c_void_p, c_void_p, c_void_p, c_void_p]),
    'psi_fit_decode_backward': (c_int, [c_void_p, c_void_p, c_void_p, c_void_p]),
    'psi_fit_profile': (c_int, [c_void_p, c_int, c_void_p, c_int, c_void_p, c_int, c_void_p, c_void_p]),
    'psi_fit_copy_buffer': (c_int, [c_void_p, ctypes.c_char_p, c_void_p, c_long, c_void_p]),
    'psi_lbs_sdf_counts': (c_int, [c_void_p] * 5 + [c_int] + [c_void_p] * 4 + [c_int] * 3 + [c_void_p] * 3),
    'psi_kmeans_create': (c_int, [c_void_p, c_void_p, c_int, c_int, c_void_p, c_int, c_int, c_float]),
    'psi_kmeans_destroy': (None, [c_void_p]),
    'psi_kmeans_iterate': (c_int, [c_void_p, c_int, c_void_p]),
    'psi_kmeans_read': (c_int, [c_void_p] * 7),
    'psi_vq': (c_int, [c_void_p, c_int, c_int, c_void_p, c_int, c_void_p, c_void_p, c_void_p]),
    'psi_raster_mesh_create': (c_int, [c_void_p] * 4 + [c_int, c_int]),
    'psi_raster_mesh_destroy': (None, [c_void_p]),
    'psi_raster_workspace_bytes': (c_size_t, [c_int] * 4),
    'psi_raster_render': (c_int, [c_void_p] * 3 + [c_int, c_int, c_int, c_float] + [c_void_p] * 6),
    'psi_raster_bodies_create': (c_int, [c_void_p] * 2 + [c_int, c_int]),
    'psi_raster_bodies_destroy': (None, [c_void_p]),
    'psi_raster_bodies_normals': (c_int, [c_void_p] * 2 + [c_int] + [c_void_p] * 2),
    'psi_raster_bodies_workspace_bytes': (c_size_t, [c_int] * 5),
    'psi_raster_bodies_render': (c_int, [c_void_p] * 4 + [c_int] + [c_void_p] * 3 + [c_int] + [c_void_p] * 2 + [c_int] * 3 + [c_float] + [c_void_p] * 2
                                 + [c_float] * 3 + [c_int] + [c_void_p] * 9),
    'psi_mesh_sdf_create': (c_int, [c_void_p] * 3 + [c_int, c_int]),
    'psi_mesh_sdf_destroy': (None, [c_void_p]),
    'psi_mesh_sdf_info': (c_int, [c_void_p, c_void_p]),
    'psi_mesh_sdf_compute': (c_int, [c_void_p] * 3 + [c_int, c_int, c_void_p, c_void_p]),
    'psi_mesh_sdf_count_pairs': (c_int, [c_void_p] * 3 + [c_int, c_int, c_void_p, c_void_p]),
    'psi_mesh_winding_compute': (c_int, [c_void_p] * 3 + [c_int, c_float, c_int, c_void_p, c_void_p]),
    'psi_mesh_winding_count': (c_int, [c_void_p] * 3 + [c_int, c_float, c_int, c_void_p, c_void_p]),
    'psi_mesh_sdf_apply_sign': (c_int, [c_void_p, c_float, c_void_p, ctypes.c_longlong, c_void_p]),
    'psi_snapshot_canvas_workspace_bytes': (c_size_t, [c_int]),
    'psi_snapshot_canvas': (c_int, [c_void_p] * 2 + [c_int] * 5 + [c_float] * 2 + [c_void_p] * 9),
    'psi_mesh_cloud_count': (c_int, [c_void_p] * 2 + [c_int] * 2 + [c_float] + [c_void_p] * 5),
    'psi_mesh_cloud_rows': (c_int, [c_void_p] * 2 + [c_int] * 2 + [c_float, c_void_p, ctypes.c_longlong] + [c_void_p] * 3),
    'psi_mesh_cloud_emit': (c_int, [c_void_p] * 2 + [c_int] * 2 + [c_float] + [c_void_p] * 4 + [ctypes.c_longlong] * 2 + [c_void_p] * 5),
    'psi_mesh_cloud_winners': (c_int, [c_void_p] * 3 + [ctypes.c_longlong] + [c_void_p] * 2),
    'psi_mesh_cloud_compact': (c_int, [c_void_p] * 4 + [ctypes.c_longlong] * 2 + [c_void_p] * 3),
    'psi_flood_fill': (c_int, [c_void_p] + [c_int] * 3 + [c_void_p, c_int] + [c_void_p] * 3),
    'psi_mesh_orient_votes': (c_int, [c_void_p] * 2 + [ctypes.c_longlong, c_void_p, c_int, c_void_p, c_int] + [c_void_p] * 3 + [c_int, c_float]
                              + [c_void_p] * 2),
    'psi_body_overlap_create': (c_int, [c_void_p] * 2 + [c_int] * 2),
    'psi_body_overlap_destroy': (None, [c_void_p]),
    'psi_body_overlap_info': (c_int, [c_void_p] * 2),
    'psi_body_overlap_workspace_bytes': (c_size_t, [ctypes.c_longlong, c_int]),
    'psi_body_overlap_boxes': (c_int, [c_void_p] * 2 + [c_int] + [c_void_p] * 3),
    'psi_body_overlap_count': (c_int, [c_void_p] * 3 + [c_int] + [c_void_p] * 3),
    'psi_body_overlap_emit': (c_int, [c_void_p] * 3 + [c_int] + [c_void_p] * 4 + [ctypes.c_longlong] * 2 + [c_void_p] * 3),
    'psi_body_overlap_wind': (c_int, [c_void_p] * 2 + [c_int, c_void_p, ctypes.c_longlong, c_void_p, ctypes.c_longlong, c_void_p, c_size_t, c_void_p]),
    'psi_body_overlap_decide': (c_int, [c_void_p, c_int, c_void_p, ctypes.c_longlong, c_void_p, c_size_t] + [c_void_p] * 4),
    'psi_body_depth_workspace_bytes': (c_size_t, [ctypes.c_longlong, c_int]),
    'psi_body_depth_nearest': (c_int, [c_void_p] * 2 + [c_int, c_void_p, ctypes.c_longlong, c_void_p, ctypes.c_longlong, c_void_p, c_size_t, c_void_p]),
    'psi_body_depth_finish': (c_int, [c_void_p] * 2 + [c_int, c_void_p, ctypes.c_longlong, c_void_p, c_size_t] + [c_void_p] * 6),
    'psi_body_depth_pairs': (c_int, [c_void_p, c_int, c_void_p, ctypes.c_longlong] + [c_void_p] * 8),
    'psi_body_depth_grad_rows': (c_int, [c_void_p, c_int, c_void_p, ctypes.c_longlong] + [c_void_p] * 5 + [c_int] + [c_void_p] * 3),
    'psi_segment_sum3': (c_int, [c_void_p] * 3 + [ctypes.c_longlong, c_void_p, ctypes.c_longlong, c_void_p]),
    'psi_surface_crossings_face_order': (c_int, [c_void_p, c_int, c_int, c_void_p, c_void_p]),
    'psi_surface_crossings_create': (c_int, [c_void_p] * 2 + [c_int] * 2 + [c_void_p] * 3 + [c_int]),
    'psi_surface_crossings_destroy': (None, [c_void_p]),
    'psi_surface_crossings_info': (c_int, [c_void_p] * 2),
    'psi_surface_crossings_boxes': (c_int, [c_void_p] * 2 + [c_int] + [c_void_p] * 4),
    'psi_surface_crossings_tiles': (c_int, [c_void_p] * 2 + [c_int] * 2 + [c_void_p] * 4 + [ctypes.c_longlong] + [c_void_p] * 2),
    'psi_surface_crossings_test': (c_int, [c_void_p] * 2 + [c_int, c_void_p, ctypes.c_longlong] + [c_void_p] * 2 + [ctypes.c_longlong]
                                   + [c_void_p] * 4),
    'psi_surface_crossings_finish': (c_int, [c_void_p, c_int] + [c_void_p] * 4 + [ctypes.c_longlong] + [c_void_p] * 9),
    'psi_crossing_field_eval': (c_int, [c_void_p] * 2 + [c_int, c_void_p, ctypes.c_longlong, c_float] + [c_void_p] * 3),
    'psi_crossing_field_pairs': (c_int, [c_void_p, c_int, c_void_p, ctypes.c_longlong] + [c_void_p] * 7),
    'psi_crossing_field_grad_rows': (c_int, [c_void_p] * 2 + [c_int, c_void_p, ctypes.c_longlong, c_float] + [c_void_p] * 4),
    'psi_body_separate_pose': (c_int, [c_void_p] * 4 + [c_int] * 2 + [c_void_p] * 2),
    'psi_body_separate_wrench': (c_int, [c_void_p] * 3 + [c_int] * 2 + [c_void_p] * 3),
    'psi_body_separate_step': (c_int, [c_void_p, c_int] + [c_void_p] * 6 + [c_int] + [c_float] * 7 + [c_void_p]),
    'psi_body_separate_scene': (c_int, [c_void_p] * 6 + [c_int] * 4 + [c_float] + [c_void_p] * 6),
    'psi_scene_crossings_create': (c_int, [c_void_p] * 2 + [c_int, c_void_p, c_int]),
    'psi_scene_crossings_destroy': (None, [c_void_p]),
    'psi_scene_crossings_info': (c_int, [c_void_p] * 2),
    'psi_scene_crossings_tiles': (c_int, [c_void_p] * 2 + [c_int] * 2 + [c_void_p] * 4 + [ctypes.c_longlong] + [c_void_p] * 2),
    'psi_scene_crossings_test': (c_int, [c_void_p] * 3 + [c_int, c_void_p, ctypes.c_longlong] + [c_void_p] * 2 + [ctypes.c_longlong]
                                 + [c_void_p] * 4),
    'psi_scene_crossings_finish': (c_int, [c_void_p] * 2 + [c_int] + [c_void_p] * 4 + [ctypes.c_longlong] + [c_void_p] * 10),
}


class FitConfig(ctypes.Structure):
    _fields_ = [('B', c_int), ('n_contact', c_int), ('m_scene', c_int), ('D', c_int), ('align_corners', c_int),
                ('world_size', c_int), ('num_pca_comps', c_int), ('max_history', c_int), ('nn_mode', c_int),
                ('w_rec', c_float), ('w_vposer', c_float), ('w_contact', c_float), ('w_collision', c_float),
                ('contact_const', c_float), ('lr', c_float), ('beta1', c_float), ('beta2', c_float), ('eps', c_float),
                ('independent_bodies', c_int), ('concurrent_engines', c_int),
                ('lr_d', ctypes.c_double), ('beta1_d', ctypes.c_double), ('beta2_d', ctypes.c_double)]


class FitScene(ctypes.Structure):
    _fields_ = [('d_verts', c_void_p), ('d_sdf', c_void_p), ('m', c_int), ('D', c_int),
                ('gmin', c_float * 3), ('gmax', c_float * 3)]


class PsiHipError(RuntimeError):
    pass


def lib():
    global _lib
    if _lib is None:
        if not os.path.exists(LIB_PATH):
            raise PsiHipError('libpsi_hip.so not found at %s — run `python -m psi_release_amd.build` '
                              '(there is no CPU fallback)' % LIB_PATH)
        l = ctypes.CDLL(LIB_PATH)
        for name, (res, args) in SIGNATURES.items():
            if os.environ.get('PSI_HIP_LIB') and not hasattr(l, name):
                continue
            fn = getattr(l, name)
            fn.restype = res
            fn.argtypes = args
        _lib = l
    return _lib


def last_error() -> str:
    return lib().psi_last_error().decode()


def check(rc: int, what: str):
    if rc != 0:
        raise PsiHipError('%s failed (code %d): %s' % (what, rc, lib().psi_last_error().decode()))


def ptr(t):
    if t is None:
        return None
    if not t.is_cuda:
        raise PsiHipError('expected a GPU tensor (the HIP kernels are the only implementation)')
    if not t.is_contiguous():
        raise PsiHipError('expected a contiguous tensor')
    return t.data_ptr()


class Handle(ctypes.c_void_p):

    def __init__(self, destroy):
        super().__init__()
        self.destroy, self.V, self.F, self.n_chunks = destroy, 0, 0, 0

    def close(self):
        if self.value:
            try:
                if self.destroy:
                    getattr(lib(), self.destroy)(self)
            finally:
                self.value = None

    def __del__(self):
        try:
            self.close()
        except Exception:
            pass


def stream():
    return torch.cuda.current_stream().cuda_stream

# ... 7 lines not shown
```

Before: 11700.

## Pack two kd-search slices per workgroup with global traversal stacks

In the merged scene-contact search kernel with the 2-lane search, each 256-thread workgroup now serves two query slices instead of one, halving the workgroup count. Traversal stacks move from LDS to a global per-query buffer, so LDS per workgroup no longer grows with the extra slice. The block reductions are reindexed per slice and reuse the dead transform staging area. The mode is picked at create time from an LDS occupancy check. It removes idle half-workgroups and LDS pressure, at the cost of global-memory stack traffic.

```diff
diff --git a/include/psi_hip.h b/include/psi_hip.h
--- a/include/psi_hip.h
+++ b/include/psi_hip.h
@@ -111,6 +111,8 @@
                     int *h_n_stages, void *stream);
 int psi_fit_copy_buffer(psi_fit_engine *engine, const char *name, float *d_out, long n_floats, void *stream);
 
+int psi_fit_search_shape(const psi_fit_engine *engine, int *lanes, int *slices, int *workgroups);
+
 size_t psi_linear_workspace_floats(int M, int N, int K);
 int psi_linear_forward(const void *x, int x_is_bf16, const float *W, const float *bias, const float *residual, int M, int N, int K,
                        int act, float slope, float *y, float *act_out, float *ws, void *stream);
diff --git a/psi-release_amd/csrc/fit.hip b/psi-release_amd/csrc/fit.hip
--- a/psi-release_amd/csrc/fit.hip
+++ b/psi-release_amd/csrc/fit.hip
@@ -9,6 +9,7 @@
 #define PSI_CSTOP() do { if (psi_dbg_cstop) asm volatile("s_endpgm"); } while (0)
 #define PSI_TRACE(lo, hi) PsiBlockTrace trace_((lo), (hi))
 __device__ unsigned long long psi_dbg_tl[4 * 8192];
+__device__ unsigned long long psi_dbg_tlw[2 * 4 * 8192];
 struct PsiBlockTrace {
     unsigned long long t0;
     int kind;
@@ -17,7 +18,13 @@
     __device__ ~PsiBlockTrace()
     {
         const unsigned bid = blockIdx.y * gridDim.x + blockIdx.x;
-        if (psi_dbg_sstop < sel_lo || psi_dbg_sstop > sel_hi || threadIdx.x != 0 || bid >= 8192) return;
+        if (psi_dbg_sstop < sel_lo || psi_dbg_sstop > sel_hi || bid >= 8192) return;
+        if ((threadIdx.x & 63) == 0 && threadIdx.x < 256) {
+            unsigned long long *w = psi_dbg_tlw + 2 * (4 * (size_t)bid + (threadIdx.x >> 6));
+            w[0] = wall_clock64();
+            w[1] = (unsigned long long)__builtin_amdgcn_s_getreg((31 << 11) | 4);
+        }
+        if (threadIdx.x != 0) return;
         unsigned long long *o = psi_dbg_tl + 4 * (size_t)bid;
         o[0] = t0;
         o[1] = wall_clock64();
@@ -28,6 +35,10 @@
 extern "C" int psi_dbg_timeline(unsigned long long *out, int nblocks)
 {
     return (int)hipMemcpyFromSymbol(out, HIP_SYMBOL(psi_dbg_tl), sizeof(unsigned long long) * 4 * (size_t)(nblocks < 8192 ? nblocks : 8192));
+}
+extern "C" int psi_dbg_timeline_waves(unsigned long long *out, int nblocks)
+{
+    return (int)hipMemcpyFromSymbol(out, HIP_SYMBOL(psi_dbg_tlw), sizeof(unsigned long long) * 8 * (size_t)(nblocks < 8192 ? nblocks : 8192));
 }
 #endif
 #include "lbs_device.h"
@@ -596,12 +607,13 @@
         out[p] = __builtin_bit_cast(float, __builtin_amdgcn_readlane(__builtin_bit_cast(int, x), psi_sum_last_lane(LPQ, p)));
 }
 
-template <int LPQ>
+template <int LPQ, int SPW = 1>
 struct ContactSkinSrc {
     static_assert(LPQ == 2 || LPQ == 4, "the query's lane group skins its own vertex with 2 or 4 lanes");
-    static constexpr int NT = psikd::kd_threads(LPQ);
+    static_assert(SPW == 1 || (SPW == 2 && LPQ == 2), "two slices per workgroup: the 2-lane search");
+    static constexpr int NT = SPW * psikd::kd_threads(LPQ);
     static constexpr int NST = (PSI_JP * 6 + NT - 1) / NT;
-    static constexpr int CT0 = LPQ == 2 ? 80 : 128;
+    static constexpr int CT0 = NT == 128 ? 80 : 128;
     FitDev f;
     LbsDev m;
     const float *As, *v_posed;
@@ -647,7 +659,7 @@
     {
         psi_f2 (*sA_)[6] = psi_transform_stage<1>()[0];
         __shared__ float sCT_[16];
-        __shared__ float sTR_[psikd::kd_qpb(LPQ)][9];
+        __shared__ float sTR_[SPW * psikd::kd_qpb(LPQ)][9];
 #pragma unroll
         for (int q = 0; q < NST; q++) {
             const int idx = threadIdx.x + q * NT;
@@ -737,8 +749,17 @@
     {
         if (!f.fused_bwd) return;
         constexpr int PPW = psi_sum_parts_per_wave(LPQ);
-        __shared__ float wsum3[psi_sum_parts(LPQ)][3];
-        __shared__ float wmax[psi_sum_waves(LPQ)];
+        __shared__ float wsum3_[SPW == 2 ? 1 : psi_sum_parts(LPQ)][3];
+        __shared__ float wmax_[SPW == 2 ? 1 : psi_sum_waves(LPQ)];
+        float (*wsum3)[3] = wsum3_;
+        float *wmax = wmax_;
+        if constexpr (SPW == 2) {
+            static_assert(sizeof(psi_f2) * 6 * PSI_JP >= sizeof(float) * (SPW * psi_sum_parts(LPQ) * 3 + SPW * psi_sum_waves(LPQ)), "the staging area holds both tables");
+            float *dead = (float *)&psi_transform_stage<1>()[0][0][0];
+            wsum3 = (float (*)[3])dead;
+            wmax = dead + SPW * psi_sum_parts(LPQ) * 3;
+        }
+        const int pr = SPW == 2 ? (bx & 1) : 0, t0 = pr * psi_sum_wg_pair_threads(LPQ);
         float sx[PPW], sy[PPW], sz[PPW];
         psi_contact_part_sums<LPQ>(gs[0], sx);
         psi_contact_part_sums<LPQ>(gs[1], sy);
@@ -749,24 +770,25 @@
         if ((threadIdx.x & 63) == 0) {
 #pragma unroll
             for (int p = 0; p < PPW; p++) {
-                wsum3[psi_sum_slot(LPQ, threadIdx.x >> 6, p)][0] = sx[p];
-                wsum3[psi_sum_slot(LPQ, threadIdx.x >> 6, p)][1] = sy[p];
-                wsum3[psi_sum_slot(LPQ, threadIdx.x >> 6, p)][2] = sz[p];
+                const unsigned s = SPW == 2 ? psi_sum_wg_slot(LPQ, SPW, threadIdx.x >> 6, p) : psi_sum_slot(LPQ, threadIdx.x >> 6, p);
+                wsum3[s][0] = sx[p];
+                wsum3[s][1] = sy[p];
+                wsum3[s][2] = sz[p];
             }
             wmax[threadIdx.x >> 6] = mx;
         }
         __syncthreads();
-        if (threadIdx.x == 64) {
-            float m2 = wmax[0];
-#pragma unroll
-            for (int w = 1; w < psi_sum_waves(LPQ); w++) m2 = fmaxf(m2, wmax[w]);
+        if ((int)threadIdx.x == t0 + 64) {
+            float m2 = wmax[pr * psi_sum_waves(LPQ)];
+#pragma unroll
+            for (int w = 1; w < psi_sum_waves(LPQ); w++) m2 = fmaxf(m2, wmax[pr * psi_sum_waves(LPQ) + w]);
             if (m2 > 0.0f) atomicMax(f.gvbits + PSI_GV_SLOTS + (size_t)b * f.gv_sps + (bx & (f.gv_sps - 1)), __float_as_uint(m2));
         }
-        if (threadIdx.x < 3) {
+        if ((int)threadIdx.x >= t0 && (int)threadIdx.x < t0 + 3) {
             float a = 0.0f;
 #pragma unroll
-            for (int w = 0; w < psi_sum_parts(LPQ); w++) a += wsum3[w][threadIdx.x];
-            f.gtc_part[((size_t)b * nbx + bx) * 4 + threadIdx.x] = a;
+            for (int w = 0; w < psi_sum_parts(LPQ); w++) a += wsum3[pr * psi_sum_parts(LPQ) + w][(int)threadIdx.x - t0];
+            f.gtc_part[((size_t)b * nbx + bx) * 4 + ((int)threadIdx.x - t0)] = a;
         }
     }
 };
@@ -785,9 +807,10 @@
 template <bool SCENES>
 using SceneTrees = std::conditional_t<SCENES, const psikd::KdDev *__restrict__, psikd::KdDev>;
 
-template <int NB, bool SCENES, int LPQ>
+template <int NB, bool SCENES, int LPQ, int SPW>
 __global__ __launch_bounds__(256, 6) void fwd_scene_kernel(FitDev f, LbsDev m, const float *__restrict__ As, const float *__restrict__ v_posed,
-                                                           SceneTrees<SCENES> T, int n_kd, int nqb, int rows, float gscale, int skin_first, SdfEpilogue<SCENES> epi)
+                                                           SceneTrees<SCENES> T, int n_kd, int nqb, int rows, float gscale, int skin_first, SdfEpilogue<SCENES> epi,
+                                                           int *__restrict__ kd_stack)
 {
     extern __shared__ int smem_i[];
 #ifdef PSI_HEAD_STOPS
@@ -817,8 +840,8 @@
             tab = T;
             slot = epi.slot;
         } else tree = T;
-        psikd::kd_query_body<LPQ, true, SCENES>(tree, ContactSkinSrc<LPQ>{f, m, As, v_posed, nullptr, {}, 0.0f, 0, 0.0f, 0.0f, 0.0f, nullptr, {}, 0}, f.n_c, (float *)nullptr, (int *)nullptr,
-                                           f.cconst, gscale, f.fused_bwd ? (float *)nullptr : f.gq, f.fpart, f.nn_hint, rows, tab, slot, bx, b, nqb, smem_i);
+        psikd::kd_query_body<LPQ, true, SCENES, SPW>(tree, ContactSkinSrc<LPQ, SPW>{f, m, As, v_posed, nullptr, {}, 0.0f, 0, 0.0f, 0.0f, 0.0f, nullptr, {}, 0}, f.n_c, (float *)nullptr, (int *)nullptr,
+                                           f.cconst, gscale, f.fused_bwd ? (float *)nullptr : f.gq, f.fpart, f.nn_hint, rows, tab, slot, bx, b, SPW == 2 ? f.nfp : nqb, smem_i, kd_stack);
     } else {
         const int i = bid;
         if constexpr (SCENES) epi.template load_grids<NB>((i / f.nsdfblk) * NB, f.B);
@@ -1447,7 +1470,7 @@
 
 struct FitKnobs {
     bool split_scene, keep_verts, no_fused_bwd, sdf_linear, scene_skin_first, bwdv_mb, no_pen_skip, bwd_pf1, chain_in_head;
-    int head_cluster, skin_nb, ska_nbody, search_lanes;
+    int head_cluster, skin_nb, ska_nbody, search_lanes, search_spw;
 #ifdef PSI_HEAD_STOPS
     int head_stop, tail_stop, skin_stop;
 #endif
@@ -1473,6 +1496,7 @@
     k.ska_nbody = psi_ska_nbody_override(SKA_NBODY);
     const int sl = num("PSI_FIT_SEARCH_LANES");
     if (sl == 2 || sl == 4) k.search_lanes = sl;
+    if (num("PSI_FIT_SEARCH_SPW") == 1) k.search_spw = 1;
 #ifdef PSI_HEAD_STOPS
     k.head_stop = num("PSI_HEAD_STOP");
     k.tail_stop = num("PSI_TAIL_STOP");
@@ -1488,6 +1512,7 @@
     bool fused_bwd;
     int skin_nb;
     int search_lanes;
+    int search_spw;
     int hc;
     int gv_sps;
     PsiStreamSplit split;
@@ -1500,6 +1525,7 @@
     d.self_skin = cfg->nn_mode == 1 && J <= PSI_JP - 8 && psikd::kd_qpb(psikd::LPQ_OPS) == psikd::kd_qpb(2);
     d.search_lanes = knobs.search_lanes ? knobs.search_lanes : mc.compressed_weights ? 4 : PSI_FIT_SEARCH_LANES_DEFAULT;
     d.merged_scene = d.self_skin && cfg->B <= 128 && !knobs.split_scene;
+    d.search_spw = d.search_lanes == 2 && !knobs.search_spw ? 2 : 1;
     d.keep_verts = !d.merged_scene || knobs.keep_verts;
     const long bodies = (long)cfg->B * (cfg->concurrent_engines > 1 ? cfg->concurrent_engines : 1);
     d.hc = bodies <= 32 ? 8 : bodies <= 64 ? 4 : bodies <= 128 ? 2 : 1;
@@ -1635,6 +1661,8 @@
     PsiSdfGrid *d_grid_tab;
     int *d_slot;
     int kd_rows;
+    char *search_blob;
+    int *kd_stack;
     FitGraph graphs[FIT_N_GRAPHS];
     const float *half_stats[2];
     const void *dp_comm;
@@ -1699,11 +1727,11 @@
     return 0;
 }
 
-template <int NB, bool SCENES, int LPQ>
+template <int NB, bool SCENES, int LPQ, int SPW>
 static void launch_fwd_scene(const psi_fit_engine *e, float gscale, hipStream_t st)
 {
     const FitDev &f = e->d;
-    const int nqb = f.nfp, n_kd = nqb * f.B, skin_first = e->knobs.scene_skin_first ? 1 : 0;
+    const int nqb = psi_cdiv(f.nfp, SPW), n_kd = nqb * f.B, skin_first = e->knobs.scene_skin_first ? 1 : 0;
     const dim3 grid(n_kd + f.nsdfblk * psi_cdiv(f.B, NB));
     FitDev fk = f;
     if (!e->mode.keep_verts) fk.verts = nullptr;
@@ -1717,8 +1745,8 @@
         T = psi_nn_index_dev(e->nn_index);
         rows = T.rows;
     }
-    hipLaunchKernelGGL((fwd_scene_kernel<NB, SCENES, LPQ>), grid, dim3(256), psikd::kd_lds_bytes(LPQ, rows), st, fk, e->lv.m, e->lv.A, e->lv.v_posed, T, n_kd, nqb, rows,
-                       gscale, skin_first, epi);
+    hipLaunchKernelGGL((fwd_scene_kernel<NB, SCENES, LPQ, SPW>), grid, dim3(256), psikd::kd_lds_bytes(LPQ, rows), st, fk, e->lv.m, e->lv.A, e->lv.v_posed, T, n_kd, nqb, rows,
+                       gscale, skin_first, epi, e->kd_stack);
 }
 
 template <int NB, bool SCENES>
@@ -1750,8 +1778,9 @@
     float gscale = f.w_contact / ((f.indep ? 1.0f : (float)f.B * (float)f.world) * (float)f.n_c);
     if (e->nn_index && e->mode.merged_scene) {
         fit_scene_dispatch(e, [&](auto nb, auto scenes) {
-            if (e->mode.search_lanes == 2) launch_fwd_scene<decltype(nb)::value, decltype(scenes)::value, 2>(e, gscale, st);
-            else launch_fwd_scene<decltype(nb)::value, decltype(scenes)::value, 4>(e, gscale, st);
+            if (e->mode.search_lanes == 2 && e->mode.search_spw == 2) launch_fwd_scene<decltype(nb)::value, decltype(scenes)::value, 2, 2>(e, gscale, st);
+            else if (e->mode.search_lanes == 2) launch_fwd_scene<decltype(nb)::value, decltype(scenes)::value, 2, 1>(e, gscale, st);
+            else launch_fwd_scene<decltype(nb)::value, decltype(scenes)::value, 4, 1>(e, gscale, st);
         });
         PSI_CHECK_LAUNCH("fwd_scene_kernel");
         psi_mark("fwd_scene_kernel", st);
@@ -1860,6 +1889,39 @@
     std::vector<float> hs((size_t)m * 3);
     *err = hipMemcpy(hs.data(), d_verts, hs.size() * 4, hipMemcpyDeviceToHost);
     return *err == hipSuccess ? psi_nn_index_create(out, hs.data(), m) : (int)*err;
+}
+
+template <int NB, bool SCENES, int SPW>
+static size_t fwd_scene_static_lds()
+{
+    hipFuncAttributes a;
+    if (hipFuncGetAttributes(&a, reinterpret_cast<const void *>(&fwd_scene_kernel<NB, SCENES, 2, SPW>)) != hipSuccess) {
+        (void)hipGetLastError();
+        return 0;
+    }
+    return a.sharedSizeBytes;
+}
+static int fit_search_shape(psi_fit_engine *e)
+{
+    const FitDev &f = e->d;
+    const char *who = e->n_scenes ? "psi_fit_create_scenes" : "psi_fit_create";
+    const int rows = e->n_scenes ? e->kd_rows : psi_nn_index_dev(e->nn_index).rows;
+    int dev = 0, lds_cu = 0;
+    PSI_CHECK_HIP(hipGetDevice(&dev));
+    if (hipDeviceGetAttribute(&lds_cu, hipDeviceAttributeMaxSharedMemoryPerMultiprocessor, dev) != hipSuccess) {
+        (void)hipGetLastError();
+        lds_cu = 0;
+    }
+    size_t s1 = 0, s2 = 0;
+    fit_scene_dispatch(e, [&](auto nb, auto scenes) {
+        s1 = fwd_scene_static_lds<decltype(nb)::value, decltype(scenes)::value, 1>();
+        s2 = fwd_scene_static_lds<decltype(nb)::value, decltype(scenes)::value, 2>();
+    });
+    e->mode.search_spw = psi_search_stack_fits(f.n_c, rows) ? psi_search_spw_for((size_t)lds_cu, s1, s2, psikd::kd_lds_bytes(2, rows), 6) : 1;
+    if (e->mode.search_spw != 2) return 0;
+    PsiBlob T;
+    T.raw(e->kd_stack, psi_search_stack_bytes(f.B, f.n_c, rows));
+    return psi_blob_realise(T, &e->search_blob, who);
 }
 
 static int fit_create(psi_fit_engine **out, const psi_lbs_model *lbs, const psi_fit_config *cfg,
@@ -2032,6 +2094,8 @@
     } else if (cfg->nn_mode == 1) {
         if (int rc = fit_scene_index(&e->nn_index, d_scene_verts, f.m, &err)) return rc;
     }
+    if (e->nn_index && mode.merged_scene && mode.search_spw == 2)
+        if (int rc = fit_search_shape(e)) return rc;
     owner.release();
     *out = e;
     return 0;
@@ -2152,6 +2216,7 @@
         delete[] e->scene_vol;
     }
     (void)hipFree(e->scene_blob);
+    (void)hipFree(e->search_blob);
     for (FitGraph &G : e->graphs) fit_graph_drop(&G);
     (void)hipFree(e->blob);
     delete e;
@@ -2381,6 +2446,16 @@
     PSI_REQUIRE(e && d_out4 && adam_step >= 1, "bad arguments");
     FitDev &f = e->d;
     PSI_CHECK_HIP(hipMemcpyAsync(d_out4, f.history + (size_t)((adam_step - 1) % f.max_hist) * 4, 16, hipMemcpyDeviceToDevice, (hipStream_t)stream));
+    return 0;
+}
+
+extern "C" int psi_fit_search_shape(const psi_fit_engine *e, int *lanes, int *slices, int *workgroups)
+{
+    PSI_REQUIRE(e && lanes && slices && workgroups, "null pointer");
+    const bool shared = e->nn_index && e->mode.merged_scene;
+    *lanes = shared ? e->mode.search_lanes : 0;
+    *slices = shared ? e->mode.search_spw : 0;
+    *workgroups = shared ? e->d.B * psi_cdiv(e->d.nfp, e->mode.search_spw) : 0;
     return 0;
 }
 
diff --git a/psi-release_amd/csrc/nnindex.hip b/psi-release_amd/csrc/nnindex.hip
--- a/psi-release_amd/csrc/nnindex.hip
+++ b/psi-release_amd/csrc/nnindex.hip
@@ -23,7 +23,7 @@
                                                         const int *__restrict__ slot = nullptr)
 {
     extern __shared__ int smem_i[];
-    kd_query_body<LPQ, CONTACT, MULTI>(T0, KdQueryFromMemory{xyz1, qidx, qstride}, n, dist, idx, cconst, gscale, gq, fpart, hint, rows, tab, slot,
+    kd_query_body<LPQ, CONTACT, MULTI, 1>(T0, KdQueryFromMemory{xyz1, qidx, qstride}, n, dist, idx, cconst, gscale, gq, fpart, hint, rows, tab, slot,
                                   (int)blockIdx.x, (int)blockIdx.y, (int)gridDim.x, smem_i);
 }
 
diff --git a/psi-release_amd/csrc/nnindex_device.h b/psi-release_amd/csrc/nnindex_device.h
--- a/psi-release_amd/csrc/nnindex_device.h
+++ b/psi-release_amd/csrc/nnindex_device.h
@@ -3,6 +3,7 @@
 #include <math.h>
 #include "psi_common.h"
 #include "search_sum_order.h"
+#include "search_shape.h"
 
 #ifndef PSI_SSTOP
 #define PSI_SSTOP(k)
@@ -122,25 +123,42 @@
     __device__ __forceinline__ void contact_finish(int, int, int) {}
 };
 
-template <int LPQ>
-__device__ __forceinline__ void kd_block_fsum(float fval, float *__restrict__ out)
-{
-    __shared__ float wsum[psi_sum_parts(LPQ)];
+template <int LPQ, int SPW = 1>
+__device__ __forceinline__ void kd_block_fsum(float fval, float *__restrict__ out, int pr = 0)
+{
+    __shared__ float wsum[SPW * psi_sum_parts(LPQ)];
     const int tid = threadIdx.x;
     float v = fval;
 #pragma unroll
     for (int o2 = psi_sum_part_lanes(LPQ) / 2; o2 > 0; o2 >>= 1) v += __shfl_down(v, o2, 64);
 #pragma unroll
     for (int p = 0; p < psi_sum_parts_per_wave(LPQ); p++)
-        if ((tid & 63) == psi_sum_first_lane(LPQ, p)) wsum[(int)psi_sum_slot(LPQ, tid >> 6, p)] = v;
+        if ((tid & 63) == psi_sum_first_lane(LPQ, p)) wsum[(int)(SPW == 2 ? psi_sum_wg_slot(LPQ, SPW, tid >> 6, p) : psi_sum_slot(LPQ, tid >> 6, p))] = v;
     __syncthreads();
-    if (tid == 0) {
+    if (tid == pr * psi_sum_wg_pair_threads(LPQ)) {
         float t = 0.0f;
 #pragma unroll
-        for (int w = 0; w < psi_sum_parts(LPQ); w++) t += wsum[w];
+        for (int w = 0; w < psi_sum_parts(LPQ); w++) t += wsum[pr * psi_sum_parts(LPQ) + w];
         *out = t;
     }
 }
+
+template <int SPW, class T>
+__device__ __forceinline__ T kd_stack_ld(const T *p)
+{
+    if constexpr (SPW == 2) return __hip_atomic_load(p, __ATOMIC_RELAXED, __HIP_MEMORY_SCOPE_WORKGROUP);
+    else return *p;
+}
+template <int SPW, class T>
+__device__ __forceinline__ void kd_stack_st(T *p, T v)
+{
+    if constexpr (SPW == 2) __hip_atomic_store(p, v, __ATOMIC_RELAXED, __HIP_MEMORY_SCOPE_WORKGROUP);
+    else *p = v;
+}
+template <int SPW>
+__device__ __forceinline__ void kd_stack_pushed() { if constexpr (SPW == 2) __builtin_amdgcn_fence(__ATOMIC_RELEASE, "workgroup"); }
+template <int SPW>
+__device__ __forceinline__ void kd_stack_popped() { if constexpr (SPW == 2) __builtin_amdgcn_fence(__ATOMIC_ACQUIRE, "workgroup"); }
 
 __device__ __forceinline__ int kd_warm_hint(const int *__restrict__ hint, bool active, size_t o) { return (active && hint) ? hint[o] : -1; }
 __device__ __forceinline__ int kd_warm_candidate(const KdDev &T, int h, float4 &hp)
@@ -157,17 +175,17 @@
     return *(T *)((char *)(tab + obase * K + k) + (unsigned)jq * (unsigned)(4 * K));
 }
 
-template <int LPQ, int RPL, bool CONTACT, class QSrc>
+template <int LPQ, int RPL, bool CONTACT, int SPW, class QSrc>
 __device__ __forceinline__ float kd_query_round(const KdDev &T, QSrc &qsrc, float qx, float qy, float qz, bool active, size_t o, float *__restrict__ dist,
                                                 int *__restrict__ idx, float cconst, float gscale, float *__restrict__ gq, int *__restrict__ hint,
-                                                int rows, int *smem_i, int h, const float4 &hp, size_t obase, int jq)
+                                                int rows, int *smem_i, int h, const float4 &hp, size_t obase, int jq, int *__restrict__ gstk)
 {
 #pragma clang fp contract(off)
     constexpr int CPL = kd_cpl(LPQ);
     const int tid = threadIdx.x;
     const int c = tid & (LPQ - 1);
     const int g = tid / LPQ;
-    int *stk_n = smem_i + (size_t)g * rows * 2;
+    int *stk_n = smem_i + (size_t)g * rows * (SPW == 2 ? 1 : 2);
     float *stk_d = (float *)(stk_n + rows);
     kd_key bestk = kd_pack(INFINITY, 0x7fffffff);
     float best = INFINITY;
@@ -218,7 +236,7 @@
         if (fncand <= (float)GRID_MAX_CAND) {
             const int ncand = (int)fncand;
             const float rny = __builtin_amdgcn_rcpf(fny);
-            const int list_max = min(GRID_LIST_MAX, 2 * rows);
+            const int list_max = min(GRID_LIST_MAX, SPW == 2 ? rows : 2 * rows);
             int nsurv = 0;
             for (int c0 = 0; c0 < ncand; c0 += LPQ) {
                 const float fcol = (float)(c0 + c);
@@ -306,11 +324,21 @@
             } else { PSI_KD_STAT(if (c == 0 && psi_dbg_sstop == 10) { atomicAdd(psi_kd_reason + 1, 1); atomicMax(psi_kd_reason + 5, nsurv); }) }
         } else { PSI_KD_STAT(if (c == 0 && psi_dbg_sstop == 10) { atomicAdd(psi_kd_reason + 0, 1); atomicMax(psi_kd_reason + 4, (int)fminf(fncand, 1e6f)); }) }
     } else { PSI_KD_STAT(if (have && c == 0 && psi_dbg_sstop == 10) atomicAdd(psi_kd_reason + 3, 1);) }
+    char *const gbase = SPW == 2 ? (char *)gstk + obase * (size_t)rows * 8 : nullptr;
+    auto ref_at = [&](int i) -> int * {
+        if constexpr (SPW == 2) return (int *)(gbase + psi_search_stack_entry(jq, rows, 0, i));
+        else return stk_n + i;
+    };
+    auto dist_at = [&](int i) -> float * {
+        if constexpr (SPW == 2) return (float *)(gbase + psi_search_stack_entry(jq, rows, 1, i));
+        else return stk_d + i;
+    };
     while (true) {
         while (!have && sp > 0) {
             --sp;
-            cur = stk_n[sp];
-            curd = stk_d[sp];
+            cur = kd_stack_ld<SPW>(ref_at(sp));
+            curd = kd_stack_ld<SPW>(dist_at(sp));
+            kd_stack_popped<SPW>();
             have = !(curd * 0.999999f > best);
         }
         if (!have) break;
@@ -341,11 +369,12 @@
                 const unsigned gm = (unsigned)(__ballot(push) >> gshift) & ((1u << LPQ) - 1u);
                 if (push) {
                     const int pos = sp + __popc(gm & ((1u << c) - 1u));
-                    stk_n[pos] = ref[u];
-                    stk_d[pos] = dc[u];
+                    kd_stack_st<SPW>(ref_at(pos), ref[u]);
+                    kd_stack_st<SPW>(dist_at(pos), dc[u]);
                 }
                 sp += __popc(gm);
             }
+            kd_stack_pushed<SPW>();
             int rsel = ref[0];
 #pragma unroll
             for (int u = 1; u < CPL; u++) rsel = (cmin / LPQ == u) ? ref[u] : rsel;
@@ -411,15 +440,18 @@
     return fval;
 }
 
-template <int LPQ, bool CONTACT, bool MULTI, class QSrc>
+template <int LPQ, bool CONTACT, bool MULTI, int SPW, class QSrc>
 __device__ __forceinline__ void kd_query_body(KdDev T0, QSrc qsrc, int n, float *__restrict__ dist, int *__restrict__ idx, float cconst,
                                               float gscale, float *__restrict__ gq, float *__restrict__ fpart, int *__restrict__ hint,
                                               int rows, const KdDev *__restrict__ tab, const int *__restrict__ slot, int bx, int b, int nbx,
-                                              int *smem_i)
-{
-    constexpr int QPB = kd_qpb(LPQ);
+                                              int *smem_i, int *__restrict__ gstk = nullptr)
+{
+    static_assert(SPW == 1 || (SPW == 2 && 2 * kd_threads(LPQ) == QBLK), "two slices per workgroup: two wave pairs of 64 queries");
+    constexpr int QPB = SPW * kd_qpb(LPQ);
     const int tid = threadIdx.x;
-    if (kd_threads(LPQ) < QBLK && tid >= kd_threads(LPQ)) return;
+    if (SPW == 1 && kd_threads(LPQ) < QBLK && tid >= kd_threads(LPQ)) return;
+    const int pr = SPW == 2 ? __builtin_amdgcn_readfirstlane(psi_sum_wg_pair(LPQ, SPW, tid)) : 0;
+    const int sl = psi_sum_wg_slice(SPW, bx, pr);
     const int c = tid & (LPQ - 1), g = tid / LPQ;
     const KdDev T = MULTI ? tab[slot[b]] : T0;
     const int j = bx * QPB + g;
@@ -434,13 +466,14 @@
     qsrc.fetch(b);
     const int h = kd_warm_candidate(T, h0, hp);
     qsrc.prepare(b);
+    if (SPW == 2 && sl >= nbx) return;
     qsrc.point(b, active ? j : 0, c, qx, qy, qz);
     PSI_SSTOP(4);
     PSI_KD_MARK(0);
-    const float fval = kd_query_round<LPQ, kd_rpl(LPQ), CONTACT>(T, qsrc, qx, qy, qz, active, o, dist, idx, cconst, gscale, gq, hint, rows, smem_i, h, hp, obase, jq);
+    const float fval = kd_query_round<LPQ, kd_rpl(LPQ), CONTACT, SPW>(T, qsrc, qx, qy, qz, active, o, dist, idx, cconst, gscale, gq, hint, rows, smem_i, h, hp, obase, jq, gstk);
     if (CONTACT) {
-        kd_block_fsum<LPQ>(fval, fpart + (size_t)b * nbx + bx);
-        qsrc.contact_finish(b, bx, nbx);
+        kd_block_fsum<LPQ, SPW>(fval, fpart + (size_t)b * nbx + sl, pr);
+        qsrc.contact_finish(b, sl, nbx);
     }
 }
 
diff --git a/psi-release_amd/csrc/search_shape.h b/psi-release_amd/csrc/search_shape.h
--- /dev/null
+++ b/psi-release_amd/csrc/search_shape.h
@@ -0,0 +1,25 @@
+#pragma once
+#include <stddef.h>
+
+#if defined(__HIPCC__) || defined(__CUDACC__)
+#define PSI_SHAPE_HD __host__ __device__
+#else
+#define PSI_SHAPE_HD
+#endif
+
+PSI_SHAPE_HD constexpr size_t psi_search_stack_bytes(int B, int n, int rows) { return (size_t)B * (size_t)n * (size_t)rows * 8; }
+PSI_SHAPE_HD constexpr size_t psi_search_stack_body_base(int b, int n, int rows) { return (size_t)b * (size_t)n * (size_t)rows * 8; }
+PSI_SHAPE_HD constexpr bool psi_search_stack_fits(int n, int rows) { return n > 0 && rows > 0 && (size_t)n * (size_t)rows * 8 < ((size_t)1 << 32); }
+PSI_SHAPE_HD constexpr unsigned psi_search_stack_entry(int jq, int rows, int which, int i)
+{
+    return (unsigned)jq * (unsigned)(8 * rows) + 4u * (unsigned)(which * rows + i);
+}
+
+PSI_SHAPE_HD constexpr int psi_search_wgs_per_cu(size_t lds_cu, size_t lds_static, size_t lds_dynamic, int cap)
+{
+    return lds_static + lds_dynamic == 0 ? cap : (int)(lds_cu / (lds_static + lds_dynamic)) < cap ? (int)(lds_cu / (lds_static + lds_dynamic)) : cap;
+}
+PSI_SHAPE_HD constexpr int psi_search_spw_for(size_t lds_cu, size_t static1, size_t static2, size_t lds_dynamic, int cap)
+{
+    return static1 && static2 && psi_search_wgs_per_cu(lds_cu, static2, lds_dynamic, cap) >= psi_search_wgs_per_cu(lds_cu, static1, lds_dynamic, cap) ? 2 : 1;
+}
diff --git a/psi-release_amd/csrc/search_sum_order.h b/psi-release_amd/csrc/search_sum_order.h
--- a/psi-release_amd/csrc/search_sum_order.h
+++ b/psi-release_amd/csrc/search_sum_order.h
@@ -15,6 +15,14 @@
 PSI_SUM_HD constexpr unsigned psi_sum_slot(int lpq, unsigned w, int p) { return w * (unsigned)psi_sum_parts_per_wave(lpq) + (unsigned)p; }
 PSI_SUM_HD constexpr int psi_sum_first_lane(int lpq, int p) { return p * psi_sum_part_lanes(lpq); }
 PSI_SUM_HD constexpr int psi_sum_last_lane(int lpq, int p) { return (p + 1) * psi_sum_part_lanes(lpq) - 1; }
+PSI_SUM_HD constexpr int psi_sum_wg_pair_threads(int lpq) { return psi_sum_waves(lpq) * 64; }
+PSI_SUM_HD constexpr int psi_sum_wg_pair(int lpq, int spw, int tid) { return spw == 2 ? tid / psi_sum_wg_pair_threads(lpq) : 0; }
+PSI_SUM_HD constexpr int psi_sum_wg_slice(int spw, int bx, int pair) { return spw * bx + pair; }
+PSI_SUM_HD constexpr unsigned psi_sum_wg_slot(int lpq, int spw, unsigned w, int p)
+{
+    return spw == 2 ? (w / (unsigned)psi_sum_waves(lpq)) * (unsigned)psi_sum_parts(lpq) + psi_sum_slot(lpq, w % (unsigned)psi_sum_waves(lpq), p)
+                    : psi_sum_slot(lpq, w, p);
+}
 PSI_SUM_HD inline float psi_sum_slots(const float *slot, int stride, int lpq)
 {
     float t = 0.0f;
diff --git a/psi-release_amd/hip.py b/psi-release_amd/hip.py
--- a/psi-release_amd/hip.py
+++ b/psi-release_amd/hip.py
@@ -105,6 +105,7 @@
     'psi_fit_decode_backward': (c_int, [c_void_p, c_void_p, c_void_p, c_void_p]),
     'psi_fit_profile': (c_int, [c_void_p, c_int, c_void_p, c_int, c_void_p, c_int, c_void_p, c_void_p]),
     'psi_fit_copy_buffer': (c_int, [c_void_p, ctypes.c_char_p, c_void_p, c_long, c_void_p]),
+    'psi_fit_search_shape': (c_int, [c_void_p, c_void_p, c_void_p, c_void_p]),
     'psi_lbs_sdf_counts': (c_int, [c_void_p] * 5 + [c_int] + [c_void_p] * 4 + [c_int] * 3 + [c_void_p] * 3),
     'psi_kmeans_create': (c_int, [c_void_p, c_void_p, c_int, c_int, c_void_p, c_int, c_int, c_float]),
     'psi_kmeans_destroy': (None, [c_void_p]),
```

New measurement: 11890 (median of 6 runs). 1.02x the previous value.
